# NealLiufighting/hpmpc

Measured on AMD Instinct MI355X. Metric: Riccati factorisations/sec + IP iters/sec, fp64, N=100 nx=12 nu=4 batch=1024, higher is better.
Workload: dtype f64

## Files before the change

hpmpc_amd/bindings.py:

```python
from __future__ import annotations

import ctypes as C
import os

import numpy as np

LIBPATH = os.environ.get("HPMPC_MI355X_LIB") or os.path.join(os.path.dirname(os.path.abspath(__file__)), "lib",
                                                             "libhpmpc_mi355x.so")

_CTYPE = dict(v=None, i=C.c_int, d=C.c_double, l=C.c_longlong, p=C.c_void_p, s=C.c_char_p)
_SIG = dict(
    plan_create="p:ippppp",
    plan_destroy="v:p",
    ws_doubles="l:p",
    ipm_batch="i:ppiiippppppppidddiipppp",
    ipm_solo="i:ppiiippppppppidddiipppp",
    ipm_pass="i:ppiiippppppppidddiipppip",
    ipm_batch_profiled="i:ppiiippppppppidddiippppp",
    ipm_queue="i:ppiiipppppppppidddiipppppp",
    ric_sv_batch="i:ppiiipppppiipp",
    ric_trf_batch="i:ppiiipppp",
    ric_trs_batch="i:ppiiipppppppiipp",
    last_error="i:",
    version="s:",
    pcond_plan_create="p:ipppppi",
    pcond_plan_destroy="v:p",
    pcond_sizes="i:pp",
    pcond_offsets="i:pip",
    pcond_batch="i:piiippppppppp",
    pcond_ric_sv_batch="i:piiipppppip",
    pexpand_batch="i:piiippppppppppp",
    wide_plan_create="p:ippppp",
    wide_plan_destroy="v:p",
    wide_sizes="i:pp",
    wide_offsets="i:pp",
    wide_ipm_batch="i:piiipppppppppidddiipppp",
    pcond_wide_plan="p:p",
    soft_plan_create="p:ipppppp",
    soft_plan_destroy="v:p",
    soft_sizes="i:pp",
    soft_offsets="i:pp",
    ipm_soft_batch="i:ppiiippppppppppidddiipppp",
    ocp_plan_create="p:ipppppi",
    ocp_plan_destroy="v:p",
    ocp_tile_plan="p:p",
    ocp_sizes="i:pp",
    ocp_offsets="i:pp",
    ocp_pack_batch="i:ppiiiipppppppp",
    ocp_ipm_batch="i:piiipppppppppidddiipppp",
    ocp_finish_batch="i:piiipppppppppppppppp",
    kkt_scratch_doubles="l:p",
    kkt_new_rhs_batch="i:ppiiiippppppppppppip",
    ocp_kkt_batch="i:piiippppppppppp",
    ocp_unpack_sets="i:piiiippppppppppp",
    kkt_tangent_batch="i:ppiiiippppppppppppip",
    ocp_tangent_batch="i:ppiiiippppppppppip",
    kkt_adjoint_batch="i:ppiiiippppppppppppp",
    ocp_adjoint_batch="i:piiiipppppppppppppppppp",
    ocp_matrix_grads_batch="i:piiiipppppppp",
    ocp_adjoint_data_batch="i:piiiippppppppppppppp",
    ocp_matrix_dirs_batch="i:ppiiiippppppp",
    ocp_tangent_data_batch="i:ppiiiipppppppppppppip",
)
SIGNATURES = {"hpmpc_mi355x_" + n: (_CTYPE[s[0]], [_CTYPE[c] for c in s[2:]]) for n, s in _SIG.items()}

_LIB = None


def bind(L):
    for name, (restype, argtypes) in SIGNATURES.items():
        fn = getattr(L, name, None)
        if fn is not None:
            fn.restype, fn.argtypes = restype, argtypes
    return L


def lib() -> C.CDLL:
    global _LIB
    if _LIB is None:
        if not os.path.exists(LIBPATH):
            raise RuntimeError(f"libhpmpc_mi355x.so not built ({LIBPATH}); run __graft_entry__.build()")
        _LIB = bind(C.CDLL(LIBPATH, mode=os.RTLD_LOCAL | getattr(os, "RTLD_NOW", 2)))
    return _LIB


def check(rc: int, name: str) -> None:
    if rc != 0:
        raise RuntimeError(f"{name} failed ({rc})")


def plan_args(idxb, *sizes):
    ints = lambda a: np.ascontiguousarray(a, dtype=np.int32)
    arrs, idx = [ints(a) for a in sizes], [ints(a) for a in idxb]
    idxp = (C.POINTER(C.c_int) * len(idx))(*[a.ctypes.data_as(C.POINTER(C.c_int)) for a in idx])
    return [a.ctypes.data for a in arrs], C.cast(idxp, C.c_void_p), (arrs, idx, idxp)
```

hpmpc_amd/build.py:

```python
from __future__ import annotations

import os
import subprocess

ROOT = os.path.dirname(os.path.dirname(os.path.abspath(__file__)))
CSRC = os.path.join(ROOT, "hpmpc_amd", "csrc")
LIBDIR = os.path.join(ROOT, "hpmpc_amd", "lib")
HIPCC = os.environ.get("HIPCC", "/opt/rocm/bin/hipcc")
ARCH = os.environ.get("HPMPC_ARCH", "gfx950")
SOURCES = ["hpmpc_kernels.hip", "hk_wide.hip", "hk_wide_ipm.hip", "hk_soft.hip", "hk_soft_ipm.hip", "hk_ocp.hip", "hk_kkt.hip", "hk_tan.hip", "hk_adj.hip", "hk_matgrad.hip", "hk_matdir.hip", "hpmpc_capi.cpp",
           "hpmpc_capi_queue.cpp", "hpmpc_capi_dropin.cpp", "hpmpc_capi_soft.cpp", "hpmpc_capi_soft_batch.cpp",
           "hpmpc_capi_wide.cpp", "hpmpc_capi_pcond.cpp", "hpmpc_capi_wide_ipm.cpp", "hpmpc_capi_iface.cpp",
           "hpmpc_capi_mpc.cpp", "hpmpc_capi_ocp.cpp", "hpmpc_capi_kkt.cpp"]
HEADERS = ["hpmpc_api.h", "hk_ipm_body.h", "hk_prims.h", "hk_riccati.h", "hk_ipm.h", "hk_mw.h", "hpmpc_kargs.h", "hk_wide_args.h", "hk_wide_core.h", "hk_wide_host.h", "hk_pcond_plan.h", "hk_soft_args.h", "hk_soft_body.h", "hk_launch_guard.h", "hk_launch.h", "hk_host.h", "hk_plan.h", "hk_ocp_args.h", "hk_kkt_args.h", "hk_kkt_body.h", "hk_ocp_plan.h", "hk_tan_args.h", "hk_tan_body.h", "hk_ocp_place.h", "hk_kkt_launch.h", "hk_adj_args.h", "hk_adj_body.h", "hk_matgrad_args.h", "hk_matdir_args.h"]
KFLAGS = ["-mllvm", "-amdgpu-mfma-vgpr-form"] + os.environ.get("HK_EXTRA_FLAGS", "").split()
SRC_FLAGS = {"hpmpc_kernels.hip": ["-mllvm", "-amdgpu-sched-strategy=max-memory-clause"],
             "hk_kkt.hip": ["-mllvm", "-amdgpu-sched-strategy=max-memory-clause"],
             "hk_tan.hip": ["-mllvm", "-amdgpu-sched-strategy=max-memory-clause"],
             "hk_adj.hip": ["-mllvm", "-amdgpu-sched-strategy=max-memory-clause"]}


EXPORTS = os.path.join(CSRC, "exports.map")


def _newer(out, deps):
    if not os.path.exists(out):
        return False
    t = os.path.getmtime(out)
    return all(os.path.getmtime(d) <= t for d in deps)


def _deps(src, hdrs_all):
    import re
    seen, todo = set(), [os.path.join(CSRC, src)]
    while todo:
        path = todo.pop()
        try:
            text = open(path).read()
        except OSError:
            continue
        for name in re.findall(r'^\s*#\s*include\s+"([^"]+)"', text, re.M):
            for cand in (os.path.join(os.path.dirname(path), name), os.path.join(CSRC, name),
                         os.path.join(ROOT, "include", os.path.basename(name))):
                if os.path.exists(cand) and cand not in seen:
                    seen.add(cand)
                    todo.append(cand)
                    break
    return sorted(seen | {h for h in hdrs_all if os.path.basename(h) == "hpmpc_mi355x.h"})


def build_hip(force: bool = False, verbose: bool = False, variant: str | None = None, extra=(), sources=()) -> str:
    os.makedirs(LIBDIR, exist_ok=True)
    objdir = os.path.join(ROOT, "build", "obj" if variant is None else f"obj_{variant}")
    os.makedirs(objdir, exist_ok=True)
    out = os.path.join(LIBDIR, "libhpmpc_mi355x.so")
    if variant is not None:
        os.makedirs(os.path.join(LIBDIR, "ab"), exist_ok=True)
        out = os.path.join(LIBDIR, "ab", f"lib{variant}.so")
    hdrs_all = [os.path.join(CSRC, h) for h in HEADERS] + [os.path.join(ROOT, "include", "hpmpc_mi355x.h")]
    common = [HIPCC, f"--offload-arch={ARCH}", "-O3", "-std=c++17", "-fPIC", "-fvisibility=hidden", "-Wall",
              "-Wno-unused-function"] + KFLAGS + list(extra)
    objs, procs = [], []
    for src in SOURCES + list(sources):
        obj = os.path.join(objdir, src + ".o")
        objs.append(obj)
        if force or not _newer(obj, [os.path.join(CSRC, src)] + _deps(src, hdrs_all)):
            cmd = common + SRC_FLAGS.get(src, []) + ["-c", os.path.join(CSRC, src), "-o", obj]
            if verbose:
                print(" ".join(cmd), flush=True)
            procs.append((src, subprocess.Popen(cmd)))
    for src, pr in procs:
        if pr.wait() != 0:
            raise subprocess.CalledProcessError(pr.returncode, src)
    if procs or force or not _newer(out, objs + [EXPORTS]):
        cmd = [HIPCC, f"--offload-arch={ARCH}", "-shared", "-fPIC", f"-Wl,--version-script={EXPORTS}"] + objs + \
              ["-o", out]
        if verbose:
            print(" ".join(cmd), flush=True)
        subprocess.run(cmd, check=True)
    return out


def build_stamps(verbose: bool = False, force: bool = False) -> str:
    out = build_hip(force=force, verbose=verbose, variant="stamps", extra=["-DHK_STAMPS"])
    dst = os.path.join(LIBDIR, "libhpmpc_mi355x_stamps.so")
    if not _newer(dst, [out]):
        import shutil

        shutil.copy2(out, dst)
    return dst


def build_ric2(verbose: bool = False, force: bool = False) -> str:
    return build_hip(force=force, verbose=verbose, variant="ric2", extra=["-DHK_RIC2"], sources=["hk_ric2.hip"])


def build_calib(verbose: bool = False) -> str:
    os.makedirs(LIBDIR, exist_ok=True)
    out = os.path.join(LIBDIR, "libhbm_calib.so")
    src = os.path.join(ROOT, "tools", "hbm_calib.hip")
    if _newer(out, [src, os.path.join(CSRC, "hk_prims.h")]):
        return out
    cmd = [HIPCC, f"--offload-arch={ARCH}", "-O3", "-std=c++17", "-fPIC", "-shared", src, "-o", out]
    if verbose:
        print(" ".join(cmd), flush=True)
    subprocess.run(cmd, check=True)
    return out


def build_oracle(force: bool = False) -> None:
    odir = os.path.join(ROOT, "oracle")
    targets = ["oracle", "oracle_fma"]
    if os.path.isdir(os.environ.get("HPMPC_REF", "/root/reference")):
        targets += ["ref", "ref_avx"]
    subprocess.run(["make", "-s", "-C", odir] + (["-B"] if force else []) + targets, check=True)
    if "ref" in targets:
        subprocess.run(["make", "-s", "-C", os.path.join(ROOT, "tools", "relink"), "drivers"], check=True)


def build_all(force: bool = False, verbose: bool = False) -> None:
    build_hip(force=force, verbose=verbose)
    build_stamps(verbose=verbose, force=force)
    build_ric2(verbose=verbose, force=force)
    build_calib(verbose=verbose)
    build_oracle(force=force)


if __name__ == "__main__":
    build_all(force=True, verbose=True)
```

hpmpc_amd/csrc/hk_ipm_body.h:

```cpp
#pragma once
#include "hk_ipm.h"
#include "hk_launch_guard.h"
#include "hpmpc_kargs.h"

using namespace hk;

#ifndef HK_WAVES
#define HK_WAVES 2
#endif
#define HK_TWO_WAVES __attribute__((amdgpu_waves_per_eu(HK_WAVES)))

namespace {

struct Ws {
    double *F, *dux, *dpi, *Pb, *Qx, *qx, *res_q, *res_b, *ux_bkp, *pi_bkp;
    double *dlam, *dt, *t_inv, *lamt, *res_d, *res_m, *t_bkp, *lam_bkp;
    double* state;
    double* cert;
};

enum { S_MU = 0, S_ALPHA, S_SIGMA, S_SMU, S_KK, S_PHASE, S_ACTIVE, S_MUSCAL, S_RET };

__device__ __forceinline__ Ws carve(double* W, int N) {
    Ws w;
    const long n1 = N + 1, a = n1 * V16, b = n1 * V32;
    w.F = W;
    W += n1 * FSTRIDE;
    w.dux = W;
    w.dpi = W + a;
    w.Pb = W + 2 * a;
    w.Qx = W + 3 * a;
    w.qx = W + 4 * a;
    w.res_q = W + 5 * a;
    w.res_b = W + 6 * a;
    w.ux_bkp = W + 7 * a;
    w.pi_bkp = W + 8 * a;
    W += 9 * a;
    w.dlam = W;
    w.dt = W + b;
    w.t_inv = W + 2 * b;
    w.lamt = W + 3 * b;
    w.res_d = W + 4 * b;
    w.res_m = W + 5 * b;
    w.t_bkp = W + 6 * b;
    w.lam_bkp = W + 7 * b;
    w.state = W + 8 * b;
    w.cert = w.state + 16;
    return w;
}

extern __shared__ __attribute__((aligned(16))) char hk_smem[];

struct LdsTabs {
    Scratch* sm;
    const StageInfo* st;
    const signed char* tileslot;
    const signed char* slotvar;
    double* gc;
};

__device__ __forceinline__ LdsTabs lds_tables(const KArgs& a) {
    LdsTabs T;
    T.sm = reinterpret_cast<Scratch*>(hk_smem);
    StageInfo* st = reinterpret_cast<StageInfo*>(hk_smem + sizeof(Scratch));
    signed char* ts = reinterpret_cast<signed char*>(st + (a.N + 1));
    signed char* sv = ts + (a.N + 1) * 16;
    const int l = lane_id(), n1 = a.N + 1;
    const int* gst = reinterpret_cast<const int*>(a.st);
    int* lst = reinterpret_cast<int*>(st);
    for (int i = l; i < n1 * 16; i += 64) lst[i] = gst[i];
    const int* gts = reinterpret_cast<const int*>(a.tileslot);
    const int* gsv = reinterpret_cast<const int*>(a.slotvar);
    int* lts = reinterpret_cast<int*>(ts);
    int* lsv = reinterpret_cast<int*>(sv);
    for (int i = l; i < n1 * 4; i += 64) {
        lts[i] = gts[i];
        lsv[i] = gsv[i];
    }
    __syncthreads();
    T.st = st;
    T.tileslot = ts;
    T.slotvar = sv;
    T.gc = reinterpret_cast<double*>(sv + n1 * 16);
    return T;
}

static_assert(LDS_FIXED == sizeof(Scratch) && LDS_PER_STAGE == sizeof(StageInfo) + 40, "hpmpc_kargs.h LDS constants");
constexpr size_t lds_table_bytes(int N) { return LDS_FIXED + (size_t)(N + 1) * LDS_PER_STAGE; }

__device__ __forceinline__ RicIO make_io(const KArgs& a, const LdsTabs& T, int p, double* F) {
    RicIO io;
    io.N = a.N;
    io.st = T.st;
    io.tileslot = T.tileslot;
    io.BAbt = a.BAbt + (long)p * a.sB;
    io.RSQ = a.RSQ + (long)p * a.sR;
    io.BAbtS = a.BAbt;
    io.RSQS = a.RSQ;
    io.F = F;
    io.DCt = a.DCt ? a.DCt + (long)p * a.sG : a.RSQ;
    return io;
}

__device__ __forceinline__ void wsync() { __syncthreads(); }

}

namespace {

template <int CH>
__device__ void init_var(const RicIO& io, const double* dv, double* ux, double* pi, double* dpi, double* lam,
                         double* t, double mu0, int warm_start) {
    const int l = lane_id(), g = l >> 4, c = l & 15;
    const double thr0 = 0.1;
    const int nq = (io.N + 4) / 4;
    for (int q0 = 0; q0 < nq; q0 += CH) {
        double dl[CH], du[CH], xv[CH];
        int lo[CH], up[CH], iv[CH];
        bool kv[CH], bx[CH], kp[CH];
#pragma unroll
        for (int j = 0; j < CH; j++) {
            const int k = 4 * (q0 + j) + g;
            kv[j] = k <= io.N;
            kp[j] = k < io.N;
            const int kc = kv[j] ? k : io.N;
            const StageInfo& si = io.st[kc];
            const bool okv = c < si.nu + si.nx;
            const int tile = c < si.nu ? c : si.xo + (c - si.nu);
            const int slot = okv ? io.tileslot[kc * 16 + (okv ? tile : 0)] : -1;
            bx[j] = kv[j] && slot >= 0;
            lo[j] = kc * V32 + (slot >= 0 ? slot : 0);
            up[j] = lo[j] + si.pnb;
            iv[j] = kc * V16 + c;
            dl[j] = gld(dv, lo[j], bx[j]);
            du[j] = gld(dv, up[j], bx[j]);
            xv[j] = warm_start ? gld(ux, iv[j], kv[j]) : 0.0;
        }
#pragma unroll
        for (int j = 0; j < CH; j++) {
            double x = xv[j];
            double tl = -dl[j] + x, tu = du[j] - x;
            if (tl < thr0) {
                if (tu < thr0) {
                    x = (-du[j] + dl[j]) * 0.5;
                    tl = thr0;
                    tu = thr0;
                } else {
                    tl = thr0;
                    x = dl[j] + thr0;
                }
            } else if (tu < thr0) {
                tu = thr0;
                x = du[j] - thr0;
            }
            x = bx[j] ? x : xv[j];
            gst(ux, iv[j], x, kv[j]);
            gst(pi, iv[j], 0.0, kp[j]);
            gst(dpi, iv[j], 0.0, kv[j]);
            gst(t, lo[j], tl, bx[j]);
            gst(t, up[j], tu, bx[j]);
            gst(lam, lo[j], mu0 / tl, bx[j]);
            gst(lam, up[j], mu0 / tu, bx[j]);
        }
    }
}

__device__ void init_var_gen(const RicIO& io, const double* dv, const double* ux, double* lam, double* t,
                             double mu0) {
    const int l = lane_id(), c = l & 15;
    const double thr0 = 0.1;
    for (int k = 0; k <= io.N; k++) {
        const StageInfo si = load_stage(io.st, k);
        if (si.ng == 0) continue;
        const DynSh sh(si);
        const int vc = tile_var(c, sh.nu, sh.nx, sh.xo);
        const double x = gld(ux, k * V16 + vc, vc >= 0);
        double dg[4];
        gen_dg(io, sh, dg);
#pragma unroll
        for (int lc = 0; lc < 4; lc++) {
            if (4 * lc >= sh.ng) continue;
            const GenLane q = gen_lane(k, sh.pnb, sh.ng, lc);
            const bool st = q.ok && c == 0;
            const double dx = row_sum16(dg[lc] * x);
            const double tl = fmax(thr0, dx + (-gld(dv, q.lo, q.ok)));
            const double tu = fmax(thr0, -dx + gld(dv, q.up, q.ok));
            gst(t, q.lo, tl, st);
            gst(t, q.up, tu, st);
            gst(lam, q.lo, mu0 / tl, st);
            gst(lam, q.up, mu0 / tu, st);
        }
    }
}

__device__ __forceinline__ BoxCtx box_ctx(const Ws& w, const double* dv, double* lam, double* t) {
    BoxCtx bc{};
    bc.d = dv;
    bc.lam = lam;
    bc.t = t;
    bc.dlam = w.dlam;
    bc.dt = w.dt;
    bc.t_inv = w.t_inv;
    bc.lamt = w.lamt;
    bc.res_d = w.res_d;
    bc.res_m = w.res_m;
    bc.qxs = w.qx;
    bc.Qx = w.Qx;
    bc.qx = w.qx;
    bc.cert = w.cert;
    bc.cert_out = w.cert;
    bc.cert_new = 0;
    bc.res_q = w.res_q;
    bc.res_b = w.res_b;
    return bc;
}

}

namespace {

struct IpmView {
    int N, q, l;
    Ws w;
    RicIO io;
    BoxTab bt;
    double *ux, *pi, *lam, *t, *stat;
    const double* dv;
    BoxCtx bc;
};

__device__ __forceinline__ int* qcount(const KArgs& a, int p) { return a.qctl + 2 + a.nslots + p; }
__device__ __forceinline__ int* qlist(const KArgs& a, int p) { return a.qctl + 4 + a.nslots + p * a.nslots; }
__device__ __forceinline__ void qlist_push(const KArgs& a, int p, int s) {
    if (lane_id() == 0) qlist(a, p)[atomicAdd(qcount(a, p), 1)] = s;
}

struct Who {
    int s, q, d;
};

__device__ __forceinline__ bool who_am_i(const KArgs& a, Who& w) {
    if (a.nq == 0) {
        const int p = blockIdx.x + a.p0;
        w.s = w.q = w.d = p;
        return p < a.nprob;
    }
    const int n = __builtin_amdgcn_readfirstlane(*qcount(a, a.qpar));
    if ((int)blockIdx.x >= n) return false;
    w.s = __builtin_amdgcn_readfirstlane(qlist(a, a.qpar)[blockIdx.x]);
    w.q = __builtin_amdgcn_readfirstlane(a.qctl[2 + w.s]);
    w.d = w.q >= 0 ? w.q % a.nprob : 0;
    return w.q >= 0;
}

__device__ __forceinline__ bool slot_active(const KArgs& a, const Who& who) {
    return carve(a.ws + (long)who.s * a.sW, a.N).state[S_ACTIVE] != 0.0;
}

__device__ __forceinline__ IpmView ipm_view(const KArgs& a, const LdsTabs& T, const Who& who) {
    IpmView v;
    v.N = a.N;
    v.q = who.q;
    v.l = lane_id();
    v.w = carve(a.ws + (long)who.s * a.sW, a.N);
    v.io = make_io(a, T, who.d, v.w.F);
    v.bt = BoxTab{T.tileslot, T.slotvar};
    const long o16 = (long)who.q * a.sV16, o32 = (long)who.q * a.sV32;
    v.ux = a.ux + o16;
    v.pi = a.pi + o16;
    v.lam = a.lam + o32;
    v.t = a.t + o32;
    v.dv = a.d + (long)who.d * a.sV32;
    v.stat = a.stat + (long)who.q * 5 * a.k_max;
    v.bc = box_ctx(v.w, v.dv, v.lam, v.t);
    v.bc.ux = v.ux;
    v.bc.pi = v.pi;
    return v;
}

__device__ __forceinline__ ResIO res_io(const IpmView& v) {
    ResIO ro{};
    ro.ux = v.ux;
    ro.pi = v.pi;
    ro.dux = v.w.dux;
    ro.dpi = v.w.dpi;
    ro.ux_bkp = v.w.ux_bkp;
    ro.pi_bkp = v.w.pi_bkp;
    ro.lam_bkp = v.w.lam_bkp;
    ro.t_bkp = v.w.t_bkp;
    ro.rq = v.w.res_q;
    ro.rb = v.w.res_b;
    ro.rd = v.w.res_d;
    ro.rm = v.w.res_m;
    return ro;
}

template <class FX, int CI, int NW = 1>
__device__ double p2_start(const KArgs& a, IpmView& v, const MwSplit& mws = MwSplit{0, nullptr}) {
    const double mu = update_p2_pass<CI, false, true, NW>(v.io, v.bc, v.bt.slotvar, 0.0, 1.0 / (2.0 * a.nbt), v.ux,
                                                          v.pi, nullptr, nullptr, nullptr, nullptr, nullptr, nullptr,
                                                          v.w.res_d, v.w.res_m, mws);
    wsync();
    return mu;
}

template <class FX, int CI, int NW = 1>
__device__ bool ipm_continue(const KArgs& a, IpmView& v, int kk, double mu, double alpha, double sigma, int phase,
                             const MwSplit& mws = MwSplit{0, nullptr}) {
    const bool sn = a.single_newton != 0;
    bool active;
    if (a.phase1_only) {
        active = kk < a.k_max && mu > a.mu_tol && alpha >= a.alpha_min;
    } else {
        if (phase == 1) {
            const double mu_tol_low = a.mu_tol < 1e-5 ? 1e-5 : a.mu_tol;
            if (!(kk < a.k_max && mu > mu_tol_low && alpha >= a.alpha_min)) {
                mu = p2_start<FX, CI, NW>(a, v, mws);
                phase = 2;
            }
        }
        active = phase == 1;
        if (phase == 2) active = kk < a.k_max && (sn || (mu > a.mu_tol && alpha >= a.alpha_min));
    }
    int ret = 0;
    if (!active) {
        if (!sn && mu <= a.mu_tol)
            ret = 0;
        else if (kk >= a.k_max)
            ret = 1;
        else if (alpha < a.alpha_min)
            ret = 2;
        else
            ret = -1;
    }
    if (v.l == 0) {
        double* st = v.w.state;
        st[S_MU] = mu;
        st[S_ALPHA] = alpha;
        st[S_SIGMA] = sigma;
        st[S_KK] = kk;
        st[S_PHASE] = phase;
        st[S_ACTIVE] = active ? 1.0 : 0.0;
        if (!active) {
            a.kk[v.q] = kk;
            a.ret[v.q] = ret;
        }
    }
    return active;
}

template <class FX, int CI, bool SHORTCUT>
__device__ bool ipm_start(const KArgs& a, const LdsTabs& T, IpmView& v) {
    Scratch& sm = *T.sm;
    const int N = v.N, l = v.l;
    const int nbt = a.nbt;
    if (!SHORTCUT && nbt == 0) return false;
    if (SHORTCUT && nbt == 0 && a.phase1_only) {
        ric_backward<true, BX_NONE, FX>(v.io, &sm, 0, nullptr, 0, nullptr, v.bc, 1, v.w.Pb);
        wsync();
        ric_forward_sv<FX>(v.io, &sm, 0, nullptr, v.w.dux, a.compute_mult, v.w.dpi);
        if (l == 0) {
            v.w.state[S_ACTIVE] = 0.0;
            a.kk[v.q] = 0;
            a.ret[v.q] = 0;
        }
        return false;
    }
    if (SHORTCUT && nbt == 0) {
        ric_backward<true, BX_NONE, FX>(v.io, &sm, 0, nullptr, 0, nullptr, v.bc, 1, v.w.Pb);
        wsync();
        ric_forward_sv<FX>(v.io, &sm, 0, nullptr, v.ux, a.compute_mult, v.pi);
        wsync();
        for (int i = l; i < (N + 1) * V16; i += 64) {
            v.w.ux_bkp[i] = v.ux[i];
            v.w.pi_bkp[i] = v.pi[i];
        }
        if (l == 0) {
            v.w.state[S_ACTIVE] = 0.0;
            a.kk[v.q] = 0;
            a.ret[v.q] = 0;
        }
        return false;
    }
    const bool sn = a.single_newton != 0;
    if (!sn) {
        init_var<CI>(v.io, v.dv, v.ux, v.pi, v.w.dpi, v.lam, v.t, a.mu0, a.warm_start);
        if (a.ngt) {
            wsync();
            init_var_gen(v.io, v.dv, v.ux, v.lam, v.t, a.mu0);
        }
    } else {
        for (int i = l; i < (N + 1) * V16; i += 64) v.w.dpi[i] = 0.0;
    }
    if (l == 0) v.w.state[S_MUSCAL] = 1.0 / (2.0 * nbt);
    wsync();
    double mu = a.mu0;
    if (sn) mu = p2_start<FX, CI>(a, v);
    return ipm_continue<FX, CI>(a, v, 0, mu, 1.0, 0.0, sn ? 2 : 1);
}

template <class FX, int CI, bool SHORTCUT>
__device__ bool ipm_refill(const KArgs& a, const LdsTabs& T, int s) {
    const bool l0 = lane_id() == 0;
    for (;;) {
        int q = 0;
        if (l0) q = atomicAdd(a.qnext, 1);
        q = __builtin_amdgcn_readfirstlane(q);
        if (q >= a.nq) {
            if (l0) a.qctl[2 + s] = -1;
            return false;
        }
        if (l0) a.qctl[2 + s] = q;
        const Who who{s, q, q % a.nprob};
        IpmView v = ipm_view(a, T, who);
        if (ipm_start<FX, CI, SHORTCUT>(a, T, v)) return true;
        if (l0) atomicAdd(&a.qctl[1], 1);
    }
}

}

namespace {

template <class FX>
__device__ __forceinline__ void fact_body(const KArgs& a, const LdsTabs& T, IpmView& v) {
    Scratch& sm = *T.sm;
    const double* st = v.w.state;
    const bool sn = a.single_newton != 0;
    const bool first = st[S_KK] == 0.0;
    if (first && st[S_PHASE] != 1.0) {
        cert_pass(v.io, v.w.cert);
        wsync();
    }
    if (!first || st[S_PHASE] != 1.0)
        for (int i = v.l; i <= v.N; i += 64) T.gc[i] = v.w.cert[i];
    wsync();
    v.bc.cert = T.gc;
    if (st[S_PHASE] == 1.0) {
        if (first)
            ric_backward<true, BX_P1, FX, CERT_FORM>(v.io, &sm, 0, nullptr, 0, nullptr, v.bc, 1, v.w.Pb);
        else
            ric_backward<true, BX_P1, FX, CERT_LOAD>(v.io, &sm, 0, nullptr, 0, nullptr, v.bc, 1, v.w.Pb);
    } else {
        v.bc.res_rhs = !sn;
        v.bc.no_tinv = a.no_bkp;
        ric_backward<true, BX_P2R, FX, CERT_LOAD>(v.io, &sm, 0, nullptr, 0, nullptr, v.bc, 1, v.w.Pb);
    }
}

template <class FX>
__device__ __forceinline__ void pred_body(const KArgs& a, const LdsTabs& T, IpmView& v) {
    Scratch& sm = *T.sm;
    double* st = v.w.state;
    const bool sn = a.single_newton != 0;
    const int phase = (int)st[S_PHASE], kk = (int)st[S_KK];
    const double mu = st[S_MU];
    double sigma = st[S_SIGMA];
    double al = 1.0;
    if (phase == 1) {
        v.bc.pred = 1;
        ric_forward<0, BX_P1, FX, true>(v.io, &sm, nullptr, 0, v.w.dux, 0, v.w.dpi, v.bc, al);
    } else {
        ric_forward<0, BX_P2, FX, true>(v.io, &sm, v.w.res_b, !sn, v.w.dux, 0, v.w.dpi, v.bc, al);
    }
    al = wave_min(al);
    wsync();
    const double alpha = al * 0.995;
    const double mu_aff = mu_aff_pass<7>(v.io, v.bc, alpha, st[S_MUSCAL]);
    double smu = a.mu0;
    if (!sn) {
        sigma = mu_aff / mu;
        sigma = sigma * sigma * sigma;
        smu = sigma * mu;
    }
    if (v.l == 0) {
        v.stat[5 * kk] = st[S_SIGMA];
        v.stat[5 * kk + 1] = al;
        v.stat[5 * kk + 2] = mu_aff;
        st[S_SIGMA] = sigma;
        st[S_SMU] = smu;
    }
}

template <class FX>
__device__ __forceinline__ void corr_body(const KArgs& a, const LdsTabs& T, IpmView& v) {
    Scratch& sm = *T.sm;
    double* st = v.w.state;
    const int phase = (int)st[S_PHASE], kk = (int)st[S_KK];
    v.bc.smu = st[S_SMU];
    double al = 1.0;
    if (phase == 1)
        ric_trs<BX_P1, BX_P1, FX, false>(v.io, &sm, nullptr, nullptr, v.bc, v.w.dux, a.compute_mult, v.w.dpi, 0, v.w.Pb,
                                         al);
    else
        ric_trs<BX_P2, BX_P2, FX, false>(v.io, &sm, v.w.res_b, v.w.res_q, v.bc, v.w.dux, a.compute_mult, v.w.dpi, 0,
                                         v.w.Pb, al);
    al = wave_min(al);
    if (v.l == 0) {
        v.stat[5 * kk] = st[S_SIGMA];
        v.stat[5 * kk + 3] = al;
        st[S_ALPHA] = al * 0.995;
    }
}

template <class FX, int CI>
__device__ __forceinline__ bool update_body(const KArgs& a, IpmView& v) {
    double* st = v.w.state;
    const int phase = (int)st[S_PHASE];
    int kk = (int)st[S_KK];
    const double alpha = st[S_ALPHA];
    double mu;
    if (phase == 1) {
        mu = update_p1_pass<CI>(v.io, v.bc, alpha, st[S_MUSCAL], v.ux, v.pi, v.w.dux, v.w.dpi, v.w.ux_bkp,
                                v.w.pi_bkp, v.w.lam_bkp, v.w.t_bkp);
    } else {
        if (a.no_bkp)
            mu = update_p2_pass<CI, true, false>(v.io, v.bc, v.bt.slotvar, alpha, st[S_MUSCAL], v.ux, v.pi, v.w.dux,
                                                 v.w.dpi, v.w.ux_bkp, v.w.pi_bkp, v.w.lam_bkp, v.w.t_bkp, v.w.res_d,
                                                 v.w.res_m);
        else
            mu = update_p2_pass<CI, true>(v.io, v.bc, v.bt.slotvar, alpha, st[S_MUSCAL], v.ux, v.pi, v.w.dux, v.w.dpi,
                                          v.w.ux_bkp, v.w.pi_bkp, v.w.lam_bkp, v.w.t_bkp, v.w.res_d, v.w.res_m);
    }
    wsync();
    if (v.l == 0) v.stat[5 * kk + 4] = mu;
    kk++;
    return ipm_continue<FX, CI>(a, v, kk, mu, alpha, st[S_SIGMA], phase);
}

}
```

hpmpc_amd/csrc/hk_plan.h:

```cpp
#pragma once
#include <climits>
#include <mutex>
#include <vector>

#include "hk_host.h"
#include "hk_soft_args.h"
#include "hpmpc_kargs.h"

struct StageInfoH {
    int nu, nx, nb, ng, xo, nx1, nu1, xo1, sdB, sdR, oB, oR, oD, pnb, r0, oG;
};

struct hpmpc_mi355x_plan {
    int N = 0;
    std::vector<int> nx, nu, nb, ng;
    std::vector<std::vector<int>> idxb;
    std::vector<StageInfoH> st;
    std::vector<signed char> tileslot, slotvar;
    std::vector<long long> offB, offR;
    long long packB = 0, packR = 0;
    DevTable<StageInfoH> d_st;
    DevTable<signed char> d_tileslot, d_slotvar;
    struct LayoutTable {
        std::vector<StageInfoH> st;
        DevTable<StageInfoH> d;
    };
    mutable std::vector<LayoutTable> ltabs;
    mutable std::mutex ltabs_mu;
    int fixcls = 0;
    int nbt = 0;
    int ngt = 0;
    std::vector<long long> offG;
    long long packG = 0;
};

inline long long ws_doubles(int N) {
    const long long n = (long long)(N + 1) * (FSTRIDE + 9 * V16 + 8 * V32 + 1) + 16;
    return (n + 31) / 32 * 32;
}

bool plan_supported(int N, const int* nx, const int* nu, const int* nb, const int* const* idxb, const int* ng,
                    const char** why);
void idxb_table(int N, const int* nb, const int* const* idxb, int* out);
bool range_ok(const void* plan, int nprob, int p0, int count, const char* who);
int null_array(const char* who);
int launch_error(int e, const char* what);
inline bool sets_ok(int nprob, int n, const char* what) {
    if (n >= 1 && (long long)nprob * n <= INT_MAX) return true;
    hk_set_error(HPMPC_MI355X_EUNSUPPORTED, what);
    return false;
}
enum DctPolicy { DCT_NONE, DCT_ARRAY };
bool batch_args(KArgs& a, const hpmpc_mi355x_plan* P, const hpmpc_mi355x_layout* lay, int nprob, int p0,
                DctPolicy policy, const double* DCt = nullptr);
int launch(int which, const KArgs* a, int count, hipStream_t s);
int ipm_run(KArgs& a, int count, const double* BAbt, const double* RSQrq, const double* d, double* ux, double* pi,
            double* lam, double* t, double* ws, int k_max, double mu0, double mu_tol, double alpha_min, int warm_start,
            int compute_mult, int* kk, int* ret, double* stat, int which, void* stream);
hpmpc_mi355x_plan* thread_plan(int N, const int* nx, const int* nu, const int* nb, int** idxb, const int* ng);

struct Arena {
    size_t BAbt, RSQ, DCt, d, ux, pi, lam, t, ws, vb, vq, vQx, vqx, vPb, stat, ints, qctl, total;
};
Arena arena(const hpmpc_mi355x_plan* P, int k_max);
KArgs arena_args(const hpmpc_mi355x_plan* P, const Arena& A, double* dev);
void stage_BAbt(const hpmpc_mi355x_plan* P, double* H, const Arena& A, double** hpBAbt);
void stage_RSQ(const hpmpc_mi355x_plan* P, double* H, const Arena& A, double** hpQ);
bool run(int which, const KArgs& a, const char* name);
enum VecKind { VEC_UX, VEC_PI, VEC_CV };
void vec_in(const hpmpc_mi355x_plan* P, VecKind kind, double* H, size_t off, double** v);
void vec_out(const hpmpc_mi355x_plan* P, VecKind kind, double** v, const double* H, size_t off);

struct SoftLayout {
    std::vector<SoftStage> st;
    long sC = 0, sD = 0, sZ = 0;
    long sF = 0;
};
double soft_mu_scal(int N, const int* nb, const int* ns);
void soft_ric_flags(KArgs& a, int compute_mult);
SoftArgs soft_scalars(int N, int nprob, int p0, int k_max, int warm_start, double mu0, double mu_tol, double alpha_min,
                      double mu_scal);
const char* soft_unsupported(int N, const int* nx, const int* nu, const int* ng);
const char* soft_layout(int N, const int* nx, const int* nu, const int* nb, const int* ns, SoftLayout& L);
```

hpmpc_amd/csrc/hk_riccati.h:

```cpp
#pragma once

#include "hk_prims.h"
#include "hpmpc_kargs.h"

namespace hk {

struct StageInfo {
    int nu, nx, nb, ng;
    int xo;
    int nx1, nu1, xo1;
    int sdB, sdR;
    int oB, oR, oD;
    int pnb;
    int r0;
    int oG;
};

using ::FSTRIDE;
using ::V16;
using ::V32;

__device__ __forceinline__ bool tile_active(int t, int nu, int nx, int xo) {
    return t < nu || (t >= xo && t < xo + nx);
}
// ... 81 lines not shown
    HK_BSTAMP(2);
    const double i1 = chol_inv(fma(-l10, l10, a11));
    const double l21 = fma(-l20, l10, a21) * i1, l31 = fma(-l30, l10, a31) * i1;
    const double y1 = fma(-y0, l10, x[1]) * i1;
    const double p1 = fma(-p0, l10, m1) * i1;
    HK_BSTAMP(3);
    const double i2 = chol_inv(fma(-l21, l21, fma(-l20, l20, a22)));
    const double l32 = fma(-l31, l21, fma(-l30, l20, a32)) * i2;
    const double y2 = fma(-y1, l21, fma(-y0, l20, x[2])) * i2;
    const double p2 = fma(-p1, l21, fma(-p0, l20, m2)) * i2;
    HK_BSTAMP(4);
    const double i3 = chol_inv(fma(-l32, l32, fma(-l31, l31, fma(-l30, l30, a33))));
    const double y3 = fma(-y2, l32, fma(-y1, l31, fma(-y0, l30, x[3]))) * i3;
    const double p3 = fma(-p2, l32, fma(-p1, l31, fma(-p0, l30, m3))) * i3;
    HK_BSTAMP(5);
    if (KGEN && B == 0) {
        const bool ut = c < 4;
        const double e0 = ut ? (c == 0 ? 1.0 : 0.0) : y0, e1 = ut ? (c == 1 ? 1.0 : 0.0) : y1;
        const double e2 = ut ? (c == 2 ? 1.0 : 0.0) : y2, e3 = ut ? (c == 3 ? 1.0 : 0.0) : y3;
        const double z3 = e3 * i3;
        const double z2 = fma(-l32, z3, e2) * i2;
        const double z1 = fma(-l31, z3, fma(-l21, z2, e1)) * i1;
        const double z0 = fma(-l30, z3, fma(-l20, z2, fma(-l10, z1, e0))) * i0;
        *kg = -sel_g(z0, z1, z2, z3);
    }
    const double yg = sel_g(y0, y1, y2, y3);
    M[B] = yg;
    const int j = c - 4 * B;
    const bool inb = (c >> 2) == B, below = c > 4 * B + 3;
    invd = inb ? sel_q(i0, i1, i2, i3) : invd;
    if (AUG) {
        const double mt = fma(-p3, y3, fma(-p2, y2, fma(-p1, y1, fma(-p0, y0, ml))));
        const double mb = sel_q(p0, p1, p2, p3);
        ml = below ? mt : (inb ? mb : ml);
    }
    HK_BSTAMP(6);
    (void)j;
    if (B < 3) {
        const double a = below ? yg : 0.0;
        M = mfma(-a, a, M);
    }
#undef HK_BSTAMP
}

template <int B, bool AUG, bool KGEN>
__device__ __forceinline__ void chol_block_row(const d4& S, double invd, double& ml, double* kg) {
    const int l = lane_id(), c = l & 15;
    double y[4];
    rowgroup_gather(S[B], y);
    const double i0 = row_bcast<4 * B + 0>(invd), i1 = row_bcast<4 * B + 1>(invd);
    const double i2 = row_bcast<4 * B + 2>(invd), i3 = row_bcast<4 * B + 3>(invd);
    const double l10 = row_bcast<4 * B + 1>(y[0]), l20 = row_bcast<4 * B + 2>(y[0]), l30 = row_bcast<4 * B + 3>(y[0]);
    const double l21 = row_bcast<4 * B + 2>(y[1]), l31 = row_bcast<4 * B + 3>(y[1]);
    const double l32 = row_bcast<4 * B + 3>(y[2]);
    if (KGEN && B == 0) {
        const bool ut = c < 4;
        const double e0 = ut ? (c == 0 ? 1.0 : 0.0) : y[0], e1 = ut ? (c == 1 ? 1.0 : 0.0) : y[1];
        const double e2 = ut ? (c == 2 ? 1.0 : 0.0) : y[2], e3 = ut ? (c == 3 ? 1.0 : 0.0) : y[3];
        const double z3 = e3 * i3;
        const double z2 = fma(-l32, z3, e2) * i2;
        const double z1 = fma(-l31, z3, fma(-l21, z2, e1)) * i1;
        const double z0 = fma(-l30, z3, fma(-l20, z2, fma(-l10, z1, e0))) * i0;
        *kg = -sel_g(z0, z1, z2, z3);
    }
    if (AUG) {
        const double m0 = row_bcast<4 * B + 0>(ml), m1 = row_bcast<4 * B + 1>(ml);
        const double m2 = row_bcast<4 * B + 2>(ml), m3 = row_bcast<4 * B + 3>(ml);
        const double p0 = m0 * i0;
        const double p1 = fma(-p0, l10, m1) * i1;
        const double p2 = fma(-p1, l21, fma(-p0, l20, m2)) * i2;
        const double p3 = fma(-p2, l32, fma(-p1, l31, fma(-p0, l30, m3))) * i3;
        const bool inb = (c >> 2) == B, below = c > 4 * B + 3;
        const double mt = fma(-p3, y[3], fma(-p2, y[2], fma(-p1, y[1], fma(-p0, y[0], ml))));
        const double mb = sel_q(p0, p1, p2, p3);
        ml = below ? mt : (inb ? mb : ml);
    }
}

template <bool AUG, bool KGEN>
__device__ __forceinline__ void stage_chol_row(const d4& S, double invd, double& ml, int nu, int nx, int xo, bool full,
                                               double* kg) {
    const int hi = full ? xo + nx : nu;
    if (0 < nu || (full && 3 >= xo && 0 < hi)) chol_block_row<0, AUG, KGEN>(S, invd, ml, kg);
    if (4 < nu || (full && 7 >= xo && 4 < hi)) chol_block_row<1, AUG, false>(S, invd, ml, nullptr);
    if (8 < nu || (full && 11 >= xo && 8 < hi)) chol_block_row<2, AUG, false>(S, invd, ml, nullptr);
    if (12 < nu || (full && 15 >= xo && 12 < hi)) chol_block_row<3, AUG, false>(S, invd, ml, nullptr);
}

__device__ __forceinline__ double diag_sel(const d4& v) {
    const int c = lane_id() & 15;
    const bool b0 = (c & 4) != 0, b1 = (c & 8) != 0;
    const double lo = b0 ? v[1] : v[0], hi = b0 ? v[3] : v[2];
    return b1 ? hi : lo;
}
__device__ __forceinline__ bool diag_lane() {
    const int l = lane_id();
    return (l & 3) == (l >> 4);
}

__device__ __forceinline__ double wave_min_lb(double x) {
    float f = (float)x;
    f = f - fabsf(f) * 0x1p-22f - 0x1p-126f;
    asm volatile(
        "s_nop 1\n\t"
        "v_min_f32_dpp %0, %0, %0 row_ror:8 row_mask:0xf bank_mask:0xf\n\t"
        "s_nop 1\n\t"
        "v_min_f32_dpp %0, %0, %0 row_ror:4 row_mask:0xf bank_mask:0xf\n\t"
        "s_nop 1\n\t"
        "v_min_f32_dpp %0, %0, %0 row_ror:2 row_mask:0xf bank_mask:0xf\n\t"
        "s_nop 1\n\t"
        "v_min_f32_dpp %0, %0, %0 row_ror:1 row_mask:0xf bank_mask:0xf"
        : "+v"(f));
    int v = __builtin_bit_cast(int, f);
    const auto a = __builtin_amdgcn_permlane32_swap(v, v, false, false);
    f = __builtin_fminf(__builtin_bit_cast(float, (int)a[0]), __builtin_bit_cast(float, (int)a[1]));
    v = __builtin_bit_cast(int, f);
    const auto b = __builtin_amdgcn_permlane16_swap(v, v, false, false);
    return (double)__builtin_fminf(__builtin_bit_cast(float, (int)b[0]), __builtin_bit_cast(float, (int)b[1]));
}

template <class SH>
__device__ __forceinline__ double cert_g_gersh(const d4& Mi, const SH& sh) {
    const int c = lane_id() & 15;
    const double rs = xrow_sum((fabs(Mi[0]) + fabs(Mi[1])) + (fabs(Mi[2]) + fabs(Mi[3])));
    const double d = diag_sel(Mi);
    const double m = (diag_lane() && tile_active(c, sh.nu, sh.nx, sh.xo)) ? d + fabs(d) - rs : 1e300;
    return wave_min_lb(m);
}

#ifdef HK_STAMPS
__device__ unsigned long long g_xfac_stat[6];
__device__ unsigned g_xfac_sweep[1 << 16];
#endif
constexpr double CERT_ALLOW = 1e-11;

__device__ __forceinline__ bool cert_ok(const d4& M, double dq, double gc, double allow = CERT_ALLOW) {
    const double cc = fma(allow, gc, 1e-15), g2 = gc * gc;
    const bool bad = !(gc > 0.0) || dq < 0.0 || (diag_lane() && !((diag_sel(M) - dq) * cc < g2));
    return __builtin_amdgcn_ballot_w64(bad) == 0;
}

__device__ __forceinline__ double cert_thr(double g) {
    const double T = (g * g) * rcp_nr(fma(CERT_ALLOW, g, 1e-15)) * (1.0 - 0x1p-40);
    return g > 0.0 ? T : -__builtin_inf();
}
__device__ __forceinline__ d4 cert_diag_w() {
    const int l = lane_id(), g = l >> 4, c = l & 15;
    d4 w;
#pragma unroll
    for (int r = 0; r < 4; r++) w[r] = (c == g + 4 * r) ? 1.0 : 0.0;
    return w;
}
__device__ __forceinline__ bool cert_ok_thr(const d4& M, double dq, double T, const d4& w) {
    const double d = w[0] * M[0] + w[1] * M[1] + w[2] * M[2] + w[3] * M[3];
    return __builtin_amdgcn_ballot_w64(!(d - dq < T)) == 0;
}

template <class SH>
__device__ __forceinline__ double cert_form(const d4& Mi, double dq, const SH& sh) {
    const double T = cert_thr(cert_g(Mi, sh));
    return __builtin_amdgcn_ballot_w64(dq < 0.0) != 0 ? -__builtin_inf() : T;
}
__device__ __forceinline__ bool cert_test(const d4& M, double dq, double gc) {
    return cert_ok_thr(M, dq, gc, cert_diag_w());
}

template <int R>
__device__ __forceinline__ double lrow_blk(double v) {
    return sel_g(row_bcast<4 * R + 0>(v), row_bcast<4 * R + 1>(v), row_bcast<4 * R + 2>(v), row_bcast<4 * R + 3>(v));
}

__device__ __forceinline__ double xcol_op(const d4& L, int R, int xo) {
    const int l = lane_id(), g = l >> 4, c = l & 15;
    const int p = 4 * R + g;
    return (p >= xo && c >= p) ? L[R] : 0.0;
}

__device__ __forceinline__ void pform_eff_tile(const d4& L, int nx, int xo, d4& M) {
    const int l = lane_id(), g = l >> 4, c = l & 15;
    const d4 z = {0.0, 0.0, 0.0, 0.0};
    d4 Pe = z;
#pragma unroll
    for (int R = 0; R < 4; R++) {
        if (4 * R + 3 < xo || 4 * R >= xo + nx) continue;
        const double a = xcol_op(L, R, xo);
        Pe = mfma(a, a, Pe);
    }
#pragma unroll
    for (int r = 0; r < 4; r++) M[r] = (g + 4 * r >= xo && c >= xo) ? Pe[r] : M[r];
}

__device__ __forceinline__ void pform_eff_row(const d4& L, double lx, int nx, int xo, double& ml) {
    const int c = lane_id() & 15;
    double part = 0.0;
    if (4 * 0 + 3 >= xo && 0 < xo + nx) part += xcol_op(L, 0, xo) * lrow_blk<0>(lx);
    if (4 * 1 + 3 >= xo && 4 < xo + nx) part += xcol_op(L, 1, xo) * lrow_blk<1>(lx);
    if (4 * 2 + 3 >= xo && 8 < xo + nx) part += xcol_op(L, 2, xo) * lrow_blk<2>(lx);
    if (4 * 3 + 3 >= xo && 12 < xo + nx) part += xcol_op(L, 3, xo) * lrow_blk<3>(lx);
    const double pe = xrow_sum(part);
    ml = c >= xo ? pe : ml;
}

template <bool AUG>
__device__ __forceinline__ void xblocks_chol(d4& M, double& ml, double& invd, int nx, int xo) {
    const int hi = xo + nx;
    if (0 >= xo && 0 < hi) chol_block<0, AUG>(M, ml, invd);
    if (4 >= xo && 4 < hi) chol_block<1, AUG>(M, ml, invd);
    if (8 >= xo && 8 < hi) chol_block<2, AUG>(M, ml, invd);
    if (12 >= xo && 12 < hi) chol_block<3, AUG>(M, ml, invd);
}

__device__ __forceinline__ void xblocks_chol_row(const d4& L, double invd, double& ml, int nx, int xo) {
    const int hi = xo + nx;
    if (0 >= xo && 0 < hi) chol_block_row<0, true, false>(L, invd, ml, nullptr);
    if (4 >= xo && 4 < hi) chol_block_row<1, true, false>(L, invd, ml, nullptr);
    if (8 >= xo && 8 < hi) chol_block_row<2, true, false>(L, invd, ml, nullptr);
    if (12 >= xo && 12 < hi) chol_block_row<3, true, false>(L, invd, ml, nullptr);
}

struct XFac {
    d4 L;
    double invd;
};

template <bool AUG, bool KGEN = false>
__device__ __forceinline__ void stage_chol(d4& M, double& ml, double& invd, int nu, int nx, int xo, bool full,
                                           bool transpose, double* kg = nullptr, int kdbg = -1, bool xfac = false,
                                           XFac* xf = nullptr) {
    const int l = lane_id(), g = l >> 4, c = l & 15;
    (void)kdbg;
    invd = 0.0;
    const int hi = full ? xo + nx : nu;
    if (0 < nu || (full && 3 >= xo && 0 < hi)) chol_block<0, AUG, KGEN>(M, ml, invd, kg, kdbg);
    HK_STAMP(16, kdbg);
    if (4 < nu || (full && 7 >= xo && 4 < hi)) chol_block<1, AUG>(M, ml, invd, nullptr, kdbg);
    HK_STAMP(18, kdbg);
    if (8 < nu || (full && 11 >= xo && 8 < hi)) chol_block<2, AUG>(M, ml, invd, nullptr, kdbg);
    HK_STAMP(20, kdbg);
    if (12 < nu || (full && 15 >= xo && 12 < hi)) chol_block<3, AUG>(M, ml, invd, nullptr, kdbg);
    HK_STAMP(22, kdbg);
    const bool xf_now = xfac;
#ifdef HK_COUNT_NOFALLBACK
    asm volatile("" ::"s"(__builtin_amdgcn_readfirstlane((int)xf_now)));
    if (false) {
#else
    if (!full && xf_now) {
#endif
        d4 L = M;
        double lx = ml, ivx = invd;
        xblocks_chol<AUG>(L, lx, ivx, nx, xo);
        pform_eff_tile(L, nx, xo, M);
        if (AUG) pform_eff_row(L, lx, nx, xo, ml);
        if (xf) {
            xf->L = L;
            xf->invd = ivx;
        }
    }
    if (!transpose) return;
    const d4 z = {0.0, 0.0, 0.0, 0.0};
    d4 T0 = mfma(M[0], (c == g) ? 1.0 : 0.0, z);
    d4 T1 = mfma(M[1], (c == 4 + g) ? 1.0 : 0.0, z);
    T0 = mfma(M[2], (c == 8 + g) ? 1.0 : 0.0, T0);
    T1 = mfma(M[3], (c == 12 + g) ? 1.0 : 0.0, T1);
    const d4 T = T0 + T1;
#pragma unroll
    for (int r = 0; r < 4; r++) M[r] = (g + 4 * r > c) ? T[r] : M[r];
}

template <class SH>
__device__ __forceinline__ double cert_g_shift(const d4& Mi, const SH& sh) {
    const int l = lane_id(), g = l >> 4, c = l & 15;
    const bool act = tile_active(c, sh.nu, sh.nx, sh.xo);
    const double dm = -wave_min((diag_lane() && act) ? -diag_sel(Mi) : 0.0);
    const double tau = dm * 0x1p-10;
    d4 A = Mi;
#pragma unroll
    for (int r = 0; r < 4; r++) A[r] -= (g + 4 * r == c && act) ? tau : 0.0;
    double ml = 0.0, invd = 0.0;
    stage_chol<false, false>(A, ml, invd, sh.nu, sh.nx, sh.xo, true, false);
    const bool ok = dm > 0.0 && __builtin_amdgcn_ballot_w64(act && !(invd > 0.0)) == 0;
    return ok ? tau - 1e-12 * dm : -1.0;
}

template <class SH>
__device__ __forceinline__ double cert_g(const d4& Mi, const SH& sh) {
    const double g = cert_g_gersh(Mi, sh);
#ifdef HK_COUNT_NOSHIFT
    return g;
#endif
    if (g > 0.0) return g;
    return cert_g_shift(Mi, sh);
}

struct RicIO {
    int N;
    const StageInfo* st;
    const signed char* tileslot;
    const double* BAbt;
    const double* RSQ;
    const double* BAbtS;
    const double* RSQS;
    double* F;
    const double* DCt;
};

__device__ __forceinline__ StageInfo load_stage(const StageInfo* st, int k) {
    const StageInfo v = st[k];
    StageInfo u;
    u.nu = __builtin_amdgcn_readfirstlane(v.nu);
    u.nx = __builtin_amdgcn_readfirstlane(v.nx);
    u.nb = __builtin_amdgcn_readfirstlane(v.nb);
    u.ng = __builtin_amdgcn_readfirstlane(v.ng);
    u.xo = __builtin_amdgcn_readfirstlane(v.xo);
    u.nx1 = __builtin_amdgcn_readfirstlane(v.nx1);
    u.nu1 = __builtin_amdgcn_readfirstlane(v.nu1);
    u.xo1 = __builtin_amdgcn_readfirstlane(v.xo1);
    u.sdB = __builtin_amdgcn_readfirstlane(v.sdB);
    u.sdR = __builtin_amdgcn_readfirstlane(v.sdR);
    u.oB = __builtin_amdgcn_readfirstlane(v.oB);
    u.oR = __builtin_amdgcn_readfirstlane(v.oR);
    u.oD = __builtin_amdgcn_readfirstlane(v.oD);
    u.pnb = __builtin_amdgcn_readfirstlane(v.pnb);
    u.r0 = __builtin_amdgcn_readfirstlane(v.r0);
    u.oG = __builtin_amdgcn_readfirstlane(v.oG);
    return u;
}

struct StageRef {
    const StageInfo* p;
    int k;
};
__device__ __forceinline__ int srd(const StageRef& s, int StageInfo::*m) {
    return __builtin_amdgcn_readfirstlane(s.p[s.k].*m);
}

struct DynSh {
    static constexpr bool fixed = false;
    int nu, nx, xo, nx1, nu1, xo1, sdB, sdR, nb, pnb, oB, oR, ng, oG, fl;
    __device__ __forceinline__ explicit DynSh(const StageInfo& s)
        : nu(s.nu), nx(s.nx), xo(s.xo), nx1(s.nx1), nu1(s.nu1), xo1(s.xo1), sdB(s.sdB), sdR(s.sdR), nb(s.nb),
          pnb(s.pnb), oB(s.oB), oR(s.oR), ng(s.ng), oG(s.oG), fl(s.r0) {}
    __device__ __forceinline__ explicit DynSh(const StageRef& s)
        : nu(srd(s, &StageInfo::nu)), nx(srd(s, &StageInfo::nx)), xo(srd(s, &StageInfo::xo)),
          nx1(srd(s, &StageInfo::nx1)), nu1(srd(s, &StageInfo::nu1)), xo1(srd(s, &StageInfo::xo1)),
          sdB(srd(s, &StageInfo::sdB)), sdR(srd(s, &StageInfo::sdR)), nb(srd(s, &StageInfo::nb)),
          pnb(srd(s, &StageInfo::pnb)), oB(srd(s, &StageInfo::oB)), oR(srd(s, &StageInfo::oR)),
          ng(srd(s, &StageInfo::ng)), oG(srd(s, &StageInfo::oG)), fl(srd(s, &StageInfo::r0)) {}
};

template <int NU, int NX>
struct FixSh {
    static constexpr bool fixed = true, enabled = true;
    static constexpr int nu = NU, nx = NX, xo = (NU + 3) / 4 * 4, nx1 = NX, nu1 = NU, xo1 = xo,
                         sdB = (NX + 1) / 2 * 2, sdR = (NU + NX + 1) / 2 * 2;
    int nb, pnb, oB, oR, fl;
    __device__ __forceinline__ explicit FixSh(const StageInfo& s)
        : nb(s.nb), pnb(s.pnb), oB(s.oB), oR(s.oR), fl(s.r0) {}
    __device__ __forceinline__ explicit FixSh(const StageRef& s)
        : nb(srd(s, &StageInfo::nb)), pnb(srd(s, &StageInfo::pnb)), oB(srd(s, &StageInfo::oB)),
          oR(srd(s, &StageInfo::oR)), fl(srd(s, &StageInfo::r0)) {}
};


__device__ __forceinline__ int stage_flags(const StageInfo& s) { return s.r0; }
template <class SH>
__device__ __forceinline__ int stage_flags(const SH& s) { return s.fl; }
template <class SH>
__device__ __forceinline__ const double* stage_B(const RicIO& io, const SH& sh) {
    return ((stage_flags(sh) & 2) ? io.BAbtS : io.BAbt) + sh.oB;
}
template <class SH>
__device__ __forceinline__ const double* stage_R(const RicIO& io, const SH& sh) {
    return ((stage_flags(sh) & 4) ? io.RSQS : io.RSQ) + sh.oR;
}

struct NoFix {
    static constexpr bool enabled = false;
    __device__ __forceinline__ explicit NoFix(const StageInfo&) {}
    __device__ __forceinline__ explicit NoFix(const StageRef&) {}
};

inline int fixcls_of(int nu, int nx) { return nu == 4 && nx == 12 ? 1 : nu == 3 && nx == 8 ? 2 : 0; }
template <class FX>
struct FxTag {
    using type = FX;
};
template <class F>
int with_fixcls(int fixcls, F&& f) {
    switch (fixcls) {
        case 1: return f(FxTag<FixSh<4, 12>>{});
        case 2: return f(FxTag<FixSh<3, 8>>{});
        default: return f(FxTag<NoFix>{});
    }
}

template <class FX, class F>
__device__ __forceinline__ void with_shape(const StageInfo& s, F&& f) {
#ifdef HK_COUNT_FIXED
    if constexpr (FX::enabled) { f(FX(s)); return; }
#endif
    if constexpr (FX::enabled) {
        if (s.r0 & 1) {
            f(FX(s));
            return;
        }
    }
    f(DynSh(s));
}
template <class FX, class F>
__device__ __forceinline__ void with_shape(const StageRef& s, F&& f) {
#ifdef HK_COUNT_FIXED
    if constexpr (FX::enabled) { f(FX(s)); return; }
#endif
    if constexpr (FX::enabled) {
        if (srd(s, &StageInfo::r0) & 1) {
            f(FX(s));
            return;
        }
    }
    f(DynSh(s));
}

__device__ __forceinline__ double lowS(const d4& S, int r, int g, int c) { return (g + 4 * r >= c) ? S[r] : 0.0; }

__device__ __forceinline__ void load_factor(const double* Fk, d4& S, double& lc, double& invd) {
    const int l = lane_id(), c = l & 15;
#pragma unroll
    for (int r = 0; r < 4; r++) S[r] = Fk[r * 64 + l];
    lc = Fk[256 + c];
    invd = Fk[272 + c];
}

__device__ __forceinline__ void store_factor(double* Fk, const d4& S, double lc, double invd, double kg,
                                             bool ok = true) {
    const int l = lane_id(), g = l >> 4, c = l & 15;
#pragma unroll
    for (int r = 0; r < 4; r++) gst(Fk, r * 64 + l, S[r], ok);
    gst(Fk, 256 + 16 * g + c, g == 0 ? lc : invd, ok && g < 2);
    gst(Fk, 288 + l, kg, ok);
}

constexpr int FXR_L = 64, FXR_INVD = 80, FXR_KG = 96, FXR_P = 160;

__device__ __forceinline__ int fxr_pidx(int i, int j) {
    const int a = i > j ? i : j, b = i > j ? j : i;
    return FXR_P + (a * (a + 1) >> 1) + b;
}

template <int NX>
__device__ __forceinline__ void store_factor_fixed(double* Fk, const d4& S, double lc, double invd, double kg,
                                                   bool ok) {
    const int l = lane_id(), g = l >> 4, c = l & 15;
    gst(Fk, l, S[0], false);
    gst(Fk, FXR_L + 16 * g + c, g == 0 ? lc : invd, ok && g < 2);
    gst(Fk, FXR_KG + l, kg, ok);
    const int j = c - 4;
#pragma unroll
    for (int r = 1; r < 4; r++) {
        const int i = g + 4 * r - 4;
        gst(Fk, fxr_pidx(i, j), S[r], ok && j >= 0 && j <= i && i < NX);
    }
}

template <int NX>
__device__ __forceinline__ void load_p_fixed(const double* Fk, d4& S, bool ok) {
    const int l = lane_id(), g = l >> 4, c = l & 15;
    const int j = c - 4;
#pragma unroll
    for (int r = 1; r < 4; r++) {
        const int i = g + 4 * r - 4;
        S[r] = gld(Fk, fxr_pidx(i, j), ok && j >= 0 && i < NX && j < NX);
    }
}

enum BoxMode { BX_NONE = 0, BX_GIVEN = 1, BX_P1 = 2, BX_P2 = 3, BX_P2R = 4 };

constexpr bool cert_loaded(int bm) { return bm == BX_P1 || bm == BX_P2 || bm == BX_P2R; }

struct BoxCtx {
    const double* d;
    double *lam, *t;
    double *dlam, *dt, *t_inv, *lamt, *res_d, *res_m;
    double* qxs;
    const double *Qx, *qx;
    double smu;
    int pred;
    const double *ux, *pi;
    double *res_q, *res_b;
    int res_rhs;
    int no_tinv;
    const double* cert;
    double* cert_out;
    int cert_new;
};

struct BoxLane {
    int lo, up, s16;
    bool ok;
};

__device__ __forceinline__ BoxLane box_lane(const signed char* tileslot, int pnb, int k) {
    const int c = lane_id() & 15;
    const int slot = tileslot[k * 16 + c];
    BoxLane b;
    b.ok = slot >= 0;
    b.lo = k * V32 + slot;
    b.up = b.lo + pnb;
    b.s16 = k * V16 + slot;
    return b;
}

__device__ __forceinline__ void ld_lu(const double* p, const BoxLane& b, double& vlo, double& vup) {
    const bool odd = (lane_id() & 16) != 0;
    const int m = -(int)odd;
    const double x = gld(p, (b.up & m) | (b.lo & ~m), b.ok);
    const int xl = __double2loint(x), xh = __double2hiint(x);
    const auto cl = __builtin_amdgcn_permlane16_swap(xl, xl, false, false);
    const auto ch = __builtin_amdgcn_permlane16_swap(xh, xh, false, false);
    vlo = mk((int)ch[0], (int)cl[0]);
    vup = mk((int)ch[1], (int)cl[1]);
}

__device__ __forceinline__ void fetch_pair(const double* p, const BoxLane& b, double& e0, double& e1) {
    e0 = gld(p, b.lo, b.ok);
    e1 = gld(p, b.up, b.ok);
}
__device__ __forceinline__ void use_pair(double e0, double e1, double& vlo, double& vup) {
    vlo = e0;
    vup = e1;
}

__device__ __forceinline__ void st_lu(double* p, const BoxLane& b, double vlo, double vup, bool ok) {
    const bool odd = (lane_id() & 16) != 0;
    const int m = -(int)odd;
    gst(p, (b.up & m) | (b.lo & ~m), odd ? vup : vlo, ok && lane_id() < 32);
}

__device__ __forceinline__ void alpha_rule(double& al, double v, double dv) {
    const double cand = -v * rcp_nr(dv);
    al = (-al * dv > v) ? cand : al;
}


struct GenLane {
    int lo, up, s16;
    bool ok;
};

__device__ __forceinline__ GenLane gen_lane(int k, int pnb, int ng, int lc) {
    const int gl = 4 * lc + (lane_id() >> 4);
    const int png = (ng + 3) & ~3;
    GenLane q;
    q.ok = gl < ng;
    q.lo = k * V32 + 2 * pnb + gl;
    q.up = q.lo + png;
    q.s16 = k * V16 + pnb + gl;
    return q;
}

__device__ __forceinline__ void gen_dg(const RicIO& io, const DynSh& sh, double dg[4]) {
    const int l = lane_id(), g = l >> 4, c = l & 15;
    const int vc = tile_var(c, sh.nu, sh.nx, sh.xo);
    const int cng = (sh.ng + 1) & ~1;
    const double* D = io.DCt + sh.oG;
#pragma unroll
    for (int lc = 0; lc < 4; lc++) {
        const int gl = 4 * lc + g;
        dg[lc] = (4 * lc < sh.ng) ? gld(D, lib4_idx(cng, vc, gl), vc >= 0 && gl < sh.ng) : 0.0;
    }
}

template <int BM>
__device__ void gen_hessian(const RicIO& io, const DynSh& sh, int k, const BoxCtx& bc, double x, d4& M, double& ml,
                            bool aug) {
    const int c = lane_id() & 15;
    double dg[4];
    gen_dg(io, sh, dg);
    double part = 0.0;
#pragma unroll
    for (int lc = 0; lc < 4; lc++) {
        if (4 * lc >= sh.ng) continue;
        const GenLane q = gen_lane(k, sh.pnb, sh.ng, lc);
        const bool st = q.ok && c == 0;
        double Q = 0.0, qv = 0.0;
        if (BM == BX_GIVEN) {
            Q = gld(bc.Qx, q.s16, q.ok);
            qv = aug ? gld(bc.qx, q.s16, q.ok) : 0.0;
        } else if (BM == BX_P1) {
            const double lml = gld(bc.lam, q.lo, q.ok), lmu = gld(bc.lam, q.up, q.ok);
            const double tl = gld(bc.t, q.lo, q.ok), tu = gld(bc.t, q.up, q.ok);
            const double dl = gld(bc.d, q.lo, q.ok), du = gld(bc.d, q.up, q.ok);
            const double til = rcp_nr(tl), tiu = rcp_nr(tu);
            const double ltl = lml * til, ltu = lmu * tiu;
            const double dll = til * 0.0, dlu = tiu * 0.0;
            qv = lmu - ltu * du + dlu - lml - ltl * dl - dll;
            Q = ltl + ltu;
            gst(bc.t_inv, q.lo, til, st);
            gst(bc.t_inv, q.up, tiu, st);
            gst(bc.lamt, q.lo, ltl, st);
            gst(bc.lamt, q.up, ltu, st);
            gst(bc.qxs, q.s16, qv, st);
        } else if (BM == BX_P2 || BM == BX_P2R) {
            const double lml = gld(bc.lam, q.lo, q.ok), lmu = gld(bc.lam, q.up, q.ok);
            const double tl = gld(bc.t, q.lo, q.ok), tu = gld(bc.t, q.up, q.ok);
            const double rml = gld(bc.res_m, q.lo, q.ok), rmu = gld(bc.res_m, q.up, q.ok);
            double rdl, rdu;
            if (BM == BX_P2R) {
                const double dx = row_sum16(dg[lc] * x);
                rdl = gld(bc.d, q.lo, q.ok) - dx + tl;
                rdu = gld(bc.d, q.up, q.ok) - dx - tu;
                gst(bc.res_d, q.lo, rdl, st);
                gst(bc.res_d, q.up, rdu, st);
            } else {
                rdl = gld(bc.res_d, q.lo, q.ok);
                rdu = gld(bc.res_d, q.up, q.ok);
            }
            const double til = rcp_nr(tl), tiu = rcp_nr(tu);
            qv = til * (rml - lml * rdl) - tiu * (rmu + lmu * rdu);
            Q = til * lml + tiu * lmu;
            gst(bc.t_inv, q.lo, til, st);
            gst(bc.t_inv, q.up, tiu, st);
        }
        Q = q.ok ? Q : 0.0;
        qv = q.ok ? qv : 0.0;
        M = mfma(dg[lc] * Q, dg[lc], M);
        part += dg[lc] * qv;
    }
    if (aug) ml += xrow_sum(part);
}

__device__ double gen_rq(const RicIO& io, const DynSh& sh, int k, const double* lam) {
    double dg[4];
    gen_dg(io, sh, dg);
    double part = 0.0;
#pragma unroll
    for (int lc = 0; lc < 4; lc++) {
        if (4 * lc >= sh.ng) continue;
        const GenLane q = gen_lane(k, sh.pnb, sh.ng, lc);
        const double w = gld(lam, q.up, q.ok) - gld(lam, q.lo, q.ok);
        part += dg[lc] * (q.ok ? w : 0.0);
    }
    return xrow_sum(part);
}

template <int FM>
__device__ void gen_alpha(const RicIO& io, const DynSh& sh, int k, const BoxCtx& bc, double x, double& al) {
    if (FM == BX_NONE) return;
    const int c = lane_id() & 15;
    double dg[4];
    gen_dg(io, sh, dg);
#pragma unroll
    for (int lc = 0; lc < 4; lc++) {
        if (4 * lc >= sh.ng) continue;
        const GenLane q = gen_lane(k, sh.pnb, sh.ng, lc);
        const bool st = q.ok && c == 0;
        const double dx = row_sum16(dg[lc] * x);
        const double lml = gld(bc.lam, q.lo, q.ok), lmu = gld(bc.lam, q.up, q.ok);
        const double tl = gld(bc.t, q.lo, q.ok), tu = gld(bc.t, q.up, q.ok);
        double dtl, dtu, dll, dlu;
        if (FM == BX_P1) {
            dtl = dx - gld(bc.d, q.lo, q.ok) - tl;
            dtu = -dx + gld(bc.d, q.up, q.ok) - tu;
            const double d0l = gld(bc.dlam, q.lo, q.ok && !bc.pred), d0u = gld(bc.dlam, q.up, q.ok && !bc.pred);
            dll = d0l - (gld(bc.lamt, q.lo, q.ok) * dtl + lml);
            dlu = d0u - (gld(bc.lamt, q.up, q.ok) * dtu + lmu);
        } else {
            dtl = dx - gld(bc.res_d, q.lo, q.ok);
            dtu = -dx + gld(bc.res_d, q.up, q.ok);
            dll = -gld(bc.t_inv, q.lo, q.ok) * (lml * dtl + gld(bc.res_m, q.lo, q.ok));
            dlu = -gld(bc.t_inv, q.up, q.ok) * (lmu * dtu + gld(bc.res_m, q.up, q.ok));
        }
        gst(bc.dt, q.lo, dtl, st);
        gst(bc.dt, q.up, dtu, st);
        gst(bc.dlam, q.lo, dll, st);
        gst(bc.dlam, q.up, dlu, st);
        if (q.ok) {
            alpha_rule(al, lml, dll);
            alpha_rule(al, lmu, dlu);
            alpha_rule(al, tl, dtl);
            alpha_rule(al, tu, dtu);
        }
    }
}

template <int TM>
__device__ double gen_gradient(const RicIO& io, const DynSh& sh, int k, const BoxCtx& bc) {
    if (TM == BX_NONE) return 0.0;
    const int c = lane_id() & 15;
    double dg[4];
    gen_dg(io, sh, dg);
    double part = 0.0;
#pragma unroll
    for (int lc = 0; lc < 4; lc++) {
        if (4 * lc >= sh.ng) continue;
        const GenLane q = gen_lane(k, sh.pnb, sh.ng, lc);
        const bool st = q.ok && c == 0;
        double qv = 0.0;
        if (TM == BX_GIVEN) {
            qv = gld(bc.qx, q.s16, q.ok);
        } else if (TM == BX_P1) {
            const double dll = gld(bc.t_inv, q.lo, q.ok) * (bc.smu - gld(bc.dlam, q.lo, q.ok) * gld(bc.dt, q.lo, q.ok));
            const double dlu = gld(bc.t_inv, q.up, q.ok) * (bc.smu - gld(bc.dlam, q.up, q.ok) * gld(bc.dt, q.up, q.ok));
            gst(bc.dlam, q.lo, dll, st);
            gst(bc.dlam, q.up, dlu, st);
            qv = gld(bc.qxs, q.s16, q.ok) + (dlu - dll);
        } else if (TM == BX_P2) {
            const double rml = gld(bc.res_m, q.lo, q.ok) + (gld(bc.dt, q.lo, q.ok) * gld(bc.dlam, q.lo, q.ok) - bc.smu);
            const double rmu = gld(bc.res_m, q.up, q.ok) + (gld(bc.dt, q.up, q.ok) * gld(bc.dlam, q.up, q.ok) - bc.smu);
            gst(bc.res_m, q.lo, rml, st);
            gst(bc.res_m, q.up, rmu, st);
            qv = gld(bc.t_inv, q.lo, q.ok) * (rml - gld(bc.lam, q.lo, q.ok) * gld(bc.res_d, q.lo, q.ok)) -
                 gld(bc.t_inv, q.up, q.ok) * (rmu + gld(bc.lam, q.up, q.ok) * gld(bc.res_d, q.up, q.ok));
        }
        part += dg[lc] * (q.ok ? qv : 0.0);
    }
    return xrow_sum(part);
}

struct BwdFrag {
    d4 Mi;
    double mlq;
    d4 bop;
    d4 brow;
    double bx[8];
    BoxLane bl;
    double uc, pc, pim1;
    double gc;
};

template <class SH>
__device__ __forceinline__ void load_rsq_tile(const double* R, const SH& sh, d4& Mi) {
    const int l = lane_id(), g = l >> 4, c = l & 15;
    const int vc = tile_var(c, sh.nu, sh.nx, sh.xo);
#pragma unroll
    for (int r = 0; r < 4; r++) {
        const int vi = tile_var(g + 4 * r, sh.nu, sh.nx, sh.xo);
        const int hi = vi > vc ? vi : vc, lo = vi > vc ? vc : vi;
        Mi[r] = ldsel(R, lib4_idx(sh.sdR, hi, lo), vi >= 0 && vc >= 0);
    }
}

__device__ void cert_pass(const RicIO& io, double* cert) {
    const int l = lane_id(), g = l >> 4, c = l & 15;
    for (int k0 = 0; k0 <= io.N; k0 += 8) {
        d4 Mi[8], bop[8];
#pragma unroll
        for (int j = 0; j < 8; j++) {
            const int k = k0 + j <= io.N ? k0 + j : io.N;
            const DynSh sh(StageRef{io.st, k});
            load_rsq_tile(stage_R(io, sh), sh, Mi[j]);
            const int vc = tile_var(c, sh.nu, sh.nx, sh.xo);
            const double* Bk = stage_B(io, sh);
#pragma unroll
            for (int r = 0; r < 4; r++) {
                const int s = 4 * r + g - sh.xo1;
                bop[j][r] = ldsel(Bk, lib4_idx(sh.sdB, vc, s), k < io.N && s >= 0 && s < sh.nx1 && vc >= 0);
            }
        }
#pragma unroll
        for (int j = 0; j < 8; j++) {
            const int k = k0 + j <= io.N ? k0 + j : io.N;
            const DynSh sh(StageRef{io.st, k});
            const double tau = cert_form(Mi[j], 0.0, sh);
            gst(cert, k0 + j, tau, lane_id() == 0 && k0 + j <= io.N);
        }
    }
}

template <bool AUG, int BM, class SH>
__device__ __forceinline__ void bwd_fetch(const RicIO& io, const SH& sh, int k, int update_b, const double* bsrc,
                                          int update_q, const double* qsrc, const BoxCtx& bc, BwdFrag& f) {
    const int l = lane_id(), g = l >> 4, c = l & 15;
    const int nux = sh.nu + sh.nx;
    const double* R = stage_R(io, sh);
    const int vc = tile_var(c, sh.nu, sh.nx, sh.xo);
    load_rsq_tile(R, sh, f.Mi);
    f.mlq = 0.0;
    if (AUG) {
        const double* qp = update_q ? qsrc + k * V16 : R;
        const int qi = update_q ? vc : lib4_idx(sh.sdR, nux, vc);
        f.mlq = ldsel(qp, qi, vc >= 0);
    }
    const BoxLane b = box_lane(io.tileslot, sh.pnb, k);
    f.bl = b;
    f.gc = cert_loaded(BM) ? bc.cert[k] : 0.0;
#pragma unroll
    for (int i = 0; i < 8; i++) f.bx[i] = 0.0;
    if (BM == BX_GIVEN) {
        f.bx[0] = ldsel(bc.Qx, b.s16, b.ok);
        f.bx[1] = AUG ? ldsel(bc.qx, b.s16, b.ok) : 0.0;
    } else if (BM == BX_P1) {
        f.bx[0] = ldsel(bc.lam, b.lo, b.ok);
        f.bx[1] = ldsel(bc.lam, b.up, b.ok);
        f.bx[2] = ldsel(bc.t, b.lo, b.ok);
        f.bx[3] = ldsel(bc.t, b.up, b.ok);
        f.bx[4] = ldsel(bc.d, b.lo, b.ok);
        f.bx[5] = ldsel(bc.d, b.up, b.ok);
    } else if (BM == BX_P2 || BM == BX_P2R) {
        ld_lu(bc.lam, b, f.bx[0], f.bx[1]);
        ld_lu(bc.t, b, f.bx[2], f.bx[3]);
        if (BM == BX_P2) ld_lu(bc.res_m, b, f.bx[4], f.bx[5]);
        ld_lu(bc.res_d, b, f.bx[6], f.bx[7]);
    }
    const bool live = SH::fixed || k < io.N;
    const double* Bk = stage_B(io, sh);
    const double* bp = update_b ? bsrc + k * V16 : Bk;
#pragma unroll
    for (int r = 0; r < 4; r++) {
        const int s = 4 * r + g - sh.xo1;
        const bool ok = live && s >= 0 && s < sh.nx1;
        f.bop[r] = ldsel(Bk, lib4_idx(sh.sdB, vc, s), ok && vc >= 0);
        if (BM != BX_P2R) f.brow[r] = AUG ? ldsel(bp, update_b ? s : lib4_idx(sh.sdB, nux, s), ok) : 0.0;
    }
    if (BM == BX_P2R) {
        static_assert(BM != BX_P2R || AUG, "residual right-hand sides need the augmented row");
        const int sc = c - sh.xo1;
        const bool oks = live && sc >= 0 && sc < sh.nx1;
        f.uc = ldsel(bc.ux, k * V16 + vc, vc >= 0);
        f.pc = ldsel(bc.pi, k * V16 + sc, oks);
        f.pim1 = ldsel(bc.pi, (k - 1) * V16 + (vc - sh.nu), k > 0 && vc >= sh.nu);
        f.brow[0] = ldsel(Bk, lib4_idx(sh.sdB, nux, sc), oks);
    }
}

template <bool AUG, int BM>
__device__ __forceinline__ void box_hessian(const BoxCtx& bc, const BwdFrag& f, double& dq, double& qxv) {
    const int g = lane_id() >> 4;
    const BoxLane& b = f.bl;
    const bool st = b.ok && g == 0;
    dq = 0.0;
    qxv = 0.0;
    if (BM == BX_GIVEN) {
        dq = f.bx[0];
        qxv = f.bx[1];
    } else if (BM == BX_P1) {
        const double til = rcp_nr(f.bx[2]), tiu = rcp_nr(f.bx[3]);
        const double ltl = f.bx[0] * til, ltu = f.bx[1] * tiu;
        const double dll = til * 0.0, dlu = tiu * 0.0;
        const double q = f.bx[1] - ltu * f.bx[5] + dlu - f.bx[0] - ltl * f.bx[4] - dll;
        gst(bc.t_inv, b.lo, til, st);
        gst(bc.t_inv, b.up, tiu, st);
        gst(bc.lamt, b.lo, ltl, st);
        gst(bc.lamt, b.up, ltu, st);
        gst(bc.qxs, b.s16, q, st);
        dq = b.ok ? ltl + ltu : 0.0;
        qxv = (AUG && b.ok) ? q : 0.0;
    } else if (BM == BX_P2 || BM == BX_P2R) {
        const double til = rcp_nr(f.bx[2]), tiu = rcp_nr(f.bx[3]);
        const double rml = BM == BX_P2R ? f.bx[0] * f.bx[2] : f.bx[4];
        const double rmu = BM == BX_P2R ? f.bx[1] * f.bx[3] : f.bx[5];
        const double q = til * (rml - f.bx[0] * f.bx[6]) - tiu * (rmu + f.bx[1] * f.bx[7]);
        if (!bc.no_tinv) st_lu(bc.t_inv, b, til, tiu, b.ok);
        dq = b.ok ? til * f.bx[0] + tiu * f.bx[1] : 0.0;
        qxv = (AUG && b.ok) ? q : 0.0;
    }
}

template <class SH>
__device__ __forceinline__ void bwd_residual(const RicIO& io, Scratch* sm, const SH& sh, int k, const BoxCtx& bc,
                                             BwdFrag& f, double x1c, bool store) {
    const int l = lane_id(), g = l >> 4, c = l & 15;
    const bool live = SH::fixed || k < io.N;
    const int vc = tile_var(c, sh.nu, sh.nx, sh.xo);
    const int sc = c - sh.xo1;
    const bool oks = live && sc >= 0 && sc < sh.nx1;
    double h = f.mlq;
    if (k > 0 && vc >= sh.nu) h -= f.pim1;
    if (f.bl.ok) h += -f.bx[0] + f.bx[1];
    double ur[4], pr[4];
    col2row2(sm, f.uc, f.pc, ur, pr);
    d4 bt = {0.0, 0.0, 0.0, 0.0};
#pragma unroll
    for (int r = 0; r < 4; r++) {
        if (4 * r + 3 < sh.xo1 || 4 * r >= sh.xo1 + sh.nx1) continue;
        bt = mfma(f.bop[r], (c == 4 * r + g) ? 1.0 : 0.0, bt);
    }
    double part = 0.0, p2 = 0.0, p3 = 0.0;
#pragma unroll
    for (int r = 0; r < 4; r++) part += f.Mi[r] * ur[r];
    h += xrow_sum(part);
#pragma unroll
    for (int r = 0; r < 4; r++) {
        p2 += f.bop[r] * pr[r];
        p3 += bt[r] * ur[r];
    }
    const double bpi = xrow_sum(p2);
    const double atu = xrow_sum(p3);
    if (live) h += bpi;
    if constexpr (!SH::fixed) {
        if (sh.ng > 0) h += gen_rq(io, sh, k, bc.lam);
    }
    const double rb = f.brow[0] - (oks ? x1c : 0.0) + atu;
    const int db = (int)(bc.res_b - bc.res_q);
    gst(bc.res_q, g == 0 ? k * V16 + vc : db + k * V16 + sc, g == 0 ? h : rb,
        store && ((g == 0 && vc >= 0) || (g == 1 && oks)));
    f.mlq = bc.res_rhs ? h : f.mlq;
    double bcol = bc.res_rhs ? rb : f.brow[0];
    bcol = oks ? bcol : 0.0;
    double br[4];
    col2row(sm, bcol, br);
#pragma unroll
    for (int r = 0; r < 4; r++) f.brow[r] = br[r];
}

enum CertMode { CERT_LOAD = 0, CERT_FORM = 1, CERT_RT = 2 };
template <bool AUG, int BM, int CN = CERT_RT, class SH>
__device__ __forceinline__ void bwd_pre(const RicIO& io, const SH& sh, int k, const BwdFrag& cur, const BoxCtx& bc,
                                        d4& M, double& ml, double& dq, double& gc) {
    const int l = lane_id(), g = l >> 4, c = l & 15;
    double qxv;
    box_hessian<AUG, BM>(bc, cur, dq, qxv);
#ifdef HK_COUNT_NOCERT
    gc = 0.0;
#else
    if constexpr (cert_loaded(BM)) {
        if constexpr (CN == CERT_LOAD) {
            gc = cur.gc;
        } else if constexpr (CN == CERT_FORM) {
            gc = cert_form(cur.Mi, 0.0, sh);
            gst(bc.cert_out, k, gc, lane_id() == 0);
        } else {
            gc = bc.cert_new ? cert_form(cur.Mi, 0.0, sh) : cur.gc;
            gst(bc.cert_out, k, gc, bc.cert_new && lane_id() == 0);
        }
    } else {
        gc = (SH::fixed || k > 0) ? cert_form(cur.Mi, dq, sh) : 0.0;
    }
#endif
    M = cur.Mi;
    ml = cur.mlq + qxv;
#pragma unroll
    for (int r = 0; r < 4; r++) M[r] += (g + 4 * r == c) ? dq : 0.0;
    if constexpr (!SH::fixed && BM != BX_NONE) {
        if (sh.ng > 0) gen_hessian<BM>(io, sh, k, bc, BM == BX_P2R ? cur.uc : 0.0, M, ml, AUG);
    }
}

template <class SH>
__device__ __forceinline__ void bwd_tile_update(const SH& sh, bool live, const d4& bop, const d4& S, d4& M) {
    const int nx1 = sh.nx1, xo1 = sh.xo1;
    if (live) {
        d4 a0 = {0.0, 0.0, 0.0, 0.0}, a1 = {0.0, 0.0, 0.0, 0.0};
#pragma unroll
        for (int kc = 0; kc < 4; kc++) {
            if (4 * kc + 3 < xo1 || 4 * kc >= xo1 + nx1) continue;
            const double aop = S[kc];
            if (kc & 1)
                a1 = mfma(aop, bop[kc], a1);
            else
                a0 = mfma(aop, bop[kc], a0);
        }
        const d4 acc = a0 + a1;
        d4 m1 = {0.0, 0.0, 0.0, 0.0};
#pragma unroll
        for (int r = 0; r < 4; r++) {
            if (4 * r + 3 < xo1 || 4 * r >= xo1 + nx1) continue;
            if (r & 1)
                m1 = mfma(bop[r], acc[r], m1);
            else
                M = mfma(bop[r], acc[r], M);
        }
        M = M + m1;
    }
}

template <class SH>
__device__ __forceinline__ void bwd_row_update(const RicIO& io, Scratch* sm, const SH& sh, int k, bool live,
                                               const d4& bop, const d4& brow, const d4& S, double ml_prev,
                                               int compute_Pb, double* Pb, double& ml) {
    const int l = lane_id(), g = l >> 4, c = l & 15;
    const int nx1 = sh.nx1, xo1 = sh.xo1;
    const bool xc = c >= xo1;
    double part = 0.0;
#pragma unroll
    for (int r = 0; r < 4; r++) part += S[r] * brow[r];
    const double pb = xrow_sum(part);
    gst(Pb, k * V16 + (c - xo1), pb, compute_Pb && live && g == 0 && xc && c < xo1 + nx1);
    const double wc = xc ? pb + ml_prev : 0.0;
    double wrow[4];
    col2row(sm, wc, wrow);
    double mp = 0.0;
#pragma unroll
    for (int r = 0; r < 4; r++) mp += bop[r] * wrow[r];
    if (live) ml += xrow_sum(mp);
}

template <bool AUG, bool THR, class SH>
__device__ __forceinline__ void bwd_core(const RicIO& io, Scratch* sm, const SH& sh, int k, const d4& bop,
                                         const d4& brow, d4 M, double ml, double dq, double gc, int compute_Pb,
                                         double* Pb, d4& S, double& ml_prev, double& invd_prev, double& kg_prev) {
    const bool live = SH::fixed || k < io.N;
    bwd_tile_update(sh, live, bop, S, M);
    const bool full = !SH::fixed && k == 0;
#ifdef HK_COUNT_NOCERT
    const bool xcert = false;
    (void)dq;
    (void)gc;
#else
    const bool xcert = !full && !cert_test(M, dq, gc);
#endif
#ifdef HK_STAMPS
    if (!full) {
        const bool xfac = xcert, f12 = xcert, f13 = xcert;
        if (lane_id() == 0) {
            atomicAdd(&g_xfac_stat[0], 1ull);
            if (xfac) atomicAdd(&g_xfac_stat[1], 1ull);
            if (xfac) g_xfac_sweep[blockIdx.x & 0xffff] = 1u;
            if (f12) atomicAdd(&g_xfac_stat[2], 1ull);
            if (f13) atomicAdd(&g_xfac_stat[3], 1ull);
        }
    }
#endif
    if (AUG) bwd_row_update(io, sm, sh, k, live, bop, brow, S, ml_prev, compute_Pb, Pb, ml);
    HK_STAMP(2, k);
    double invd, kg = 0.0;
    stage_chol<AUG, SH::fixed>(M, ml, invd, sh.nu, sh.nx, sh.xo, full, !SH::fixed, &kg, k, xcert);
    kg_prev = kg;
    HK_STAMP(3, k);
#pragma unroll
    for (int r = 0; r < 4; r++) S[r] = M[r];
    ml_prev = ml;
    invd_prev = invd;
}

template <bool AUG, int BM, int CN, class SH>
__device__ __forceinline__ void bwd_step(const RicIO& io, Scratch* sm, const SH& sh, int k, const BwdFrag& cur,
                                         const BoxCtx& bc, int compute_Pb, double* Pb, d4& S, double& ml_prev,
                                         double& invd_prev, double& kg_prev) {
    d4 M;
    double ml, dq, gc;
    bwd_pre<AUG, BM, CN>(io, sh, k, cur, bc, M, ml, dq, gc);
    bwd_core<AUG, cert_loaded(BM)>(io, sm, sh, k, cur.bop, cur.brow, M, ml, dq, gc, compute_Pb, Pb, S, ml_prev, invd_prev, kg_prev);
}

template <bool AUG, int BM, class FX, int CN = CERT_LOAD>
__device__ void ric_backward(const RicIO& io, Scratch* sm, int update_b, const double* bsrc, int update_q,
                             const double* qsrc, const BoxCtx& bc, int compute_Pb, double* Pb) {
    d4 S = {0.0, 0.0, 0.0, 0.0};
    double ml_prev = 0.0, invd_prev = 0.0, kg_prev = 0.0;
#ifdef HK_STAMPS
    if (lane_id() == 0) g_xfac_sweep[blockIdx.x & 0xffff] = 0u;
#endif
    StageRef si{io.st, io.N};
    BwdFrag cur;
    with_shape<FX>(si, [&](const auto& sh) {
        bwd_fetch<AUG, BM>(io, sh, io.N, update_b, bsrc, update_q, qsrc, bc, cur);
        if constexpr (BM == BX_P2R) bwd_residual(io, sm, sh, io.N, bc, cur, 0.0, true);
    });
    bool rec_fixed = false;
    auto stage = [&](int k, const BwdFrag& cur, BwdFrag& nxt) __attribute__((always_inline)) {
        HK_STAMP(0, k);
        const int kn = k > 0 ? k - 1 : 0;
        const StageRef sn{io.st, kn};
        HK_STAMP(5, k);
        with_shape<FX>(sn, [&](const auto& sh) { bwd_fetch<AUG, BM>(io, sh, kn, update_b, bsrc, update_q, qsrc, bc, nxt); });
        HK_STAMP(6, k);
        double* Fk1 = io.F + (long)(k + 1) * FSTRIDE;
        if constexpr (FX::enabled) {
            if (rec_fixed)
                store_factor_fixed<FX::nx>(Fk1, S, AUG ? ml_prev : 0.0, invd_prev, kg_prev, k < io.N);
            else
                store_factor(Fk1, S, AUG ? ml_prev : 0.0, invd_prev, kg_prev, k < io.N);
        } else {
            store_factor(Fk1, S, AUG ? ml_prev : 0.0, invd_prev, kg_prev, k < io.N);
        }
        asm volatile("" ::: "memory");
        HK_STAMP(1, k);
        with_shape<FX>(si, [&](const auto& sh) {
            bwd_step<AUG, BM, CN>(io, sm, sh, k, cur, bc, compute_Pb, Pb, S, ml_prev, invd_prev, kg_prev);
            rec_fixed = std::remove_reference_t<decltype(sh)>::fixed;
        });
        if constexpr (BM == BX_P2R)
            with_shape<FX>(sn, [&](const auto& sh) { bwd_residual(io, sm, sh, kn, bc, nxt, cur.uc, k > 0); });
        HK_STAMP(4, k);
        si = sn;
    };
    BwdFrag alt;
    for (int k = io.N;;) {
        stage(k, cur, alt);
        if (--k < 0) break;
        stage(k, alt, cur);
        if (--k < 0) break;
    }
    store_factor(io.F, S, AUG ? ml_prev : 0.0, invd_prev, kg_prev);
#ifdef HK_STAMPS
    if (lane_id() == 0) {
        atomicAdd(&g_xfac_stat[4], 1ull);
        if (g_xfac_sweep[blockIdx.x & 0xffff]) atomicAdd(&g_xfac_stat[5], 1ull);
    }
#endif
}

template <class SH>
__device__ __forceinline__ void solve_lt(const SH& sh, const d4& S, double invd, double rrow[4], double ur[4],
                                         bool all) {
    const int l = lane_id(), g = l >> 4;
#pragma unroll
    for (int p = 15; p >= 0; p--) {
        const bool unk = all ? tile_active(p, sh.nu, sh.nx, sh.xo) : (p < sh.nu);
        if (!unk) continue;
        const int rp = p >> 2, gp = p & 3;
        const double rv = (rp == 0) ? rrow[0] : (rp == 1) ? rrow[1] : (rp == 2) ? rrow[2] : rrow[3];
        const double y = readlane(rv, gp * 16) * readlane(invd, p);
#pragma unroll
        for (int r = 0; r < 4; r++) {
            double sv;
            switch (p) {
#define HK_CASE(P) \
    case P: sv = row_bcast<P>(S[r]); break;
                HK_CASE(0) HK_CASE(1) HK_CASE(2) HK_CASE(3) HK_CASE(4) HK_CASE(5) HK_CASE(6) HK_CASE(7)
                HK_CASE(8) HK_CASE(9) HK_CASE(10) HK_CASE(11) HK_CASE(12) HK_CASE(13) HK_CASE(14)
                default: sv = row_bcast<15>(S[r]); break;
#undef HK_CASE
            }
            if (g + 4 * r < p) rrow[r] -= sv * y;
            if (r == rp && g == gp) ur[r] = y;
        }
    }
}

template <class SH>
__device__ __forceinline__ double solve_ln(const SH& sh, const d4& S, double invd, double h, bool all) {
    const int l = lane_id(), c = l & 15;
#pragma unroll
    for (int p = 0; p < 16; p++) {
        const bool unk = all ? tile_active(p, sh.nu, sh.nx, sh.xo) : (p < sh.nu);
        if (!unk) continue;
        const int rp = p >> 2, gp = p & 3;
        const double y = readlane(h, p) * readlane(invd, p);
        const double src = (rp == 0) ? S[0] : (rp == 1) ? S[1] : (rp == 2) ? S[2] : S[3];
        double colp;
        switch (gp) {
            case 0: colp = rowgroup_bcast<0>(src); break;
            case 1: colp = rowgroup_bcast<1>(src); break;
            case 2: colp = rowgroup_bcast<2>(src); break;
            default: colp = rowgroup_bcast<3>(src); break;
        }
        h = (c == p) ? y : ((c > p) ? h - colp * y : h);
    }
    return h;
}

template <class SH>
__device__ __forceinline__ double trs_usolve(const SH& sh, const d4& S, double invd, double h, bool all) {
    if constexpr (SH::fixed) {
        static_assert(SH::xo == 4, "gain form needs the u block in tile block 0");
        const int c = lane_id() & 15;
        const double hg = sel_g(row_bcast<0>(h), row_bcast<1>(h), row_bcast<2>(h), row_bcast<3>(h));
        const double t = xrow_sum(S[0] * hg);
        return c < 4 ? -t : h + t;
    } else {
        return solve_ln(sh, S, invd, h, all);
    }
}

__device__ __forceinline__ double pi_from_x(const d4& S1, int xo1, const double x1row[4], double pcol) {
    (void)xo1;
    double part = 0.0;
#pragma unroll
    for (int r = 0; r < 4; r++) part += S1[r] * x1row[r];
    return xrow_sum(part) + pcol;
}

struct FwdFrag {
    d4 S;
    double lc, invd;
    double kg;
    d4 bt;
    double bval;
    double hc;
    double pk;
    double bx[10];
    BoxLane bl;
};

template <int MODE, int FM, bool PRED, class SH>
__device__ __forceinline__ void fwd_fetch(const RicIO& io, const SH& sh, int k, int pnbk, const double* bsrc,
                                          int use_bsrc, const double* ux, int compute_pi_, const BoxCtx& bc,
                                          FwdFrag& f) {
    const int compute_pi = PRED ? 0 : compute_pi_;
    const int l = lane_id(), g = l >> 4, c = l & 15;
    const double* Fk = io.F + (long)k * FSTRIDE;
    const bool needS = !SH::fixed || compute_pi;
    if constexpr (SH::fixed) {
        f.S[0] = 0.0;
        if (PRED) {
            f.S[1] = f.S[2] = f.S[3] = 0.0;
        } else {
            load_p_fixed<SH::nx>(Fk, f.S, needS);
        }
        f.lc = MODE == 0 ? gld(Fk, FXR_L + c) : 0.0;
        f.invd = 0.0;
        f.kg = gld(Fk, FXR_KG + l);
    } else {
#pragma unroll
        for (int r = 0; r < 4; r++) f.S[r] = gld(Fk, r * 64 + l, needS);
        f.lc = MODE == 0 ? gld(Fk, 256 + c) : 0.0;
        f.invd = gld(Fk, 272 + c);
        f.kg = gld(Fk, 288 + l);
    }
    const int kk = k < io.N ? k : io.N - 1;
    const bool live = k < io.N;
    const double* Bk = stage_B(io, sh);
    const int s = c - sh.xo1;
    const bool ok = live && s >= 0 && s < sh.nx1;
#pragma unroll
    for (int r = 0; r < 4; r++) {
        const int vi = tile_var(g + 4 * r, sh.nu, sh.nx, sh.xo);
        f.bt[r] = ldsel(Bk, lib4_idx(sh.sdB, vi, s), vi >= 0 && ok);
    }
    f.bval = use_bsrc ? ldsel(bsrc + kk * V16, s, ok) : ldsel(Bk, lib4_idx(sh.sdB, sh.nu + sh.nx, s), ok);
    f.hc = 0.0;
    f.pk = 0.0;
    if (MODE == 1) {
        const int vc = tile_var(c, sh.nu, sh.nx, sh.xo);
        f.hc = ldsel(ux + kk * V16, vc, live && vc >= 0);
    }
#pragma unroll
    for (int i = 0; i < 10; i++) f.bx[i] = 0.0;
    if (FM != BX_NONE) {
        const BoxLane b = box_lane(io.tileslot, pnbk, k);
        f.bl = b;
        if (FM == BX_P1) {
            f.bx[0] = ldsel(bc.d, b.lo, b.ok);
            f.bx[1] = ldsel(bc.d, b.up, b.ok);
            f.bx[2] = ldsel(bc.t, b.lo, b.ok);
            f.bx[3] = ldsel(bc.t, b.up, b.ok);
            f.bx[4] = ldsel(bc.lamt, b.lo, b.ok);
            f.bx[5] = ldsel(bc.lamt, b.up, b.ok);
            f.bx[6] = ldsel(bc.lam, b.lo, b.ok);
            f.bx[7] = ldsel(bc.lam, b.up, b.ok);
            f.bx[8] = ldsel(bc.dlam, b.lo, b.ok && !bc.pred);
            f.bx[9] = ldsel(bc.dlam, b.up, b.ok && !bc.pred);
        } else if (FM == BX_P2) {
            fetch_pair(bc.res_d, b, f.bx[0], f.bx[1]);
            fetch_pair(bc.lam, b, f.bx[4], f.bx[5]);
            if (!PRED) fetch_pair(bc.res_m, b, f.bx[6], f.bx[7]);
            fetch_pair(bc.t, b, f.bx[8], f.bx[9]);
        }
    }
}

template <int MODE, int FM, class FX, bool PRED>
__device__ __forceinline__ void fwd_fetch_k(const RicIO& io, int k, const double* bsrc, int use_bsrc,
                                            const double* ux, int compute_pi, const BoxCtx& bc, FwdFrag& f) {
    const int kk = k < io.N ? k : io.N - 1;
    const StageRef sk{io.st, kk};
    const int pnbk = srd(StageRef{io.st, k}, &StageInfo::pnb);
    with_shape<FX>(sk, [&](const auto& sh) {
        fwd_fetch<MODE, FM, PRED>(io, sh, k, pnbk, bsrc, use_bsrc, ux, compute_pi, bc, f);
    });
}

template <int FM, bool PRED>
__device__ __forceinline__ void box_alpha(const BoxCtx& bc, const FwdFrag& f, double x, double& al) {
    if (FM == BX_NONE) return;
    const BoxLane& b = f.bl;
    double dtl, dtu, dll, dlu, lml, lmu, tl, tu;
    if (FM == BX_P1) {
        dtl = x - f.bx[0] - f.bx[2];
        dtu = -x + f.bx[1] - f.bx[3];
        dll = f.bx[8] - (f.bx[4] * dtl + f.bx[6]);
        dlu = f.bx[9] - (f.bx[5] * dtu + f.bx[7]);
        lml = f.bx[6];
        lmu = f.bx[7];
        tl = f.bx[2];
        tu = f.bx[3];
    } else {
        double bx[10];
        use_pair(f.bx[0], f.bx[1], bx[0], bx[1]);
        use_pair(f.bx[4], f.bx[5], bx[4], bx[5]);
        if (!PRED) use_pair(f.bx[6], f.bx[7], bx[6], bx[7]);
        use_pair(f.bx[8], f.bx[9], bx[8], bx[9]);
        const double til = rcp_nr(bx[8]), tiu = rcp_nr(bx[9]);
        const double rml = PRED ? __dmul_rn(bx[4], bx[8]) : bx[6];
        const double rmu = PRED ? __dmul_rn(bx[5], bx[9]) : bx[7];
        dtl = x - bx[0];
        dtu = -x + bx[1];
        dll = -til * (bx[4] * dtl + rml);
        dlu = -tiu * (bx[5] * dtu + rmu);
        lml = bx[4];
        lmu = bx[5];
        tl = bx[8];
        tu = bx[9];
    }
    st_lu(bc.dt, b, dtl, dtu, b.ok);
    st_lu(bc.dlam, b, dll, dlu, b.ok);
    if (b.ok) {
        alpha_rule(al, lml, dll);
        alpha_rule(al, lmu, dlu);
        alpha_rule(al, tl, dtl);
        alpha_rule(al, tu, dtu);
    }
}

template <int MODE>
__device__ __forceinline__ void fwd_pi(int xo, int nx, int k, const d4& S, const double xrow[4], double pc,
                                       int compute_pi, double* pi) {
    const int g = lane_id() >> 4, c = lane_id() & 15;
    const int s = c - xo;
    const bool okp = s >= 0 && s < nx;
    double pv = 0.0;
    if (compute_pi && k > 0) pv = pi_from_x(S, xo, xrow, okp ? pc : 0.0);
    gst(pi, (k - 1) * V16 + s, pv, compute_pi && k > 0 && g == 0 && okp);
}

template <int MODE, int FM, bool PRED, class SH>
__device__ __forceinline__ void fwd_step(const RicIO& io, Scratch* sm, const SH& sh, int k, const FwdFrag& cur,
                                         double& xcol, double* ux, int compute_pi, double* pi, const BoxCtx& bc,
                                         double& al) {
    const int l = lane_id(), g = l >> 4, c = l & 15;
    const bool all = !SH::fixed && k == 0;
    double xrow[4];
    col2row(sm, xcol, xrow);
    if constexpr (!PRED) fwd_pi<MODE>(sh.xo, sh.nx, k, cur.S, xrow, MODE == 0 ? cur.lc : cur.hc, compute_pi, pi);
    const double rhs = (MODE == 0) ? cur.lc : cur.hc;
    double ur[4];
    if constexpr (SH::fixed) {
        const double v = (c < sh.xo) ? rhs : xcol;
        ur[0] = row_sum16(cur.kg * v);
#pragma unroll
        for (int r = 1; r < 4; r++) ur[r] = xrow[r];
        static_assert(SH::xo <= 4, "gain form needs the u block in tile block 0");
    } else {
        double part = 0.0;
        if (!all) {
#pragma unroll
            for (int r = 0; r < 4; r++) part += (g + 4 * r >= sh.xo) ? lowS(cur.S, r, g, c) * xrow[r] : 0.0;
        }
        const double rc = -rhs - xrow_sum(part);
        double rrow[4];
        col2row(sm, rc, rrow);
#pragma unroll
        for (int r = 0; r < 4; r++) ur[r] = all ? 0.0 : xrow[r];
        HK_STAMP(9, k);
        solve_lt(sh, cur.S, cur.invd, rrow, ur, all);
        HK_STAMP(10, k);
    }
    const double ucol = row2col(sm, ur);
    const int vcs = tile_var(c, sh.nu, sh.nx, sh.xo);
    if (!PRED) gst(ux, k * V16 + vcs, ucol, g == 0 && vcs >= 0);
    box_alpha<FM, PRED>(bc, cur, ucol, al);
    if constexpr (!SH::fixed && FM != BX_NONE) {
        if (sh.ng > 0) gen_alpha<FM>(io, sh, k, bc, ucol, al);
    }
    double gp = 0.0;
#pragma unroll
    for (int r = 0; r < 4; r++) gp += cur.bt[r] * ur[r];
    const int s = c - sh.xo1;
    const bool ok = s >= 0 && s < sh.nx1;
    const double x1 = cur.bval + xrow_sum(gp);
    xcol = ok ? x1 : 0.0;
    HK_STAMP(11, k);
}

template <int MODE, int FM, class FX, bool PRED = false>
__device__ void ric_forward(const RicIO& io, Scratch* sm, const double* bsrc, int use_bsrc, double* ux,
                            int compute_pi, double* pi, const BoxCtx& bc, double& al) {
    const int l = lane_id(), g = l >> 4, c = l & 15;
    double xcol = 0.0;
    FwdFrag f0, f1, f2;
    fwd_fetch_k<MODE, FM, FX, PRED>(io, 0, bsrc, use_bsrc, ux, compute_pi, bc, f0);
    fwd_fetch_k<MODE, FM, FX, PRED>(io, 1, bsrc, use_bsrc, ux, compute_pi, bc, f1);
    auto stage = [&](int k, const FwdFrag& fa, const FwdFrag& fb, FwdFrag& fc) __attribute__((always_inline)) {
        (void)fb;
        HK_STAMP(8, k);
        fwd_fetch_k<MODE, FM, FX, PRED>(io, k + 2 <= io.N ? k + 2 : io.N, bsrc, use_bsrc, ux, compute_pi, bc, fc);
        const StageRef si{io.st, k};
        with_shape<FX>(si, [&](const auto& sh) {
            fwd_step<MODE, FM, PRED>(io, sm, sh, k, fa, xcol, ux, compute_pi, pi, bc, al);
        });
        HK_STAMP(12, k);
    };
    auto finish = [&](const FwdFrag& fN) __attribute__((always_inline)) {
        const DynSh sN(StageRef{io.st, io.N});
        const int v = tile_var(c, sN.nu, sN.nx, sN.xo);
        if constexpr (!PRED) {
            double pc = MODE == 0 ? fN.lc : ldsel(ux + io.N * V16, v, compute_pi && v >= 0);
            double xrow[4] = {0.0, 0.0, 0.0, 0.0};
            if (compute_pi) col2row(sm, xcol, xrow);
            fwd_pi<MODE>(sN.xo, sN.nx, io.N, fN.S, xrow, pc, compute_pi, pi);
            gst(ux, io.N * V16 + v, xcol, g == 0 && v >= 0);
        }
        box_alpha<FM, PRED>(bc, fN, xcol, al);
    };
    for (int k = 0;;) {
        if (k >= io.N) { finish(f0); break; }
        stage(k, f0, f1, f2);
        if (++k >= io.N) { finish(f1); break; }
        stage(k, f1, f2, f0);
        if (++k >= io.N) { finish(f2); break; }
        stage(k, f2, f0, f1);
        ++k;
    }
    if (FM != BX_NONE) {
        const DynSh sN(StageRef{io.st, io.N});
        if (sN.ng > 0) gen_alpha<FM>(io, sN, io.N, bc, xcol, al);
    }
}

template <class FX>
__device__ __forceinline__ void ric_forward_sv(const RicIO& io, Scratch* sm, int update_b, const double* bsrc,
                                               double* ux, int compute_pi, double* pi) {
    BoxCtx bc{};
    double al = 1.0;
    ric_forward<0, BX_NONE, FX>(io, sm, bsrc, update_b, ux, compute_pi, pi, bc, al);
}

struct TrsFrag {
    d4 S;
    double invd;
    d4 bop;
    d4 brow;
    double h0;
    double pbc;
    double bx[12];
    BoxLane bl;
};

template <int TM, bool RPB, class SH>
__device__ __forceinline__ void trs_fetch(const RicIO& io, const SH& sh, int k, const double* hb, const double* hq,
                                          const BoxCtx& bc, int compute_Pb_, const double* Pb, TrsFrag& f) {
    const int compute_Pb = RPB ? compute_Pb_ : 0;
    const int l = lane_id(), g = l >> 4, c = l & 15;
    const double* Fk = io.F + (long)k * FSTRIDE;
    if constexpr (SH::fixed) {
        f.S[0] = gld(Fk, FXR_KG + l);
        if (RPB) {
            load_p_fixed<SH::nx>(Fk, f.S, compute_Pb);
        } else {
            f.S[1] = f.S[2] = f.S[3] = 0.0;
        }
        f.invd = 0.0;
    } else {
#pragma unroll
        for (int r = 0; r < 4; r++) f.S[r] = gld(Fk, r * 64 + l);
        f.invd = gld(Fk, 272 + c);
    }
    const int nux = sh.nu + sh.nx;
    const int vc = tile_var(c, sh.nu, sh.nx, sh.xo);
    const double* R = stage_R(io, sh);
    f.h0 = hq ? ldsel(hq + k * V16, vc, vc >= 0) : ldsel(R, lib4_idx(sh.sdR, nux, vc), vc >= 0);
    const BoxLane b = box_lane(io.tileslot, sh.pnb, k);
    f.bl = b;
#pragma unroll
    for (int i = 0; i < 12; i++) f.bx[i] = 0.0;
    if (TM == BX_GIVEN) {
        f.bx[0] = ldsel(bc.qx, b.s16, b.ok);
    } else if (TM == BX_P1) {
        f.bx[0] = ldsel(bc.t_inv, b.lo, b.ok);
        f.bx[1] = ldsel(bc.t_inv, b.up, b.ok);
        f.bx[2] = ldsel(bc.dlam, b.lo, b.ok);
        f.bx[3] = ldsel(bc.dlam, b.up, b.ok);
        f.bx[4] = ldsel(bc.dt, b.lo, b.ok);
        f.bx[5] = ldsel(bc.dt, b.up, b.ok);
        f.bx[6] = ldsel(bc.qxs, b.s16, b.ok);
    } else if (TM == BX_P2) {
        fetch_pair(bc.t, b, f.bx[0], f.bx[1]);
        fetch_pair(bc.dt, b, f.bx[2], f.bx[3]);
        fetch_pair(bc.dlam, b, f.bx[4], f.bx[5]);
        fetch_pair(bc.lam, b, f.bx[8], f.bx[9]);
        fetch_pair(bc.res_d, b, f.bx[10], f.bx[11]);
    }
    const bool live = SH::fixed || k < io.N;
    const double* Bk = stage_B(io, sh);
    const double* bp = hb ? hb + k * V16 : Bk;
#pragma unroll
    for (int r = 0; r < 4; r++) {
        const int sr = g + 4 * r - sh.xo1;
        const bool ok = live && sr >= 0 && sr < sh.nx1;
        f.bop[r] = ldsel(Bk, lib4_idx(sh.sdB, vc, sr), ok && vc >= 0);
        f.brow[r] = RPB ? ldsel(bp, hb ? sr : lib4_idx(sh.sdB, nux, sr), ok && compute_Pb) : 0.0;
    }
    const int s = c - sh.xo1;
    f.pbc = ldsel(Pb + k * V16, s, !compute_Pb && live && s >= 0 && s < sh.nx1);
}

template <int TM>
__device__ __forceinline__ double box_gradient(const BoxCtx& bc, const TrsFrag& f) {
    const int g = lane_id() >> 4;
    const BoxLane& b = f.bl;
    const bool st = b.ok && g == 0;
    if (TM == BX_GIVEN) return f.bx[0];
    if (TM == BX_P1) {
        const double dll = f.bx[0] * (bc.smu - f.bx[2] * f.bx[4]);
        const double dlu = f.bx[1] * (bc.smu - f.bx[3] * f.bx[5]);
        gst(bc.dlam, b.lo, dll, st);
        gst(bc.dlam, b.up, dlu, st);
        return b.ok ? f.bx[6] + (dlu - dll) : 0.0;
    }
    if (TM == BX_P2) {
        double bx[12];
        use_pair(f.bx[0], f.bx[1], bx[0], bx[1]);
        use_pair(f.bx[2], f.bx[3], bx[2], bx[3]);
        use_pair(f.bx[4], f.bx[5], bx[4], bx[5]);
        use_pair(f.bx[8], f.bx[9], bx[8], bx[9]);
        use_pair(f.bx[10], f.bx[11], bx[10], bx[11]);
        const double til = rcp_nr(bx[0]), tiu = rcp_nr(bx[1]);
        const double rml = __dmul_rn(bx[8], bx[0]) + (bx[2] * bx[4] - bc.smu);
        const double rmu = __dmul_rn(bx[9], bx[1]) + (bx[3] * bx[5] - bc.smu);
        st_lu(bc.res_m, b, rml, rmu, b.ok);
        return b.ok ? til * (rml - bx[8] * bx[10]) - tiu * (rmu + bx[9] * bx[11]) : 0.0;
    }
    return 0.0;
}

template <int TM, bool RPB, class SH>
__device__ __forceinline__ void trs_step(const RicIO& io, Scratch* sm, const SH& sh, int k, const TrsFrag& cur,
                                         const BoxCtx& bc, double* ux, int compute_Pb_, double* Pb, d4& S1,
                                         double& pcol) {
    const int compute_Pb = RPB ? compute_Pb_ : 0;
    const int l = lane_id(), g = l >> 4, c = l & 15;
    const int xo1 = sh.xo1, nx1 = sh.nx1;
    const int vc = tile_var(c, sh.nu, sh.nx, sh.xo);
    const int s = c - xo1;
    double pbc = cur.pbc;
    if (compute_Pb) {
        double part = 0.0;
#pragma unroll
        for (int r = 0; r < 4; r++) part += S1[r] * cur.brow[r];
        pbc = xrow_sum(part);
    }
    gst(Pb, k * V16 + s, pbc, compute_Pb && g == 0 && s >= 0 && s < nx1);
    const double wc = (s >= 0 && s < nx1) ? pbc + pcol : 0.0;
    double wrow[4];
    col2row(sm, wc, wrow);
    double part = 0.0;
#pragma unroll
    for (int r = 0; r < 4; r++) part += cur.bop[r] * wrow[r];
    double h = cur.h0 + box_gradient<TM>(bc, cur);
    if constexpr (!SH::fixed) {
        if (sh.ng > 0) h += gen_gradient<TM>(io, sh, k, bc);
    }
    h += xrow_sum(part);
    h = trs_usolve(sh, cur.S, cur.invd, h, !SH::fixed && k == 0);
    gst(ux, k * V16 + vc, h, g == 0 && vc >= 0);
    pcol = h;
    S1 = cur.S;
}

template <int TM, int FM, class FX, bool RPB = true>
__device__ void ric_trs(const RicIO& io, Scratch* sm, const double* hb, const double* hq, const BoxCtx& bc,
                        double* ux, int compute_pi, double* pi, int compute_Pb, double* Pb, double& al) {
    const int l = lane_id(), g = l >> 4, c = l & 15;
    TrsFrag cur;
    with_shape<FX>(StageRef{io.st, io.N}, [&](const auto& sh) { trs_fetch<TM, RPB>(io, sh, io.N, hb, hq, bc, compute_Pb, Pb, cur); });
    double hN = cur.h0 + box_gradient<TM>(bc, cur);
    {
        const DynSh sN(StageRef{io.st, io.N});
        if (sN.ng > 0) hN += gen_gradient<TM>(io, sN, io.N, bc);
        const int v = tile_var(c, sN.nu, sN.nx, sN.xo);
        gst(ux, io.N * V16 + v, hN, g == 0 && v >= 0);
    }
    double pcol = hN;
    d4 S1 = cur.S;
    TrsFrag nxt;
    {
        with_shape<FX>(StageRef{io.st, io.N - 1}, [&](const auto& sh) { trs_fetch<TM, RPB>(io, sh, io.N - 1, hb, hq, bc, compute_Pb, Pb, nxt); });
    }
    auto stage = [&](int k, const TrsFrag& fa, TrsFrag& fb) __attribute__((always_inline)) {
        const int kn = k > 0 ? k - 1 : 0;
        with_shape<FX>(StageRef{io.st, kn}, [&](const auto& sh) { trs_fetch<TM, RPB>(io, sh, kn, hb, hq, bc, compute_Pb, Pb, fb); });
        asm volatile("" ::: "memory");
        const StageRef si{io.st, k};
        with_shape<FX>(si, [&](const auto& sh) { trs_step<TM, RPB>(io, sm, sh, k, fa, bc, ux, compute_Pb, Pb, S1, pcol); });
    };
    for (int k = io.N - 1;;) {
        if (k < 0) break;
        stage(k, nxt, cur);
        if (--k < 0) break;
        stage(k, cur, nxt);
        --k;
    }
    __syncthreads();
    ric_forward<1, FM, FX>(io, sm, hb, hb != nullptr, ux, compute_pi, pi, bc, al);
}

}
```

hpmpc_amd/csrc/hpmpc_capi.cpp:

```cpp
#include <cstdlib>

#include "hk_launch_guard.h"
#include "hk_plan.h"

thread_local int g_err = 0;
thread_local DevCtx g_dev;

extern "C" void hk_set_error(int code, const char* what) {
    g_err = code;
    if (code) fprintf(stderr, "[hpmpc_mi355x] %s (code %d)\n", what, code);
}

int launch(int which, const KArgs* a, int count, hipStream_t s) {
#ifdef HK_RIC2
    if (which == K_SV) {
        const char* e = getenv("HPMPC_MI355X_RIC_WAVES");
        if (e && e[0] == '2') {
            const int r = hk_launch_ric2(which, a, count, s);
            if (r != HK_LAUNCH_REFUSED) return r;
        }
    }
#endif
    return hk_launch(which, a, count, s);
}

bool plan_supported(int N, const int* nx, const int* nu, const int* nb, const int* const* idxb, const int* ng,
                    const char** why) {
    if (LDS_FIXED + (long long)LDS_PER_STAGE * (N + 1) > 160 * 1024) {
        *why = "horizon beyond the LDS stage tables of the tile kernels (N <= 1571)";
        return false;
    }
    for (int k = 0; k <= N; k++) {
        const int u = k < N ? nu[k] : 0;
        if (ng[k] < 0 || rup(nb[k], 4) + rup(ng[k], 4) > 16) {
            *why = "round_up(nb[k],4) + round_up(ng[k],4) must be <= 16 (one 32-slot constraint vector per stage)";
            return false;
        }
        if (u < 0 || nx[k] < 0 || u + nx[k] > 16 || rup(u, 4) + nx[k] > 16) {
            *why = "stage size beyond the 16-wide tile (nu+nx <= 16, round_up(nu,4)+nx <= 16)";
            return false;
        }
        if (nb[k] < 0 || nb[k] > u + nx[k]) {
            *why = "nb[k] > nu[k]+nx[k]";
            return false;
        }
        if (idxb) {
            unsigned seen = 0;
            for (int j = 0; j < nb[k]; j++) {
                const int v = idxb[k][j];
                if (v < 0 || v >= u + nx[k] || (seen >> v & 1u)) {
                    *why = "idxb[k] must hold distinct variable indices in [0, nu[k]+nx[k])";
                    return false;
                }
                seen |= 1u << v;
            }
        }
    }
    if (N < 1) {
        *why = "N must be >= 1";
        return false;
    }
    return true;
}

static const void* plan_stage_table(const hpmpc_mi355x_plan* P, const long long* offB, const long long* offR,
                                    const unsigned char* shB = nullptr, const unsigned char* shR = nullptr) {
    const int N = P->N;
    std::vector<StageInfoH> st = P->st;
    for (int k = 0; k <= N; k++) {
        st[k].oB = k < N ? (int)offB[k] : 0;
        st[k].oR = (int)offR[k];
        st[k].r0 = (P->st[k].r0 & 1) | ((shB && k < N && shB[k]) ? 2 : 0) | ((shR && shR[k]) ? 4 : 0);
    }
    const size_t bytes = sizeof(StageInfoH) * (N + 1);
    if (!memcmp(st.data(), P->st.data(), bytes)) return P->d_st.get();
    std::lock_guard<std::mutex> lock(P->ltabs_mu);
    for (const auto& t : P->ltabs)
        if (!memcmp(st.data(), t.st.data(), bytes)) return t.d.get();
    constexpr size_t kMaxLayouts = 64;
    if (P->ltabs.size() >= kMaxLayouts) {
        hk_set_error(HPMPC_MI355X_EUNSUPPORTED, "more than 64 distinct stage layouts on one plan (create a plan per layout "
                                           "family, or keep the offsets fixed)");
        return nullptr;
    }
    DevTable<StageInfoH> d;
    if (!d.upload(st, "layout stage table")) return nullptr;
    P->ltabs.push_back({std::move(st), std::move(d)});
    return P->ltabs.back().d.get();
}

extern "C" hpmpc_mi355x_plan* hpmpc_mi355x_plan_create(int N, const int* nx, const int* nu, const int* nb,
                                                       const int* const* idxb, const int* ng) {
    const char* why = nullptr;
    if (!plan_supported(N, nx, nu, nb, idxb, ng, &why)) {
        hk_set_error(HPMPC_MI355X_EUNSUPPORTED, why);
        return nullptr;
    }
    auto* P = new hpmpc_mi355x_plan();
    P->N = N;
    P->nx.assign(nx, nx + N + 1);
    P->nu.assign(nu, nu + N + 1);
    P->nu[N] = 0;
    P->nb.assign(nb, nb + N + 1);
    P->ng.assign(ng, ng + N + 1);
    P->idxb.resize(N + 1);
    P->st.resize(N + 1);
    P->tileslot.assign((N + 1) * 16, -1);
    P->slotvar.assign((N + 1) * 16, 0);
    P->offB.resize(N);
    P->offR.resize(N + 1);
    P->offG.resize(N + 1);
    for (int k = 0; k <= N; k++) {
        StageInfoH& s = P->st[k];
        s.nu = P->nu[k];
        s.nx = nx[k];
        s.nb = nb[k];
        s.ng = ng[k];
        s.xo = rup(s.nu, 4);
        s.nx1 = k < N ? nx[k + 1] : 0;
        s.nu1 = k + 1 < N ? P->nu[k + 1] : 0;
        s.xo1 = rup(s.nu1, 4);
        s.sdB = rup(s.nx1, NCL);
        s.sdR = rup(s.nu + s.nx, NCL);
        s.pnb = rup(nb[k], BS);
        s.oD = k * V32;
        s.r0 = 0;
        s.oG = (int)P->packG;
        P->offG[k] = P->packG;
        if (ng[k] > 0) P->packG += (long long)rup(s.nu + s.nx, BS) * rup(ng[k], NCL);
        P->nbt += ng[k];
        P->ngt += ng[k];
        const int nux = s.nu + s.nx;
        if (k < N) {
            P->offB[k] = P->packB;
            P->packB += (long long)rup(nux + 1, BS) * s.sdB;
        }
        P->offR[k] = P->packR;
        P->packR += (long long)rup(nux + 1, BS) * s.sdR;
        if (nb[k] > 0) P->idxb[k].assign(idxb[k], idxb[k] + nb[k]);
        P->nbt += nb[k];
        for (int l = 0; l < nb[k]; l++) {
            const int v = idxb[k][l];
            const int t = v < s.nu ? v : s.xo + (v - s.nu);
            P->tileslot[k * 16 + t] = (signed char)l;
            P->slotvar[k * 16 + l] = (signed char)v;
        }
    }
    if (N >= 3) {
        const int nuc = P->nu[1], nxc = nx[1];
        P->fixcls = hk_fixcls(nuc, nxc);
        if (P->fixcls)
            for (int k = 1; k <= N - 2; k++)
                P->st[k].r0 = (P->nu[k] == nuc && nx[k] == nxc && P->nu[k + 1] == nuc && nx[k + 1] == nxc &&
                               ng[k] == 0)
                                  ? 1
                                  : 0;
    }
    for (int k = 0; k <= N; k++) {
        P->st[k].oB = k < N ? (int)P->offB[k] : 0;
        P->st[k].oR = (int)P->offR[k];
    }
    if (!P->d_st.upload(P->st, "plan tables") || !P->d_tileslot.upload(P->tileslot, "plan tables") ||
        !P->d_slotvar.upload(P->slotvar, "plan tables")) {
        delete P;
        return nullptr;
    }
    g_err = 0;
    return P;
}

extern "C" void hpmpc_mi355x_plan_destroy(hpmpc_mi355x_plan* P) { delete P; }

void idxb_table(int N, const int* nb, const int* const* idxb, int* out) {
    for (int k = 0; k <= N; k++)
        for (int l = 0; l < nb[k]; l++) out[k * 16 + l] = idxb[k][l];
}

extern "C" long long hpmpc_mi355x_ws_doubles(const hpmpc_mi355x_plan* P) { return P ? ws_doubles(P->N) : 0; }

extern "C" int hpmpc_mi355x_last_error(void) { return g_err; }

static unsigned long long* g_dbg_buf = nullptr;
#ifdef HK_STAMPS
extern "C" __attribute__((visibility("default"))) void hpmpc_mi355x_debug_buffer(void* dev_ptr) {
    g_dbg_buf = (unsigned long long*)dev_ptr;
}
#endif

extern "C" const char* hpmpc_mi355x_version(void) {
    return "hpmpc_mi355x 0.1 gfx950 (wave-per-problem, f64 MFMA 16x16x4 stage contractions)";
}

bool range_ok(const void* plan, int nprob, int p0, int count, const char* who) {
    if (plan && nprob > 0 && p0 >= 0 && count >= 0 && (long long)p0 + count <= nprob) return true;
    char msg[128];
    snprintf(msg, sizeof msg, "%s: plan or problem range", who);
    hk_set_error(HPMPC_MI355X_EUNSUPPORTED, msg);
    return false;
}

int null_array(const char* who) {
    char msg[128];
    snprintf(msg, sizeof msg, "%s: a required array is null", who);
    hk_set_error(HPMPC_MI355X_EUNSUPPORTED, msg);
    return g_err;
}

int launch_error(int e, const char* what) {
    hk_set_error(e == HK_LAUNCH_REFUSED ? HPMPC_MI355X_EUNSUPPORTED : HPMPC_MI355X_EHIP, what);
    return g_err;
}

bool batch_args(KArgs& a, const hpmpc_mi355x_plan* P, const hpmpc_mi355x_layout* lay, int nprob, int p0,
                DctPolicy policy, const double* DCt) {
    if (!P) {
        g_err = HPMPC_MI355X_EUNSUPPORTED;
        return false;
    }
    if (policy == DCT_NONE && P->ngt) {
        hk_set_error(HPMPC_MI355X_EUNSUPPORTED, "batched entry points: general constraints (ng > 0) need the "
                                           "reference-named entry points");
        return false;
    }
    memset(&a, 0, sizeof a);
    a.N = P->N;
    a.nprob = nprob;
    a.p0 = p0;
    a.st = P->d_st.get();
    a.tileslot = P->d_tileslot.get();
    a.slotvar = P->d_slotvar.get();
    if (lay && lay->BAbt_off && lay->RSQrq_off) {
        a.st = plan_stage_table(P, lay->BAbt_off, lay->RSQrq_off, lay->BAbt_shared, lay->RSQrq_shared);
        if (!a.st) return false;
    }
    a.sB = lay ? lay->BAbt_stride : P->packB;
    a.sR = lay ? lay->RSQrq_stride : P->packR;
    a.DCt = P->ngt ? DCt : nullptr;
    a.sV16 = (long long)(P->N + 1) * V16;
    a.sV32 = (long long)(P->N + 1) * V32;
    a.sW = ws_doubles(P->N);
    a.fixcls = P->fixcls;
    a.nbt = P->nbt;
    a.ngt = P->ngt;
    a.sG = P->packG;
    a.dbg = g_dbg_buf;
    return true;
}

hpmpc_mi355x_plan* thread_plan(int N, const int* nx, const int* nu, const int* nb, int** idxb, const int* ng) {
    struct Cache {
        hpmpc_mi355x_plan* plan = nullptr;
        std::vector<int> key;
        ~Cache() {
            if (plan) hpmpc_mi355x_plan_destroy(plan);
        }
    };
    thread_local Cache c;
    std::vector<int> k;
    k.push_back(N);
    for (int i = 0; i <= N; i++) {
        k.push_back(nx[i]);
        k.push_back(i < N ? nu[i] : 0);
        k.push_back(nb[i]);
        k.push_back(ng[i]);
        for (int l = 0; l < nb[i]; l++) k.push_back(idxb[i][l]);
    }
    if (c.plan && k == c.key) return c.plan;
    if (c.plan) hpmpc_mi355x_plan_destroy(c.plan);
    c.plan = hpmpc_mi355x_plan_create(N, nx, nu, nb, idxb, ng);
    c.key = c.plan ? k : std::vector<int>();
    return c.plan;
}

int ipm_run(KArgs& a, int count, const double* BAbt, const double* RSQrq, const double* d, double* ux, double* pi,
            double* lam, double* t, double* ws, int k_max, double mu0, double mu_tol, double alpha_min, int warm_start,
            int compute_mult, int* kk, int* ret, double* stat, int which, void* stream) {
    a.BAbt = BAbt;
    a.RSQ = RSQrq;
    a.d = d;
    a.ux = ux;
    a.pi = pi;
    a.lam = lam;
    a.t = t;
    a.ws = ws;
    a.k_max = k_max;
    a.mu0 = mu0;
    a.mu_tol = mu_tol;
    a.alpha_min = alpha_min;
    a.warm_start = warm_start;
    a.compute_mult = compute_mult;
    a.kk = kk;
    a.ret = ret;
    a.stat = stat;
    if (const int e = hk_launch(which, &a, count, (hipStream_t)stream)) return launch_error(e, "hk_ipm launch failed");
    return g_err = 0;
}

namespace {

int ipm_launch(const hpmpc_mi355x_plan* plan, const hpmpc_mi355x_layout* lay, int nprob, int p0, int count,
               const double* BAbt, const double* RSQrq, const double* d, double* ux, double* pi, double* lam,
               double* t, double* ws, int k_max, double mu0, double mu_tol, double alpha_min, int warm_start,
               int compute_mult, int* kk, int* ret, double* stat, int which, void* stream) {
    KArgs a;
    if (!batch_args(a, plan, lay, nprob, p0, DCT_NONE)) return g_err;
    return ipm_run(a, count, BAbt, RSQrq, d, ux, pi, lam, t, ws, k_max, mu0, mu_tol, alpha_min, warm_start,
                   compute_mult, kk, ret, stat, which, stream);
}

struct CallEvents {
    std::vector<hipEvent_t> e;
    bool create(int n) {
        e.reserve(n);
        for (int i = 0; i < n; i++) {
            hipEvent_t x;
            if (!hip_ok(hipEventCreate(&x), "event create")) return false;
            e.push_back(x);
        }
        return true;
    }
    hipEvent_t& operator[](size_t i) { return e[i]; }
    ~CallEvents() {
        for (hipEvent_t x : e) {
            (void)hipEventSynchronize(x);
            (void)hipEventDestroy(x);
        }
    }
};

}

extern "C" int hpmpc_mi355x_ipm_batch(const hpmpc_mi355x_plan* plan, const hpmpc_mi355x_layout* lay, int nprob,
                                      int p0, int count, const double* BAbt, const double* RSQrq, const double* d,
                                      double* ux, double* pi, double* lam, double* t, double* ws, int k_max,
                                      double mu0, double mu_tol, double alpha_min, int warm_start, int compute_mult,
                                      int* kk, int* ret, double* stat, void* stream) {
    return ipm_launch(plan, lay, nprob, p0, count, BAbt, RSQrq, d, ux, pi, lam, t, ws, k_max, mu0, mu_tol, alpha_min,
                      warm_start, compute_mult, kk, ret, stat, K_IPM, stream);
}

extern "C" int hpmpc_mi355x_ipm_solo(const hpmpc_mi355x_plan* plan, const hpmpc_mi355x_layout* lay, int nprob, int p0,
                                     int count, const double* BAbt, const double* RSQrq, const double* d, double* ux,
                                     double* pi, double* lam, double* t, double* ws, int k_max, double mu0,
                                     double mu_tol, double alpha_min, int warm_start, int compute_mult, int* kk,
                                     int* ret, double* stat, void* stream) {
    return ipm_launch(plan, lay, nprob, p0, count, BAbt, RSQrq, d, ux, pi, lam, t, ws, k_max, mu0, mu_tol, alpha_min,
                      warm_start, compute_mult, kk, ret, stat, K_SOLO, stream);
}

extern "C" int hpmpc_mi355x_ipm_batch_profiled(const hpmpc_mi355x_plan* plan, const hpmpc_mi355x_layout* lay,
                                               int nprob, int p0, int count, const double* BAbt, const double* RSQrq,
                                               const double* d, double* ux, double* pi, double* lam, double* t,
                                               double* ws, int k_max, double mu0, double mu_tol, double alpha_min,
                                               int warm_start, int compute_mult, int* kk, int* ret, double* stat,
                                               double* pass_ms, void* stream) {
    const int npass = 1 + 4 * (k_max > 0 ? k_max : 0);
    CallEvents ev;
    if (!ev.create(2 * npass)) return g_err;
    hipStream_t st = (hipStream_t)stream;
    for (int i = 0; i < npass; i++) {
        const int which = i == 0 ? K_PASS_INIT : K_PASS_FACT + (i - 1) % 4;
        if (!hip_ok(hipEventRecord(ev[2 * i], st), "event record")) return g_err;
        int rc = ipm_launch(plan, lay, nprob, p0, count, BAbt, RSQrq, d, ux, pi, lam, t, ws, k_max, mu0, mu_tol,
                            alpha_min, warm_start, compute_mult, kk, ret, stat, which, stream);
        if (rc) return rc;
        if (!hip_ok(hipEventRecord(ev[2 * i + 1], st), "event record")) return g_err;
    }
    if (!hip_ok(hipStreamSynchronize(st), "sync")) return g_err;
    for (int p = 0; p < 5; p++) pass_ms[p] = 0.0;
    for (int i = 0; i < npass; i++) {
        float ms = 0.f;
        if (!hip_ok(hipEventElapsedTime(&ms, ev[2 * i], ev[2 * i + 1]), "event time")) return g_err;
        pass_ms[i == 0 ? 0 : 1 + (i - 1) % 4] += ms;
    }
    return g_err = 0;
}

extern "C" int hpmpc_mi355x_ipm_pass(const hpmpc_mi355x_plan* plan, const hpmpc_mi355x_layout* lay, int nprob,
                                     int p0, int count, const double* BAbt, const double* RSQrq, const double* d,
                                     double* ux, double* pi, double* lam, double* t, double* ws, int k_max,
                                     double mu0, double mu_tol, double alpha_min, int warm_start, int compute_mult,
                                     int* kk, int* ret, double* stat, int pass, void* stream) {
    if (pass < 0 || pass > 4) return g_err = HPMPC_MI355X_EUNSUPPORTED;
    return ipm_launch(plan, lay, nprob, p0, count, BAbt, RSQrq, d, ux, pi, lam, t, ws, k_max, mu0, mu_tol, alpha_min,
                      warm_start, compute_mult, kk, ret, stat, K_PASS_INIT + pass, stream);
}

extern "C" int hpmpc_mi355x_ric_sv_batch(const hpmpc_mi355x_plan* plan, const hpmpc_mi355x_layout* lay, int nprob,
                                         int p0, int count, const double* BAbt, const double* RSQrq, double* ux,
                                         double* pi, double* ws, int compute_pi, int compute_Pb, double* Pb,
                                         void* stream) {
    KArgs a;
    if (!batch_args(a, plan, lay, nprob, p0, DCT_NONE)) return g_err;
    a.BAbt = BAbt;
    a.RSQ = RSQrq;
    a.ux = ux;
    a.pi = pi;
    a.ws = ws;
    a.compute_pi = compute_pi;
    a.compute_Pb = compute_Pb && Pb;
    a.vPb = Pb;
    if (const int e = launch(K_SV, &a, count, (hipStream_t)stream)) return launch_error(e, "hk_ric_sv launch failed");
    return g_err = 0;
}

extern "C" int hpmpc_mi355x_ric_trf_batch(const hpmpc_mi355x_plan* plan, const hpmpc_mi355x_layout* lay, int nprob,
                                          int p0, int count, const double* BAbt, const double* RSQrq, double* ws,
                                          void* stream) {
    KArgs a;
    if (!batch_args(a, plan, lay, nprob, p0, DCT_NONE)) return g_err;
    a.BAbt = BAbt;
    a.RSQ = RSQrq;
    a.ws = ws;
    if (const int e = hk_launch(K_TRF, &a, count, (hipStream_t)stream))
        return launch_error(e, "hk_ric_trf launch failed");
    return g_err = 0;
}

extern "C" int hpmpc_mi355x_ric_trs_batch(const hpmpc_mi355x_plan* plan, const hpmpc_mi355x_layout* lay, int nprob,
                                          int p0, int count, const double* BAbt, const double* RSQrq, const double* b,
                                          const double* q, double* ux, double* pi, double* ws, int compute_pi,
                                          int compute_Pb, double* Pb, void* stream) {
    KArgs a;
    if (!batch_args(a, plan, lay, nprob, p0, DCT_NONE)) return g_err;
    a.BAbt = BAbt;
    a.RSQ = RSQrq;
    a.vb = b;
    a.vq = q;
    a.ux = ux;
    a.pi = pi;
    a.ws = ws;
    a.compute_pi = compute_pi;
    a.compute_Pb = compute_Pb;
    a.vPb = Pb;
    if (const int e = hk_launch(K_TRS, &a, count, (hipStream_t)stream))
        return launch_error(e, "hk_ric_trs launch failed");
    return g_err = 0;
}
```

hpmpc_amd/csrc/hpmpc_kargs.h:

```cpp
#pragma once

constexpr int FSTRIDE = 352;
constexpr int V16 = 16;
constexpr int V32 = 32;
constexpr int LDS_FIXED = 256;
constexpr int LDS_PER_STAGE = 104;

enum HkLaunch {
    K_SV = 0,
    K_TRF = 1,
    K_TRS = 2,
    K_RES = 3,
    K_IPM = 4,
    K_KKT = 5,
    K_KKT_P1 = 6,
    K_PASS_INIT = 10,
    K_PASS_FACT = 11,
    K_PASS_PRED = 12,
    K_PASS_CORR = 13,
    K_PASS_UPDATE = 14,
    K_SOLO = 15,
    K_SOLO_1W = 16,
    K_QDRAIN = 17,
    K_PASS_PREDCORR = 18,
};
static_assert(K_PASS_FACT == K_PASS_INIT + 1 && K_PASS_PRED == K_PASS_INIT + 2 && K_PASS_CORR == K_PASS_INIT + 3 &&
                  K_PASS_UPDATE == K_PASS_INIT + 4,
              "the pass ids are consecutive: the host computes them as K_PASS_INIT + pass and K_PASS_FACT + i % 4");

struct KArgs {
    int N, nprob, p0;
    int nbt;
    int ngt;
    int fixcls;
    const void* st;
    const signed char* tileslot;
    const signed char* slotvar;
    const double* BAbt;
    long long sB;
    const double* RSQ;
    long long sR;
    const double* d;
    const double* DCt;
    long long sG;
    double* ws;
    long long sW;
    double *ux, *pi;
    double *lam, *t;
    long long sV16, sV32;
    const double *vb, *vq, *vQx, *vqx;
    double* vPb;
    int update_b, update_q, use_box, compute_pi, compute_Pb;
    int k_max, warm_start, compute_mult, single_newton;
    int phase1_only;
    int res_plain;
    double mu0, mu_tol, alpha_min;
    int *kk, *ret;
    double* stat;
    double* mu_out;
    int nq;
    int* qctl;
    unsigned long long* dbg;
    int nslots;
    int no_bkp;
    int qpar;
    int* dctr;
    int* qnext;
};
```

hpmpc_amd/csrc/hpmpc_kernels.hip:

```cpp
#include "hk_ipm_body.h"
#include "hk_kkt_body.h"
#include "hk_launch.h"
#include "hk_mw.h"
#include <cstdlib>

template <class FX>
__global__ __launch_bounds__(64) void hk_ric_sv(KArgs a) {
    const LdsTabs T = lds_tables(a);
    Scratch& sm = *T.sm;
    const int p = blockIdx.x + a.p0;
    if (p >= a.nprob) return;
    double* F = a.ws + (long)p * a.sW;
    RicIO io = make_io(a, T, p, F);
    const long o16 = (long)p * a.sV16;
    const double* b = a.vb ? a.vb + o16 : nullptr;
    const double* q = a.vq ? a.vq + o16 : nullptr;
    BoxCtx bc{};
    bc.Qx = a.vQx ? a.vQx + o16 : nullptr;
    bc.qx = a.vqx ? a.vqx + o16 : nullptr;
    double* Pb = a.vPb ? a.vPb + o16 : nullptr;
#ifdef HK_STAMPS
    const unsigned long long t0 = mw_clock();
#endif
    if (a.use_box)
        ric_backward<true, BX_GIVEN, FX, CERT_LOAD>(io, &sm, a.update_b, b, a.update_q, q, bc, a.compute_Pb, Pb);
    else
        ric_backward<true, BX_NONE, FX, CERT_LOAD>(io, &sm, a.update_b, b, a.update_q, q, bc, a.compute_Pb, Pb);
    wsync();
#ifdef HK_STAMPS
    const unsigned long long t1 = mw_clock();
#endif
    ric_forward_sv<FX>(io, &sm, a.update_b, b, a.ux + o16, a.compute_pi, a.pi + o16);
#ifdef HK_STAMPS
    const unsigned long long t2 = mw_clock();
    if (a.dbg && p == 0 && lane_id() == 0) {
        a.dbg[60] = t1 - t0;
        a.dbg[61] = t2 - t1;
    }
#endif
}

template <class FX>
__global__ __launch_bounds__(64) void hk_ric_trf(KArgs a) {
    const LdsTabs T = lds_tables(a);
    Scratch& sm = *T.sm;
    const int p = blockIdx.x + a.p0;
    if (p >= a.nprob) return;
    double* F = a.ws + (long)p * a.sW;
    RicIO io = make_io(a, T, p, F);
    const long o16 = (long)p * a.sV16;
    BoxCtx bc{};
    bc.Qx = a.vQx ? a.vQx + o16 : nullptr;
    if (a.use_box)
        ric_backward<false, BX_GIVEN, FX, CERT_LOAD>(io, &sm, 0, nullptr, 0, nullptr, bc, 0, nullptr);
    else
        ric_backward<false, BX_NONE, FX, CERT_LOAD>(io, &sm, 0, nullptr, 0, nullptr, bc, 0, nullptr);
}

template <class FX>
__global__ __launch_bounds__(64) void hk_ric_trs(KArgs a) {
    const LdsTabs T = lds_tables(a);
    Scratch& sm = *T.sm;
    const int p = blockIdx.x + a.p0;
    if (p >= a.nprob) return;
    double* F = a.ws + (long)p * a.sW;
    RicIO io = make_io(a, T, p, F);
    const long o16 = (long)p * a.sV16;
    BoxCtx bc{};
    bc.qx = a.vqx ? a.vqx + o16 : nullptr;
    double al = 1.0;
    if (a.use_box)
        ric_trs<BX_GIVEN, BX_NONE, FX>(io, &sm, a.vb + o16, a.vq + o16, bc, a.ux + o16, a.compute_pi, a.pi + o16,
                                   a.compute_Pb, a.vPb + o16, al);
    else
        ric_trs<BX_NONE, BX_NONE, FX>(io, &sm, a.vb + o16, a.vq + o16, bc, a.ux + o16, a.compute_pi, a.pi + o16,
                                  a.compute_Pb, a.vPb + o16, al);
}

template <class FX>
__global__ __launch_bounds__(64) void hk_res(KArgs a) {
    const LdsTabs T = lds_tables(a);
    const int p = blockIdx.x + a.p0;
    if (p >= a.nprob) return;
    RicIO io = make_io(a, T, p, nullptr);
    const long o16 = (long)p * a.sV16, o32 = (long)p * a.sV32;
    double* out = a.ws + (long)p * a.sW;
    const long n1 = a.N + 1;
    BoxCtx bc{};
    bc.d = a.d + o32;
    bc.lam = a.lam + o32;
    bc.t = a.t + o32;
    ResIO ro{};
    ro.bsrc = a.vb ? a.vb + o16 : nullptr;
    ro.qsrc = a.vq ? a.vq + o16 : nullptr;
    ro.ux = a.ux + o16;
    ro.pi = a.pi + o16;
    ro.rq = out;
    ro.rb = out + n1 * V16;
    ro.rd = out + 2 * n1 * V16;
    ro.rm = out + 2 * n1 * V16 + n1 * V32;
    double mu = 0.0;
    const bool have = residual_pass<false, FX>(io, bc, ro, mu);
    if (a.res_plain) {
        wsync();
        HK_FOR_BOX(io, k, { ro.rd[up] = -ro.rd[up]; });
        HK_FOR_GEN(io, k, { ro.rd[up] = -ro.rd[up]; });
        if (lane_id() == 0) a.mu_out[p] = have ? mu : 0.0;
        return;
    }
    if (lane_id() == 0 && have) a.mu_out[p] = mu;
}

template <class FX>
__global__ __launch_bounds__(64) HK_TWO_WAVES void hk_ipm_init(KArgs a) {
    const LdsTabs T = lds_tables(a);
    if (a.nq) {
        if (ipm_refill<FX, 7, true>(a, T, blockIdx.x)) qlist_push(a, a.qpar, blockIdx.x);
        return;
    }
    Who who;
    if (!who_am_i(a, who)) return;
    IpmView v = ipm_view(a, T, who);
    ipm_start<FX, 7, true>(a, T, v);
}


template <class FX>
__global__ __launch_bounds__(64) HK_TWO_WAVES void hk_ipm_fact(KArgs a) {
    if (a.nq && blockIdx.x == 0 && lane_id() == 0) *qcount(a, a.qpar ^ 1) = 0;
    Who who;
    if (!who_am_i(a, who) || !slot_active(a, who)) return;
    const LdsTabs T = lds_tables(a);
    IpmView v = ipm_view(a, T, who);
    if (v.w.state[S_ACTIVE] == 0.0) return;
    fact_body<FX>(a, T, v);
}

template <class FX>
__global__ __launch_bounds__(64) HK_TWO_WAVES void hk_ipm_pred(KArgs a) {
    Who who;
    if (!who_am_i(a, who) || !slot_active(a, who)) return;
    const LdsTabs T = lds_tables(a);
    IpmView v = ipm_view(a, T, who);
    if (v.w.state[S_ACTIVE] == 0.0) return;
    pred_body<FX>(a, T, v);
}

template <class FX>
__global__ __launch_bounds__(64) HK_TWO_WAVES void hk_ipm_corr(KArgs a) {
    Who who;
    if (!who_am_i(a, who) || !slot_active(a, who)) return;
    const LdsTabs T = lds_tables(a);
    IpmView v = ipm_view(a, T, who);
    if (v.w.state[S_ACTIVE] == 0.0) return;
    corr_body<FX>(a, T, v);
}

template <class FX>
__global__ __launch_bounds__(64) HK_TWO_WAVES void hk_ipm_predcorr(KArgs a) {
    Who who;
    if (!who_am_i(a, who) || !slot_active(a, who)) return;
    const LdsTabs T = lds_tables(a);
    {
        IpmView v = ipm_view(a, T, who);
        if (v.w.state[S_ACTIVE] == 0.0) return;
        pred_body<FX>(a, T, v);
    }
    wsync();
    int s = who.s, q = who.q, d = who.d;
    asm volatile("" : "+v"(s), "+v"(q), "+v"(d));
    const Who w2{__builtin_amdgcn_readfirstlane(s), __builtin_amdgcn_readfirstlane(q), __builtin_amdgcn_readfirstlane(d)};
    IpmView v = ipm_view(a, T, w2);
    corr_body<FX>(a, T, v);
}

template <class FX>
__global__ __launch_bounds__(64) HK_TWO_WAVES void hk_ipm_update(KArgs a) {
    Who who;
    if (!who_am_i(a, who) || !slot_active(a, who)) return;
    const LdsTabs T = lds_tables(a);
    IpmView v = ipm_view(a, T, who);
    if (v.w.state[S_ACTIVE] == 0.0) return;
    bool again = update_body<FX, 4>(a, v);
    if (!again && a.nq) {
        if (v.l == 0) atomicAdd(&a.qctl[1], 1);
        again = ipm_refill<FX, 4, false>(a, T, who.s);
    }
    if (a.nq && again) qlist_push(a, a.qpar ^ 1, who.s);
}

template <class FX>
__global__ __launch_bounds__(64) void hk_ipm_solo(KArgs a) {
    const LdsTabs T = lds_tables(a);
    const int p = blockIdx.x + a.p0;
    if (p >= a.nprob) return;
    if (carve(a.ws + (long)p * a.sW, a.N).state[S_ACTIVE] == 0.0) return;
    auto view = [&]() __attribute__((always_inline)) {
        int q = p;
        asm volatile("" : "+v"(q));
        q = __builtin_amdgcn_readfirstlane(q);
        const Who w{q, q, q};
        return ipm_view(a, T, w);
    };
    for (int it = 0; it < a.k_max; it++) {
        wsync();
        {
            IpmView v = view();
            fact_body<FX>(a, T, v);
        }
        wsync();
        {
            IpmView v = view();
            pred_body<FX>(a, T, v);
        }
        wsync();
        {
            IpmView v = view();
            corr_body<FX>(a, T, v);
        }
        wsync();
        IpmView v = view();
        if (!update_body<FX, 4>(a, v)) break;
    }
}

namespace {

template <class FX>
__device__ __forceinline__ void fact_body_mw(const KArgs& a, IpmView& v, int& tb, int w) {
    const double* st = v.w.state;
    const bool sn = a.single_newton != 0;
    v.bc.cert_new = st[S_KK] == 0.0;
    if (st[S_PHASE] == 1.0)
        tb = ric_backward_mw<true, BX_P1, FX>(v.io, tb, w, 0, nullptr, 0, nullptr, v.bc, 1, v.w.Pb);
    else {
        v.bc.res_rhs = !sn;
        v.bc.no_tinv = a.no_bkp;
        tb = ric_backward_mw<true, BX_P2R, FX>(v.io, tb, w, 0, nullptr, 0, nullptr, v.bc, 1, v.w.Pb);
    }
}

template <class FX>
__device__ __forceinline__ void pred_body_mw(const KArgs& a, IpmView& v, int& tb, int w) {
    double* st = v.w.state;
    const bool sn = a.single_newton != 0;
    const int phase = (int)st[S_PHASE], kk = (int)st[S_KK];
    const double mu = st[S_MU];
    double sigma = st[S_SIGMA];
    double al = 1.0;
    if (phase == 1) {
        v.bc.pred = 1;
        tb = ric_forward_mw<0, BX_P1, FX, true>(v.io, tb, w, nullptr, 0, v.w.dux, 0, v.w.dpi, v.bc, al);
    } else {
        tb = ric_forward_mw<0, BX_P2, FX, true>(v.io, tb, w, v.w.res_b, !sn, v.w.dux, 0, v.w.dpi, v.bc, al);
    }
    const double alpha = al * 0.995;
    double mu_aff;
    {
        const RicIO io = v.io;
        const BoxCtx bc = v.bc;
        mu_aff = mu_aff_pass<7>(io, bc, alpha, st[S_MUSCAL]);
    }
    double smu = a.mu0;
    if (!sn) {
        sigma = mu_aff / mu;
        sigma = sigma * sigma * sigma;
        smu = sigma * mu;
    }
    __syncthreads();
    if (v.l == 0) {
        v.stat[5 * kk] = st[S_SIGMA];
        v.stat[5 * kk + 1] = al;
        v.stat[5 * kk + 2] = mu_aff;
        st[S_SIGMA] = sigma;
        st[S_SMU] = smu;
    }
}

template <class FX>
__device__ __forceinline__ void corr_body_mw(const KArgs& a, IpmView& v, int& tb, int w) {
    double* st = v.w.state;
    const int phase = (int)st[S_PHASE], kk = (int)st[S_KK];
    v.bc.smu = st[S_SMU];
    double al = 1.0;
    if (phase == 1)
        tb = ric_trs_mw<BX_P1, BX_P1, FX>(v.io, tb, w, nullptr, nullptr, v.bc, v.w.dux, a.compute_mult, v.w.dpi,
                                     v.w.Pb, al);
    else
        tb = ric_trs_mw<BX_P2, BX_P2, FX>(v.io, tb, w, v.w.res_b, v.w.res_q, v.bc, v.w.dux, a.compute_mult, v.w.dpi,
                                     v.w.Pb, al);
    if (v.l == 0) {
        v.stat[5 * kk] = st[S_SIGMA];
        v.stat[5 * kk + 3] = al;
        st[S_ALPHA] = al * 0.995;
    }
}

template <class FX, int CI>
__device__ __forceinline__ bool update_body_mw(const KArgs& a, const IpmView& v0, const MwSplit& mws0) {
    IpmView v = v0;
    const MwSplit mws = mws0;
    double* st = v.w.state;
    const int phase = (int)st[S_PHASE];
    int kk = (int)st[S_KK];
    const double alpha = st[S_ALPHA];
    const double sigma = st[S_SIGMA];
    double mu;
    if (phase == 1) {
        mu = update_p1_pass<CI, MW_WAVES>(v.io, v.bc, alpha, st[S_MUSCAL], v.ux, v.pi, v.w.dux, v.w.dpi, v.w.ux_bkp,
                                          v.w.pi_bkp, v.w.lam_bkp, v.w.t_bkp, mws);
    } else {
        if (a.no_bkp)
            mu = update_p2_pass<CI, true, false, MW_WAVES>(v.io, v.bc, v.bt.slotvar, alpha, st[S_MUSCAL], v.ux, v.pi,
                                                           v.w.dux, v.w.dpi, v.w.ux_bkp, v.w.pi_bkp, v.w.lam_bkp,
                                                           v.w.t_bkp, v.w.res_d, v.w.res_m, mws);
        else
            mu = update_p2_pass<CI, true, true, MW_WAVES>(v.io, v.bc, v.bt.slotvar, alpha, st[S_MUSCAL], v.ux, v.pi,
                                                          v.w.dux, v.w.dpi, v.w.ux_bkp, v.w.pi_bkp, v.w.lam_bkp,
                                                          v.w.t_bkp, v.w.res_d, v.w.res_m, mws);
    }
    wsync();
    if (v.l == 0) v.stat[5 * kk + 4] = mu;
    kk++;
    return ipm_continue<FX, CI, MW_WAVES>(a, v, kk, mu, alpha, sigma, phase, mws);
}

}

template <class FX>
__device__ __forceinline__ void mw_solve(const KArgs& a, const LdsTabs& T, const Who& who) {
    const int p = who.q;
    const int w = threadIdx.x >> 6;
    if (threadIdx.x < MW_D) {
        hk_mw.full[threadIdx.x] = 0;
        hk_mw.freed[threadIdx.x] = 0;
        hk_mw.freedB[threadIdx.x] = 0;
    }
    if (threadIdx.x < MW_DP) {
        hk_mw.fullP[threadIdx.x] = 0;
        hk_mw.freedP[threadIdx.x] = 0;
    }
    if (threadIdx.x == 0) hk_mw.err = 0;
    __syncthreads();
    int tb = 0;
    const MwSplit mws{w, (lds_f64*)&hk_mw.red[0][0]};
#ifdef HK_STAMPS
    unsigned long long tph[4] = {0, 0, 0, 0}, tm = 0;
    if (threadIdx.x < MW_WAVES) hk_mw.wait_cyc[threadIdx.x] = hk_mw.seg[threadIdx.x] = 0;
#define HK_MW_PHASE(i)                            \
    do {                                          \
        const unsigned long long t_ = mw_clock(); \
        if (i >= 0) tph[(i) & 3] += t_ - tm;      \
        tm = t_;                                  \
    } while (0)
#else
#define HK_MW_PHASE(i) \
    do {               \
    } while (0)
#endif
    for (int it = 0; it < a.k_max; it++) {
        __syncthreads();
        HK_MW_PHASE(-1);
        {
            IpmView v = ipm_view(a, T, who);
            v.l = threadIdx.x;
            fact_body_mw<FX>(a, v, tb, w);
        }
        __syncthreads();
        HK_MW_PHASE(0);
        {
            IpmView v = ipm_view(a, T, who);
            v.l = threadIdx.x;
            pred_body_mw<FX>(a, v, tb, w);
        }
        __syncthreads();
        HK_MW_PHASE(1);
        {
            IpmView v = ipm_view(a, T, who);
            v.l = threadIdx.x;
            corr_body_mw<FX>(a, v, tb, w);
        }
        __syncthreads();
        HK_MW_PHASE(2);
        IpmView v = ipm_view(a, T, who);
        v.l = threadIdx.x;
        const bool again = update_body_mw<FX, 4>(a, v, mws);
        __syncthreads();
        HK_MW_PHASE(3);
        if (!again || __atomic_load_n(&hk_mw.err, __ATOMIC_RELAXED)) break;
    }
#ifdef HK_STAMPS
    if (a.dbg && p == 0 && threadIdx.x == 0) {
        for (int i = 0; i < 4; i++) a.dbg[32 + i] = tph[i];
        for (int i = 0; i < MW_WAVES; i++) a.dbg[40 + i] = hk_mw.wait_cyc[i];
        for (int i = 0; i < 4; i++) a.dbg[48 + i] = hk_mw.seg[i];
    }
#endif
#undef HK_MW_PHASE
    if (threadIdx.x == 0 && hk_mw.err) {
        a.ret[p] = HK_MW_ERR;
        for (int i = 0; i < 4; i++) a.stat[(long)p * 5 * a.k_max + i] = hk_mw.dbg[i];
    }
}

template <class FX>
__global__ __launch_bounds__(256) void hk_ipm_solo_mw(KArgs a) {
    const LdsTabs T = lds_tables(a);
    const int p = blockIdx.x + a.p0;
    if (p >= a.nprob) return;
    if (carve(a.ws + (long)p * a.sW, a.N).state[S_ACTIVE] == 0.0) return;
    mw_solve<FX>(a, T, Who{p, p, p});
}

template <class FX>
__global__ __launch_bounds__(256) void hk_ipm_qdrain_mw(KArgs a) {
    const LdsTabs T = lds_tables(a);
    const int n = __builtin_amdgcn_readfirstlane(*qcount(a, a.qpar));
    if ((int)blockIdx.x >= n) return;
    const int s = __builtin_amdgcn_readfirstlane(qlist(a, a.qpar)[blockIdx.x]);
    const int q = __builtin_amdgcn_readfirstlane(a.qctl[2 + s]);
    const double* st = carve(a.ws + (long)s * a.sW, a.N).state;
    if (q < 0 || st[S_ACTIVE] == 0.0) return;
    const int kk0 = (int)st[S_KK];
    __syncthreads();
    mw_solve<FX>(a, T, Who{s, q, q % a.nprob});
    __syncthreads();
    if (threadIdx.x == 0) {
        a.qctl[2 + s] = -1;
        atomicAdd(&a.dctr[0], a.kk[q] - kk0);
        atomicAdd(&a.dctr[1], 1);
        atomicAdd(&a.qctl[1], 1);
    }
}

template <class FX>
__global__ __launch_bounds__(64) void hk_kkt_new_rhs(KArgs a) {
    const LdsTabs T = lds_tables(a);
    Scratch& sm = *T.sm;
    const int p = blockIdx.x + a.p0;
    if (p >= a.nprob) return;
    const int N = a.N;
    Ws w = carve(a.ws + (long)p * a.sW, N);
    RicIO io = make_io(a, T, p, w.F);
    BoxTab bt{T.tileslot, T.slotvar};
    const long o16 = (long)p * a.sV16, o32 = (long)p * a.sV32;
    double* ux = a.ux + o16;
    double* pi = a.pi + o16;
    double* lam = a.lam + o32;
    double* t = a.t + o32;
    const double* dv = a.d + o32;
    const KktIO v{a.vb, a.vq, o16, dv, ux, pi, lam, t};
    kkt_body<FX, false>(a, io, &sm, bt, w, v);
}

template <class FX>
__global__ __launch_bounds__(64) void hk_kkt_new_rhs_p1(KArgs a) {
    const LdsTabs T = lds_tables(a);
    Scratch& sm = *T.sm;
    const int p = blockIdx.x + a.p0;
    if (p >= a.nprob) return;
    const int N = a.N;
    Ws w = carve(a.ws + (long)p * a.sW, N);
    RicIO io = make_io(a, T, p, w.F);
    BoxTab bt{T.tileslot, T.slotvar};
    const long o16 = (long)p * a.sV16, o32 = (long)p * a.sV32;
    double* ux = a.ux + o16;
    double* pi = a.pi + o16;
    double* lam = a.lam + o32;
    double* t = a.t + o32;
    const double* rC = a.d + o32;
    const int l = lane_id();
    BoxCtx bc = box_ctx(w, rC, lam, t);
    HK_FOR_BOX(io, k, { w.qx[k * V16 + slot] = -w.lamt[up] * rC[up] - w.lamt[lo] * rC[lo]; });
    HK_FOR_GEN(io, k, { w.qx[s16] = -w.lamt[up] * rC[up] - w.lamt[lo] * rC[lo]; });
    wsync();
    double al = 1.0;
// ... 118 lines not shown
```

include/hpmpc_mi355x.h:

```cpp
#ifndef HPMPC_MI355X_H_
#define HPMPC_MI355X_H_

#ifdef __cplusplus
extern "C" {
#endif

#define HPMPC_MI355X_EUNSUPPORTED (-10)
#define HPMPC_MI355X_EHIP (-11)
#define HPMPC_MI355X_EMW (-20)
#define HPMPC_MI355X_QUEUE_LANES_MAX 4
#define HPMPC_MI355X_QUEUE_CTL_INTS(n_slots) (6 * HPMPC_MI355X_QUEUE_LANES_MAX + 2 + 3 * (n_slots))


int d_back_ric_rec_sv_tv_work_space_size_bytes(int N, int *nx, int *nu, int *nb, int *ng);
int d_back_ric_rec_sv_tv_memory_space_size_bytes(int N, int *nx, int *nu, int *nb, int *ng);
void d_back_ric_rec_sv_tv_res(int N, int *nx, int *nu, int *nb, int **idxb, int *ng, int update_b, double **hpBAbt,
                              double **b, int update_q, double **hpQ, double **q, double **bd, double **hpDCt,
                              double **Qx, double **qx, double **hux, int compute_pi, double **hpi, int compute_Pb,
                              double **hPb, double *memory, double *work);
void d_back_ric_rec_trf_tv_res(int N, int *nx, int *nu, int *nb, int **idxb, int *ng, double **hpBAbt, double **hpQ,
                               double **hpDCt, double **Qx, double **bd, double *memory, double *work);
void d_back_ric_rec_trs_tv_res(int N, int *nx, int *nu, int *nb, int **idxb, int *ng, double **hpBAbt, double **hb,
                               double **hq, double **hpDCt, double **qx, double **hux, int compute_pi, double **hpi,
                               int compute_Pb, double **hPb, double *memory, double *work);

int d_ip2_res_mpc_hard_tv_work_space_size_bytes(int N, int *nx, int *nu, int *nb, int *ng);
int d_ip2_res_mpc_hard_tv(int *kk, int k_max, double mu0, double mu_tol, double alpha_min, int warm_start,
                          double *stat, int N, int *nx, int *nu_N, int *nb, int **idxb, int *ng, double **pBAbt,
                          double **pQ, double **pDCt, double **d, double **ux, int compute_mult, double **pi,
                          double **lam, double **t, double *double_work_memory);
int d_ip2_res_mpc_hard_tv_single_newton_step(int *kk, int k_max, double mu0, double mu_tol, double alpha_min,
                                             int warm_start, double *stat, int N, int *nx, int *nu_N, int *nb,
                                             int **idxb, int *ng, double **pBAbt, double **pQ, double **pDCt,
                                             double **d, double **ux, int compute_mult, double **pi, double **lam,
                                             double **t, double *double_work_memory, double **ux0, double **pi0,
                                             double **lam0, double **t0);
void d_kkt_solve_new_rhs_res_mpc_hard_tv(int N, int *nx, int *nu_N, int *nb, int **idxb, int *ng, double **pBAbt,
                                         double **b, double **pQ, double **q, double **pDCt, double **d,
                                         double **ux, int compute_mult, double **pi, double **lam, double **t,
                                         double *double_work_memory);
void d_res_res_mpc_hard_tv(int N, int *nx, int *nu, int *nb, int **idxb, int *ng, double **hpBAbt, double **hb,
                           double **hpQ, double **hq, double **hux, double **hpDCt, double **hd, double **hpi,
                           double **hlam, double **ht, double *work, double **hrq, double **hrb, double **hrd,
                           double **hrm, double *mu);

int d_ip2_mpc_hard_tv_work_space_size_bytes(int N, int *nx, int *nu, int *nb, int *ng);
int d_ip2_mpc_hard_tv(int *kk, int k_max, double mu0, double mu_tol, double alpha_min, int warm_start, double *stat,
                      int N, int *nx, int *nu, int *nb, int **idxb, int *ng, double **pBAbt, double **pQ,
                      double **pDCt, double **d, double **ux, int compute_mult, double **pi, double **lam, double **t,
                      double *double_work_memory);
void d_kkt_solve_new_rhs_mpc_hard_tv(int N, int *nx, int *nu_N, int *nb, int **idxb, int *ng, double **pBAbt,
                                     double **r_A, double **pQ, double **r_H, double **pDCt, double **r_C,
                                     double **ux, int compute_mult, double **pi, double **lam, double **t,
                                     double *double_work_memory);
int d_ip2_mpc_soft_tv_work_space_size_bytes(int N, int *nx, int *nu, int *nb, int *ng, int *ns);
int d_ip2_mpc_soft_tv(int *kk, int k_max, double mu0, double mu_tol, double alpha_min, int warm_start, double *stat,
                      int N, int *nx, int *nu, int *nb, int **idxb, int *ng, int *ns, double **pBAbt, double **pQ,
                      double **Z, double **z, double **pDCt, double **d, double **ux, int compute_mult, double **pi,
                      double **lam, double **t, double *double_work_memory);
void d_res_mpc_soft_tv(int N, int *nx, int *nu, int *nb, int **idxb, int *ng, int *ns, double **hpBAbt, double **hpQ,
                       double **hq, double **hZ, double **hz, double **hux, double **hpDCt, double **hd, double **hpi,
                       double **hlam, double **ht, double **hrq, double **hrb, double **hrd, double **hrz, double *mu);
void d_res_mpc_hard_tv(int N, int *nx, int *nu, int *nb, int **idxb, int *ng, double **hpBAbt, double **hb,
                       double **hpQ, double **hq, double **hux, double **hpDCt, double **hd, double **hpi,
                       double **hlam, double **ht, double **hrq, double **hrb, double **hrd, double *mu);

void d_cond_BAbt(int N, int *nx, int *nu, double **hpBAbt, double *work, double **hpGamma, double *pBAbt2);
void d_cond_RSQrq(int N, int *nx, int *nu, double **hpBAbt, double **hpRSQrq, double **hpGamma, double *work,
                  double *pRSQrq2);
void d_cond_DCtd(int N, int *nx, int *nu, int *nb, int **hidxb, double **hd, double **hpGamma, double *pDCt2,
                 double *d2, int *idxb2);
void d_part_cond_compute_problem_size(int N, int *nx, int *nu, int *nb, int **hidxb, int *ng, int N2, int *nx2,
                                      int *nu2, int *nb2, int *ng2);
int d_part_cond_work_space_size_bytes(int N, int *nx, int *nu, int *nb, int **hidxb, int *ng, int N2, int *nx2,
                                      int *nu2, int *nb2, int *ng2);
int d_part_cond_memory_space_size_bytes(int N, int *nx, int *nu, int *nb, int **hidxb, int *ng, int N2, int *nx2,
                                        int *nu2, int *nb2, int *ng2);
void d_part_cond(int N, int *nx, int *nu, int *nb, int **hidxb, int *ng, double **hpBAbt, double **hpRSQrq,
                 double **hpDCt, double **hd, int N2, int *nx2, int *nu2, int *nb2, int **hidxb2, int *ng2,
                 double **hpBAbt2, double **hpRSQrq2, double **hpDCt2, double **hd2, void *memory, void *work);
int d_part_expand_work_space_size_bytes(int N, int *nx, int *nu, int *nb, int *ng);
void d_part_expand_solution(int N, int *nx, int *nu, int *nb, int **hidxb, int *ng, double **hpBAbt, double **hb,
                            double **hpRSQrq, double **hrq, double **hpDCt, double **hux, double **hpi,
                            double **hlam, double **ht, int N2, int *nx2, int *nu2, int *nb2, int **hidxb2,
                            int *ng2, double **hux2, double **hpi2, double **hlam2, double **ht2, void *work);

int hpmpc_d_ip_ocp_hard_tv_work_space_size_bytes(int N, int *nx, int *nu, int *nb, int **hidxb, int *ng, int N2);
int hpmpc_d_ip_ocp_hard_tv_work_space_size_bytes_noidxb(int N, int *nx, int *nu, int *nb, int *nbx, int *nbu, int *ng, int N2);
int fortran_order_d_ip_ocp_hard_tv_single_newton_step(int *kk, int k_max, double mu0, double mu_tol, int N, int *nx, int *nu_N, int *nb, int **hidxb, int *ng, int N2, int warm_start, double **A, double **B, double **b, double **Q, double **S, double **R, double **q, double **r, double **lb, double **ub, double **C, double **D, double **lg, double **ug, double **x, double **u, double **pi, double **lam, double **t, double *inf_norm_res, void *work0, double *stat, double **ux0, double **pi0, double **lam0, double **t0);
int hpmpc_d_ip_ocp_soft_tv_work_space_size_bytes(int N, int *nx, int *nu, int *nb, int **hidxb, int *ng, int *ns);
int fortran_order_d_ip_ocp_soft_tv(int *kk, int k_max, double mu0, double mu_tol, int N, int *nx, int *nu_N, int *nb,
                                   int **hidxb, int *ng, int *ns, int warm_start, double **A, double **B, double **b,
                                   double **Q, double **S, double **R, double **q, double **r, double **Z, double **z,
                                   double **lb, double **ub, double **C, double **D, double **lg, double **ug,
                                   double **x, double **u, double **pi, double **lam, double *inf_norm_res,
                                   void *work0, double *stat);
int c_order_d_ip_ocp_hard_tv(int *kk, int k_max, double mu0, double mu_tol, int N, int *nx, int *nu, int *nb,
                             int **hidxb, int *ng, int N2, int warm_start, double **A, double **B, double **b,
                             double **Q, double **S, double **R, double **q, double **r, double **lb, double **ub,
                             double **C, double **D, double **lg, double **ug, double **x, double **u, double **pi,
                             double **lam, double *inf_norm_res, void *work0, double *stat);
void c_order_d_solve_kkt_new_rhs_ocp_hard_tv(int N, int *nx, int *nu, int *nb, int **hidxb, int *ng, double **A,
                                             double **B, double **b, double **Q, double **S, double **R, double **q,
                                             double **r, double **lb, double **ub, double **C, double **D, double **lg,
                                             double **ug, double **x, double **u, double **pi, double **lam,
                                             double *inf_norm_res, double *work0);
int fortran_order_d_ip_ocp_hard_tv(int *kk, int k_max, double mu0, double mu_tol, int N, int *nx, int *nu, int *nb,
                                   int **hidxb, int *ng, int N2, int warm_start, double **A, double **B, double **b,
                                   double **Q, double **S, double **R, double **q, double **r, double **lb,
                                   double **ub, double **C, double **D, double **lg, double **ug, double **x,
                                   double **u, double **pi, double **lam, double *inf_norm_res, void *work0,
                                   double *stat);
void fortran_order_d_solve_kkt_new_rhs_ocp_hard_tv(int N, int *nx, int *nu, int *nb, int **hidxb, int *ng,
                                                   double **A, double **B, double **b, double **Q, double **S,
                                                   double **R, double **q, double **r, double **lb, double **ub,
                                                   double **C, double **D, double **lg, double **ug, double **x,
                                                   double **u, double **pi, double **lam, double *inf_norm_res,
                                                   double *work0);

int hpmpc_d_ip_mpc_hard_tv_work_space_size_doubles(int N, int nx, int nu, int nb, int ng, int ngN);
int c_order_d_ip_mpc_hard_tv(int *kk, int k_max, double mu0, double mu_tol, int N, int nx, int nu, int nb, int ng,
                             int ngN, int time_invariant, int free_x0, int warm_start, double *A, double *B,
                             double *b, double *Q, double *Qf, double *S, double *R, double *q, double *qf, double *r,
                             double *lb, double *ub, double *C, double *D, double *lg, double *ug, double *Cf,
                             double *lgf, double *ugf, double *x, double *u, double *pi, double *lam, double *t,
                             double *inf_norm_res, double *work0, double *stat);
void c_order_d_solve_kkt_new_rhs_mpc_hard_tv(int N, int nx, int nu, int nb, int ng, int ngN, int time_invariant,
                                             int free_x0, double *A, double *B, double *b, double *Q, double *Qf,
                                             double *S, double *R, double *q, double *qf, double *r, double *lb,
                                             double *ub, double *C, double *D, double *lg, double *ug, double *Cf,
                                             double *lgf, double *ugf, double *x, double *u, double *pi, double *lam,
                                             double *t, double *inf_norm_res, double *work0);
int fortran_order_d_ip_mpc_hard_tv(int *kk, int k_max, double mu0, double mu_tol, int N, int nx, int nu, int nb,
                                   int ng, int ngN, int time_invariant, int free_x0, int warm_start, double *A,
                                   double *B, double *b, double *Q, double *Qf, double *S, double *R, double *q,
                                   double *qf, double *r, double *lb, double *ub, double *C, double *D, double *lg,
                                   double *ug, double *Cf, double *lgf, double *ugf, double *x, double *u, double *pi,
                                   double *lam, double *t, double *inf_norm_res, double *work0, double *stat);
void fortran_order_d_solve_kkt_new_rhs_mpc_hard_tv(int N, int nx, int nu, int nb, int ng, int ngN, int time_invariant,
                                                   int free_x0, double *A, double *B, double *b, double *Q, double *Qf,
                                                   double *S, double *R, double *q, double *qf, double *r, double *lb,
                                                   double *ub, double *C, double *D, double *lg, double *ug,
                                                   double *Cf, double *lgf, double *ugf, double *x, double *u,
                                                   double *pi, double *lam, double *t, double *inf_norm_res,
                                                   double *work0);


typedef struct hpmpc_mi355x_plan hpmpc_mi355x_plan;

hpmpc_mi355x_plan *hpmpc_mi355x_plan_create(int N, const int *nx, const int *nu, const int *nb,
                                            const int *const *idxb, const int *ng);
void hpmpc_mi355x_plan_destroy(hpmpc_mi355x_plan *plan);

typedef struct {
    long long BAbt_stride;
    long long RSQrq_stride;
    const long long *BAbt_off;
    const long long *RSQrq_off;
    const unsigned char *BAbt_shared;
    const unsigned char *RSQrq_shared;
} hpmpc_mi355x_layout;

long long hpmpc_mi355x_ws_doubles(const hpmpc_mi355x_plan *plan);

int hpmpc_mi355x_ipm_batch(const hpmpc_mi355x_plan *plan, const hpmpc_mi355x_layout *lay, int nprob, int p0,
                           int count, const double *BAbt, const double *RSQrq, const double *d, double *ux, double *pi,
                           double *lam, double *t, double *ws, int k_max, double mu0, double mu_tol, double alpha_min,
                           int warm_start, int compute_mult, int *kk, int *ret, double *stat, void *stream);

int hpmpc_mi355x_ipm_solo(const hpmpc_mi355x_plan *plan, const hpmpc_mi355x_layout *lay, int nprob, int p0, int count,
                          const double *BAbt, const double *RSQrq, const double *d, double *ux, double *pi,
                          double *lam, double *t, double *ws, int k_max, double mu0, double mu_tol, double alpha_min,
                          int warm_start, int compute_mult, int *kk, int *ret, double *stat, void *stream);

int hpmpc_mi355x_ipm_pass(const hpmpc_mi355x_plan *plan, const hpmpc_mi355x_layout *lay, int nprob, int p0,
                          int count, const double *BAbt, const double *RSQrq, const double *d, double *ux, double *pi,
                          double *lam, double *t, double *ws, int k_max, double mu0, double mu_tol, double alpha_min,
                          int warm_start, int compute_mult, int *kk, int *ret, double *stat, int pass, void *stream);

int hpmpc_mi355x_ipm_batch_profiled(const hpmpc_mi355x_plan *plan, const hpmpc_mi355x_layout *lay, int nprob,
                                    int p0, int count, const double *BAbt, const double *RSQrq, const double *d,
                                    double *ux, double *pi, double *lam, double *t, double *ws, int k_max, double mu0,
                                    double mu_tol, double alpha_min, int warm_start, int compute_mult, int *kk,
                                    int *ret, double *stat, double *pass_ms, void *stream);

int hpmpc_mi355x_ipm_queue(const hpmpc_mi355x_plan *plan, const hpmpc_mi355x_layout *lay, int nprob, int nq,
                           int n_slots, const double *BAbt, const double *RSQrq, const double *d, double *ux,
                           double *pi, double *lam, double *t, double *ws, int *qctl, int k_max, double mu0,
                           double mu_tol, double alpha_min, int warm_start, int compute_mult, int *kk, int *ret,
                           double *stat, double *pass_ms, int *n_ticks, void *stream);

int hpmpc_mi355x_ric_sv_batch(const hpmpc_mi355x_plan *plan, const hpmpc_mi355x_layout *lay, int nprob, int p0,
                              int count, const double *BAbt, const double *RSQrq, double *ux, double *pi, double *ws,
                              int compute_pi, int compute_Pb, double *Pb, void *stream);

int hpmpc_mi355x_ric_trf_batch(const hpmpc_mi355x_plan *plan, const hpmpc_mi355x_layout *lay, int nprob, int p0,
                               int count, const double *BAbt, const double *RSQrq, double *ws, void *stream);

int hpmpc_mi355x_ric_trs_batch(const hpmpc_mi355x_plan *plan, const hpmpc_mi355x_layout *lay, int nprob, int p0,
                               int count, const double *BAbt, const double *RSQrq, const double *b, const double *q,
                               double *ux, double *pi, double *ws, int compute_pi, int compute_Pb, double *Pb,
                               void *stream);

int hpmpc_mi355x_last_error(void);
const char *hpmpc_mi355x_version(void);


typedef struct hpmpc_mi355x_pcond_plan hpmpc_mi355x_pcond_plan;
hpmpc_mi355x_pcond_plan *hpmpc_mi355x_pcond_plan_create(int N, const int *nx, const int *nu, const int *nb,
                                                        const int *const *idxb, const int *ng, int N2);
void hpmpc_mi355x_pcond_plan_destroy(hpmpc_mi355x_pcond_plan *plan);
int hpmpc_mi355x_pcond_sizes(const hpmpc_mi355x_pcond_plan *plan, long long *out);
int hpmpc_mi355x_pcond_offsets(const hpmpc_mi355x_pcond_plan *plan, int which, long long *out);
int hpmpc_mi355x_pcond_batch(const hpmpc_mi355x_pcond_plan *plan, int nprob, int p0, int count, const double *BAbt,
                             const double *RSQrq, const double *d, double *G, double *BAbt2, double *RSQrq2,
                             double *DCt2, double *d2, void *stream);
int hpmpc_mi355x_pcond_ric_sv_batch(const hpmpc_mi355x_pcond_plan *plan, int nprob, int p0, int count,
                                    const double *BAbt2, const double *RSQrq2, double *ws, double *ux2, double *pi2,
                                    int compute_pi, void *stream);
int hpmpc_mi355x_pexpand_batch(const hpmpc_mi355x_pcond_plan *plan, int nprob, int p0, int count, const double *BAbt,
                               const double *RSQrq, const double *ux2, const double *pi2, const double *lam2,
                               const double *t2, double *ux, double *pi, double *lam, double *t, void *stream);

typedef struct hpmpc_mi355x_wide_plan hpmpc_mi355x_wide_plan;
hpmpc_mi355x_wide_plan *hpmpc_mi355x_wide_plan_create(int N, const int *nx, const int *nu, const int *nb,
                                                      const int *const *idxb, const int *ng);
void hpmpc_mi355x_wide_plan_destroy(hpmpc_mi355x_wide_plan *plan);
int hpmpc_mi355x_wide_sizes(const hpmpc_mi355x_wide_plan *plan, long long *out);
int hpmpc_mi355x_wide_offsets(const hpmpc_mi355x_wide_plan *plan, long long *out);
int hpmpc_mi355x_wide_ipm_batch(const hpmpc_mi355x_wide_plan *plan, int nprob, int p0, int count, const double *BAbt,
                                const double *RSQrq, const double *DCt, const double *d, double *ux, double *pi,
                                double *lam, double *t, double *work, int k_max, double mu0, double mu_tol,
                                double alpha_min, int warm_start, int compute_mult, int *kk, int *ret, double *stat,
                                void *stream);
const hpmpc_mi355x_wide_plan *hpmpc_mi355x_pcond_wide_plan(const hpmpc_mi355x_pcond_plan *plan);

typedef struct hpmpc_mi355x_soft_plan hpmpc_mi355x_soft_plan;
hpmpc_mi355x_soft_plan *hpmpc_mi355x_soft_plan_create(int N, const int *nx, const int *nu, const int *nb,
                                                      const int *const *idxb, const int *ng, const int *ns);
void hpmpc_mi355x_soft_plan_destroy(hpmpc_mi355x_soft_plan *plan);
int hpmpc_mi355x_soft_sizes(const hpmpc_mi355x_soft_plan *plan, long long *out);
int hpmpc_mi355x_soft_offsets(const hpmpc_mi355x_soft_plan *plan, long long *out);
int hpmpc_mi355x_ipm_soft_batch(const hpmpc_mi355x_soft_plan *plan, const hpmpc_mi355x_layout *lay, int nprob,
                                int p0, int count, const double *BAbt, const double *RSQrq, const double *Z,
                                const double *z, const double *d, double *ux, double *pi, double *lam, double *t,
                                double *ws, int k_max, double mu0, double mu_tol, double alpha_min, int warm_start,
                                int compute_mult, int *kk, int *ret, double *stat, void *stream);

typedef struct hpmpc_mi355x_ocp_plan hpmpc_mi355x_ocp_plan;
enum {
    HPMPC_MI355X_OCP_A, HPMPC_MI355X_OCP_B, HPMPC_MI355X_OCP_b, HPMPC_MI355X_OCP_Q, HPMPC_MI355X_OCP_S,
    HPMPC_MI355X_OCP_R, HPMPC_MI355X_OCP_q, HPMPC_MI355X_OCP_r, HPMPC_MI355X_OCP_lb, HPMPC_MI355X_OCP_ub,
    HPMPC_MI355X_OCP_C, HPMPC_MI355X_OCP_D, HPMPC_MI355X_OCP_lg, HPMPC_MI355X_OCP_ug, HPMPC_MI355X_OCP_NARRAYS
};
typedef struct {
    const double *ptr[HPMPC_MI355X_OCP_NARRAYS];
    long long stride[HPMPC_MI355X_OCP_NARRAYS];
} hpmpc_mi355x_ocp_data;
hpmpc_mi355x_ocp_plan *hpmpc_mi355x_ocp_plan_create(int N, const int *nx, const int *nu, const int *nb,
                                                    const int *const *idxb, const int *ng, int row_major);
void hpmpc_mi355x_ocp_plan_destroy(hpmpc_mi355x_ocp_plan *plan);
const hpmpc_mi355x_plan *hpmpc_mi355x_ocp_tile_plan(const hpmpc_mi355x_ocp_plan *plan);
#define HPMPC_MI355X_OCP_NSIZES 29
int hpmpc_mi355x_ocp_sizes(const hpmpc_mi355x_ocp_plan *plan, long long *out);
#define HPMPC_MI355X_OCP_NOFFSETS 18
int hpmpc_mi355x_ocp_offsets(const hpmpc_mi355x_ocp_plan *plan, long long *out);
int hpmpc_mi355x_ocp_pack_batch(const hpmpc_mi355x_ocp_plan *plan, const hpmpc_mi355x_ocp_data *data, int matrices,
                                int nprob, int p0, int count, double *BAbt, double *RSQrq, double *DCt, double *d,
                                const double *u0, const double *x0, double *ux, void *stream);
int hpmpc_mi355x_ocp_ipm_batch(const hpmpc_mi355x_ocp_plan *plan, int nprob, int p0, int count, const double *BAbt,
                               const double *RSQrq, const double *DCt, const double *d, double *ux, double *pi,
                               double *lam, double *t, double *ws, int k_max, double mu0, double mu_tol,
                               double alpha_min, int warm_start, int compute_mult, int *kk, int *ret, double *stat,
                               void *stream);
int hpmpc_mi355x_ocp_finish_batch(const hpmpc_mi355x_ocp_plan *plan, int nprob, int p0, int count, const double *BAbt,
                                  const double *RSQrq, const double *DCt, const double *d, const double *ux,
                                  const double *pi, const double *lam, const double *t, double *res, double *u,
                                  double *x, double *pi_out, double *lam_out, double *t_out, double *inf_norm_res,
                                  void *stream);

long long hpmpc_mi355x_kkt_scratch_doubles(const hpmpc_mi355x_plan *plan);
int hpmpc_mi355x_kkt_new_rhs_batch(const hpmpc_mi355x_plan *plan, const hpmpc_mi355x_layout *lay, int nprob, int p0,
                                   int count, int nrhs, const double *BAbt, const double *RSQrq, const double *DCt,
                                   const double *b, const double *q, const double *d, double *ux, double *pi,
                                   double *lam, double *t, const double *ws, double *scratch, int compute_mult,
                                   void *stream);
int hpmpc_mi355x_ocp_kkt_batch(const hpmpc_mi355x_ocp_plan *plan, int nprob, int p0, int count, const double *BAbt,
                               const double *RSQrq, const double *DCt, const double *d, double *ux, double *pi,
                               double *lam, double *t, const double *ws, double *scratch, void *stream);
int hpmpc_mi355x_ocp_unpack_sets(const hpmpc_mi355x_ocp_plan *plan, int nprob, int p0, int count, int nrhs,
                                 const double *d, const double *ux, const double *pi, const double *lam,
                                 const double *t, double *u, double *x, double *pi_out, double *lam_out,
                                 double *t_out, void *stream);

int hpmpc_mi355x_kkt_tangent_batch(const hpmpc_mi355x_plan *plan, const hpmpc_mi355x_layout *lay, int nprob, int p0,
                                   int count, int ndir, const double *BAbt, const double *RSQrq, const double *DCt,
                                   const double *db, const double *dq, const double *dd, double *dux, double *dpi,
                                   double *dlam, double *dt, const double *ws, double *scratch, int compute_mult,
                                   void *stream);
int hpmpc_mi355x_ocp_tangent_batch(const hpmpc_mi355x_ocp_plan *plan, const hpmpc_mi355x_ocp_data *dirs, int nprob,
                                   int p0, int count, int ndir, const double *BAbt, const double *RSQrq,
                                   const double *DCt, double *du, double *dx, double *dpi, double *dlam, double *dt,
                                   const double *ws, double *scratch, int compute_mult, void *stream);

int hpmpc_mi355x_kkt_adjoint_batch(const hpmpc_mi355x_plan *plan, const hpmpc_mi355x_layout *lay, int nprob, int p0,
                                   int count, int nadj, const double *BAbt, const double *RSQrq, const double *DCt,
                                   const double *gux, const double *gpi, const double *glam, const double *gt,
                                   double *bbar, double *qbar, double *dbar, const double *ws, double *scratch,
                                   void *stream);
int hpmpc_mi355x_ocp_adjoint_batch(const hpmpc_mi355x_ocp_plan *plan, int nprob, int p0, int count, int nadj,
                                   const double *BAbt, const double *RSQrq, const double *DCt, const double *gu,
                                   const double *gx, const double *gpi, const double *glam, const double *gt,
                                   double *gb, double *gq, double *gr, double *glb, double *gub, double *glg,
                                   double *gug, const double *ws, double *scratch, void *stream);

typedef struct {
    double *ptr[HPMPC_MI355X_OCP_NARRAYS];
    long long stride[HPMPC_MI355X_OCP_NARRAYS];
} hpmpc_mi355x_ocp_grads;
int hpmpc_mi355x_ocp_matrix_grads_batch(const hpmpc_mi355x_ocp_plan *plan, int nprob, int p0, int count, int nadj,
                                        const double *ux, const double *pi, const double *lam, const double *bbar,
                                        const double *qbar, const double *dbar, const hpmpc_mi355x_ocp_grads *grads,
                                        void *stream);
int hpmpc_mi355x_ocp_adjoint_data_batch(const hpmpc_mi355x_ocp_plan *plan, int nprob, int p0, int count, int nadj,
                                        const double *BAbt, const double *RSQrq, const double *DCt, const double *ux,
                                        const double *pi, const double *lam, const double *gu, const double *gx,
                                        const double *gpi, const double *glam, const double *gt,
                                        const hpmpc_mi355x_ocp_grads *grads, const double *ws, double *scratch,
                                        void *stream);

int hpmpc_mi355x_ocp_matrix_dirs_batch(const hpmpc_mi355x_ocp_plan *plan, const hpmpc_mi355x_ocp_data *dirs, int nprob,
                                       int p0, int count, int ndir, const double *ux, const double *pi,
                                       const double *lam, double *db, double *dq, double *dd, void *stream);
int hpmpc_mi355x_ocp_tangent_data_batch(const hpmpc_mi355x_ocp_plan *plan, const hpmpc_mi355x_ocp_data *dirs, int nprob,
                                        int p0, int count, int ndir, const double *BAbt, const double *RSQrq,
                                        const double *DCt, const double *ux, const double *pi, const double *lam,
                                        double *du, double *dx, double *dpi, double *dlam, double *dt, const double *ws,
                                        double *scratch, int compute_mult, void *stream);

#ifdef __cplusplus
}
#endif
#endif
```

Before: 2.149 million.

## Add uniform stage-run fast path to Riccati backward recursion

On the host, finds the longest run of consecutive stages that share the same shape, box count and tile slots and have constant offset strides. The run is passed to the kernels in KArgs. Inside that run, the backward factorisation steps pointers by a fixed delta instead of reading per-stage table entries, which removes table loads and address computation from the recursion's critical path. By default this path is on only in the fact kernel; the predictor and corrector solves keep it behind a compile flag. It adds extra code paths and template instantiations, which may raise register pressure.

```diff
diff --git a/hpmpc_amd/bindings.py b/hpmpc_amd/bindings.py
--- a/hpmpc_amd/bindings.py
+++ b/hpmpc_amd/bindings.py
@@ -12,6 +12,7 @@
 _SIG = dict(
     plan_create="p:ippppp",
     plan_destroy="v:p",
+    stage_run="i:ippppppp",
     ws_doubles="l:p",
     ipm_batch="i:ppiiippppppppidddiipppp",
     ipm_solo="i:ppiiippppppppidddiipppp",
diff --git a/hpmpc_amd/build.py b/hpmpc_amd/build.py
--- a/hpmpc_amd/build.py
+++ b/hpmpc_amd/build.py
@@ -95,6 +95,31 @@
     return build_hip(force=force, verbose=verbose, variant="ric2", extra=["-DHK_RIC2"], sources=["hk_ric2.hip"])
 
 
+def build_norun(verbose: bool = False, force: bool = False) -> str:
+    build_hip(verbose=verbose)
+    objdir = os.path.join(ROOT, "build", "obj_norun")
+    os.makedirs(objdir, exist_ok=True)
+    os.makedirs(os.path.join(LIBDIR, "ab"), exist_ok=True)
+    out = os.path.join(LIBDIR, "ab", "libnorun.so")
+    src = "hpmpc_capi.cpp"
+    hdrs_all = [os.path.join(CSRC, h) for h in HEADERS] + [os.path.join(ROOT, "include", "hpmpc_mi355x.h")]
+    obj = os.path.join(objdir, src + ".o")
+    if force or not _newer(obj, [os.path.join(CSRC, src)] + _deps(src, hdrs_all)):
+        cmd = [HIPCC, f"--offload-arch={ARCH}", "-O3", "-std=c++17", "-fPIC", "-fvisibility=hidden", "-Wall",
+               "-Wno-unused-function", "-DHK_NO_RUN"] + KFLAGS + ["-c", os.path.join(CSRC, src), "-o", obj]
+        if verbose:
+            print(" ".join(cmd), flush=True)
+        subprocess.run(cmd, check=True)
+    objs = [obj if s == src else os.path.join(ROOT, "build", "obj", s + ".o") for s in SOURCES]
+    if force or not _newer(out, objs + [EXPORTS]):
+        cmd = [HIPCC, f"--offload-arch={ARCH}", "-shared", "-fPIC", f"-Wl,--version-script={EXPORTS}"] + objs + \
+              ["-o", out]
+        if verbose:
+            print(" ".join(cmd), flush=True)
+        subprocess.run(cmd, check=True)
+    return out
+
+
 def build_calib(verbose: bool = False) -> str:
     os.makedirs(LIBDIR, exist_ok=True)
     out = os.path.join(LIBDIR, "libhbm_calib.so")
@@ -122,6 +147,7 @@
     build_hip(force=force, verbose=verbose)
     build_stamps(verbose=verbose, force=force)
     build_ric2(verbose=verbose, force=force)
+    build_norun(verbose=verbose, force=force)
     build_calib(verbose=verbose)
     build_oracle(force=force)
 
diff --git a/hpmpc_amd/csrc/hk_ipm_body.h b/hpmpc_amd/csrc/hk_ipm_body.h
--- a/hpmpc_amd/csrc/hk_ipm_body.h
+++ b/hpmpc_amd/csrc/hk_ipm_body.h
@@ -99,6 +99,7 @@
     io.RSQS = a.RSQ;
     io.F = F;
     io.DCt = a.DCt ? a.DCt + (long)p * a.sG : a.RSQ;
+    io.run = a.run;
     return io;
 }
 
@@ -422,7 +423,7 @@
 
 namespace {
 
-template <class FX>
+template <class FX, bool RUN = false>
 __device__ __forceinline__ void fact_body(const KArgs& a, const LdsTabs& T, IpmView& v) {
     Scratch& sm = *T.sm;
     const double* st = v.w.state;
@@ -438,17 +439,17 @@
     v.bc.cert = T.gc;
     if (st[S_PHASE] == 1.0) {
         if (first)
-            ric_backward<true, BX_P1, FX, CERT_FORM>(v.io, &sm, 0, nullptr, 0, nullptr, v.bc, 1, v.w.Pb);
+            ric_backward<true, BX_P1, FX, CERT_FORM, RUN>(v.io, &sm, 0, nullptr, 0, nullptr, v.bc, 1, v.w.Pb);
         else
-            ric_backward<true, BX_P1, FX, CERT_LOAD>(v.io, &sm, 0, nullptr, 0, nullptr, v.bc, 1, v.w.Pb);
+            ric_backward<true, BX_P1, FX, CERT_LOAD, RUN>(v.io, &sm, 0, nullptr, 0, nullptr, v.bc, 1, v.w.Pb);
     } else {
         v.bc.res_rhs = !sn;
         v.bc.no_tinv = a.no_bkp;
-        ric_backward<true, BX_P2R, FX, CERT_LOAD>(v.io, &sm, 0, nullptr, 0, nullptr, v.bc, 1, v.w.Pb);
-    }
-}
-
-template <class FX>
+        ric_backward<true, BX_P2R, FX, CERT_LOAD, RUN>(v.io, &sm, 0, nullptr, 0, nullptr, v.bc, 1, v.w.Pb);
+    }
+}
+
+template <class FX, bool RUN = false>
 __device__ __forceinline__ void pred_body(const KArgs& a, const LdsTabs& T, IpmView& v) {
     Scratch& sm = *T.sm;
     double* st = v.w.state;
@@ -459,9 +460,9 @@
     double al = 1.0;
     if (phase == 1) {
         v.bc.pred = 1;
-        ric_forward<0, BX_P1, FX, true>(v.io, &sm, nullptr, 0, v.w.dux, 0, v.w.dpi, v.bc, al);
+        ric_forward<0, BX_P1, FX, true, RUN>(v.io, &sm, nullptr, 0, v.w.dux, 0, v.w.dpi, v.bc, al);
     } else {
-        ric_forward<0, BX_P2, FX, true>(v.io, &sm, v.w.res_b, !sn, v.w.dux, 0, v.w.dpi, v.bc, al);
+        ric_forward<0, BX_P2, FX, true, RUN>(v.io, &sm, v.w.res_b, !sn, v.w.dux, 0, v.w.dpi, v.bc, al);
     }
     al = wave_min(al);
     wsync();
@@ -482,7 +483,7 @@
     }
 }
 
-template <class FX>
+template <class FX, bool RUN = false>
 __device__ __forceinline__ void corr_body(const KArgs& a, const LdsTabs& T, IpmView& v) {
     Scratch& sm = *T.sm;
     double* st = v.w.state;
@@ -490,10 +491,10 @@
     v.bc.smu = st[S_SMU];
     double al = 1.0;
     if (phase == 1)
-        ric_trs<BX_P1, BX_P1, FX, false>(v.io, &sm, nullptr, nullptr, v.bc, v.w.dux, a.compute_mult, v.w.dpi, 0, v.w.Pb,
+        ric_trs<BX_P1, BX_P1, FX, false, RUN>(v.io, &sm, nullptr, nullptr, v.bc, v.w.dux, a.compute_mult, v.w.dpi, 0, v.w.Pb,
                                          al);
     else
-        ric_trs<BX_P2, BX_P2, FX, false>(v.io, &sm, v.w.res_b, v.w.res_q, v.bc, v.w.dux, a.compute_mult, v.w.dpi, 0,
+        ric_trs<BX_P2, BX_P2, FX, false, RUN>(v.io, &sm, v.w.res_b, v.w.res_q, v.bc, v.w.dux, a.compute_mult, v.w.dpi, 0,
                                          v.w.Pb, al);
     al = wave_min(al);
     if (v.l == 0) {
diff --git a/hpmpc_amd/csrc/hk_plan.h b/hpmpc_amd/csrc/hk_plan.h
--- a/hpmpc_amd/csrc/hk_plan.h
+++ b/hpmpc_amd/csrc/hk_plan.h
@@ -1,5 +1,6 @@
 #pragma once
 #include <climits>
+#include <cstring>
 #include <mutex>
 #include <vector>
 
@@ -10,6 +11,48 @@
 struct StageInfoH {
     int nu, nx, nb, ng, xo, nx1, nu1, xo1, sdB, sdR, oB, oR, oD, pnb, r0, oG;
 };
+
+inline StageRun stage_run(int N, const StageInfoH* st, const signed char* tileslot) {
+    StageRun best{};
+#ifndef HK_NO_RUN
+    auto same = [&](int a, int b) {
+        return st[b].r0 == st[a].r0 && st[b].nb == st[a].nb && st[b].pnb == st[a].pnb && st[b].ng == 0 &&
+               !memcmp(tileslot + 16 * a, tileslot + 16 * b, 16);
+    };
+    int lo = 1;
+    while (lo < N) {
+        if (!(st[lo].r0 & 1) || st[lo].ng != 0) {
+            lo++;
+            continue;
+        }
+        int hi = lo, next = lo + 1;
+        while (hi + 1 < N && same(lo, hi + 1) && st[hi + 1].oD - st[hi].oD == V32) {
+            if (hi > lo && (st[hi + 1].oB - st[hi].oB != st[lo + 1].oB - st[lo].oB ||
+                            st[hi + 1].oR - st[hi].oR != st[lo + 1].oR - st[lo].oR)) {
+                next = hi;
+                break;
+            }
+            hi++;
+            next = hi + 1;
+        }
+        const int n = hi - lo + 1;
+        if (n > best.n) {
+            best.lo = lo;
+            best.n = n;
+            best.nb = st[lo].nb;
+            best.pnb = st[lo].pnb;
+            best.fl = st[lo].r0;
+            best.oB = st[lo].oB;
+            best.oR = st[lo].oR;
+            best.dB = n > 1 ? st[lo + 1].oB - st[lo].oB : 0;
+            best.dR = n > 1 ? st[lo + 1].oR - st[lo].oR : 0;
+        }
+        lo = next;
+    }
+    if (best.n < STAGE_RUN_MIN) best = StageRun{};
+#endif
+    return best;
+}
 
 struct hpmpc_mi355x_plan {
     int N = 0;
@@ -24,7 +67,9 @@
     struct LayoutTable {
         std::vector<StageInfoH> st;
         DevTable<StageInfoH> d;
+        StageRun run;
     };
+    StageRun run{};
     mutable std::vector<LayoutTable> ltabs;
     mutable std::mutex ltabs_mu;
     int fixcls = 0;
diff --git a/hpmpc_amd/csrc/hk_riccati.h b/hpmpc_amd/csrc/hk_riccati.h
--- a/hpmpc_amd/csrc/hk_riccati.h
+++ b/hpmpc_amd/csrc/hk_riccati.h
@@ -407,6 +407,7 @@
     const double* RSQS;
     double* F;
     const double* DCt;
+    StageRun run{};
 };
 
 __device__ __forceinline__ StageInfo load_stage(const StageInfo* st, int k) {
@@ -466,6 +467,41 @@
           oR(srd(s, &StageInfo::oR)), fl(srd(s, &StageInfo::r0)) {}
 };
 
+#ifdef HK_NO_RUN_BWD
+constexpr bool RUN_BWD = false;
+#else
+constexpr bool RUN_BWD = true;
+#endif
+#ifdef HK_NO_RUN_FWD
+constexpr bool RUN_FWD = false;
+#else
+constexpr bool RUN_FWD = true;
+#endif
+#ifdef HK_NO_RUN_TRS
+constexpr bool RUN_TRS = false;
+#else
+constexpr bool RUN_TRS = true;
+#endif
+
+template <class FX>
+struct RunSh;
+template <int NU, int NX>
+struct RunSh<FixSh<NU, NX>> {
+    using F = FixSh<NU, NX>;
+    static constexpr bool fixed = true, enabled = true;
+    static constexpr int nu = F::nu, nx = F::nx, xo = F::xo, nx1 = F::nx1, nu1 = F::nu1, xo1 = F::xo1, sdB = F::sdB,
+                         sdR = F::sdR;
+    int nb, pnb;
+    const double *B, *R;
+    __device__ __forceinline__ RunSh(const RicIO& io, int k)
+        : nb(io.run.nb), pnb(io.run.pnb),
+          B(((io.run.fl & 2) ? io.BAbtS : io.BAbt) + (io.run.oB + (long)(k - io.run.lo) * io.run.dB)),
+          R(((io.run.fl & 4) ? io.RSQS : io.RSQ) + (io.run.oR + (long)(k - io.run.lo) * io.run.dR)) {}
+    __device__ __forceinline__ void step(const StageRun& r, int d) {
+        B += d * r.dB;
+        R += d * r.dR;
+    }
+};
 
 __device__ __forceinline__ int stage_flags(const StageInfo& s) { return s.r0; }
 template <class SH>
@@ -478,6 +514,11 @@
 __device__ __forceinline__ const double* stage_R(const RicIO& io, const SH& sh) {
     return ((stage_flags(sh) & 4) ? io.RSQS : io.RSQ) + sh.oR;
 }
+
+template <int NU, int NX>
+__device__ __forceinline__ const double* stage_B(const RicIO&, const RunSh<FixSh<NU, NX>>& sh) { return sh.B; }
+template <int NU, int NX>
+__device__ __forceinline__ const double* stage_R(const RicIO&, const RunSh<FixSh<NU, NX>>& sh) { return sh.R; }
 
 struct NoFix {
     static constexpr bool enabled = false;
@@ -613,6 +654,11 @@
     b.up = b.lo + pnb;
     b.s16 = k * V16 + slot;
     return b;
+}
+__device__ __forceinline__ void box_lane_step(BoxLane& b, int d) {
+    b.lo += d * V32;
+    b.up += d * V32;
+    b.s16 += d * V16;
 }
 
 __device__ __forceinline__ void ld_lu(const double* p, const BoxLane& b, double& vlo, double& vup) {
@@ -873,8 +919,9 @@
 }
 
 template <bool AUG, int BM, class SH>
-__device__ __forceinline__ void bwd_fetch(const RicIO& io, const SH& sh, int k, int update_b, const double* bsrc,
-                                          int update_q, const double* qsrc, const BoxCtx& bc, BwdFrag& f) {
+__device__ __forceinline__ void bwd_fetch(const RicIO& io, const SH& sh, const BoxLane& b, int k, int update_b,
+                                          const double* bsrc, int update_q, const double* qsrc, const BoxCtx& bc,
+                                          BwdFrag& f) {
     const int l = lane_id(), g = l >> 4, c = l & 15;
     const int nux = sh.nu + sh.nx;
     const double* R = stage_R(io, sh);
@@ -886,7 +933,6 @@
         const int qi = update_q ? vc : lib4_idx(sh.sdR, nux, vc);
         f.mlq = ldsel(qp, qi, vc >= 0);
     }
-    const BoxLane b = box_lane(io.tileslot, sh.pnb, k);
     f.bl = b;
     f.gc = cert_loaded(BM) ? bc.cert[k] : 0.0;
 #pragma unroll
@@ -926,6 +972,11 @@
         f.pim1 = ldsel(bc.pi, (k - 1) * V16 + (vc - sh.nu), k > 0 && vc >= sh.nu);
         f.brow[0] = ldsel(Bk, lib4_idx(sh.sdB, nux, sc), oks);
     }
+}
+template <bool AUG, int BM, class SH>
+__device__ __forceinline__ void bwd_fetch(const RicIO& io, const SH& sh, int k, int update_b, const double* bsrc,
+                                          int update_q, const double* qsrc, const BoxCtx& bc, BwdFrag& f) {
+    bwd_fetch<AUG, BM>(io, sh, box_lane(io.tileslot, sh.pnb, k), k, update_b, bsrc, update_q, qsrc, bc, f);
 }
 
 template <bool AUG, int BM>
@@ -1138,7 +1189,7 @@
     bwd_core<AUG, cert_loaded(BM)>(io, sm, sh, k, cur.bop, cur.brow, M, ml, dq, gc, compute_Pb, Pb, S, ml_prev, invd_prev, kg_prev);
 }
 
-template <bool AUG, int BM, class FX, int CN = CERT_LOAD>
+template <bool AUG, int BM, class FX, int CN = CERT_LOAD, bool RUN = false>
 __device__ void ric_backward(const RicIO& io, Scratch* sm, int update_b, const double* bsrc, int update_q,
                              const double* qsrc, const BoxCtx& bc, int compute_Pb, double* Pb) {
     d4 S = {0.0, 0.0, 0.0, 0.0};
@@ -1182,6 +1233,35 @@
     };
     BwdFrag alt;
     for (int k = io.N;;) {
+        if constexpr (FX::enabled && RUN_BWD && RUN) {
+            const int klast = io.run.lo + 1;
+            if (io.run.n && k < io.run.lo + io.run.n - 1 && k - 1 >= klast) {
+                RunSh<FX> sh(io, k);
+                BoxLane bl = box_lane(io.tileslot, sh.pnb, k);
+                auto rstage = [&](int k, const BwdFrag& cur, BwdFrag& nxt) __attribute__((always_inline)) {
+                    HK_STAMP(0, k);
+                    sh.step(io.run, -1);
+                    box_lane_step(bl, -1);
+                    HK_STAMP(5, k);
+                    bwd_fetch<AUG, BM>(io, sh, bl, k - 1, update_b, bsrc, update_q, qsrc, bc, nxt);
+                    HK_STAMP(6, k);
+                    store_factor_fixed<FX::nx>(io.F + (long)(k + 1) * FSTRIDE, S, AUG ? ml_prev : 0.0, invd_prev,
+                                               kg_prev, true);
+                    asm volatile("" ::: "memory");
+                    HK_STAMP(1, k);
+                    bwd_step<AUG, BM, CN>(io, sm, sh, k, cur, bc, compute_Pb, Pb, S, ml_prev, invd_prev, kg_prev);
+                    if constexpr (BM == BX_P2R) bwd_residual(io, sm, sh, k - 1, bc, nxt, cur.uc, true);
+                    HK_STAMP(4, k);
+                };
+                do {
+                    rstage(k, cur, alt);
+                    rstage(k - 1, alt, cur);
+                    k -= 2;
+                } while (k - 1 >= klast);
+                si = StageRef{io.st, k};
+                rec_fixed = true;
+            }
+        }
         stage(k, cur, alt);
         if (--k < 0) break;
         stage(k, alt, cur);
@@ -1280,7 +1360,7 @@
 };
 
 template <int MODE, int FM, bool PRED, class SH>
-__device__ __forceinline__ void fwd_fetch(const RicIO& io, const SH& sh, int k, int pnbk, const double* bsrc,
+__device__ __forceinline__ void fwd_fetch(const RicIO& io, const SH& sh, int k, const BoxLane& b, const double* bsrc,
                                           int use_bsrc, const double* ux, int compute_pi_, const BoxCtx& bc,
                                           FwdFrag& f) {
     const int compute_pi = PRED ? 0 : compute_pi_;
@@ -1324,7 +1404,6 @@
 #pragma unroll
     for (int i = 0; i < 10; i++) f.bx[i] = 0.0;
     if (FM != BX_NONE) {
-        const BoxLane b = box_lane(io.tileslot, pnbk, k);
         f.bl = b;
         if (FM == BX_P1) {
             f.bx[0] = ldsel(bc.d, b.lo, b.ok);
@@ -1351,9 +1430,10 @@
                                             const double* ux, int compute_pi, const BoxCtx& bc, FwdFrag& f) {
     const int kk = k < io.N ? k : io.N - 1;
     const StageRef sk{io.st, kk};
-    const int pnbk = srd(StageRef{io.st, k}, &StageInfo::pnb);
+    BoxLane b{};
+    if (FM != BX_NONE) b = box_lane(io.tileslot, srd(StageRef{io.st, k}, &StageInfo::pnb), k);
     with_shape<FX>(sk, [&](const auto& sh) {
-        fwd_fetch<MODE, FM, PRED>(io, sh, k, pnbk, bsrc, use_bsrc, ux, compute_pi, bc, f);
+        fwd_fetch<MODE, FM, PRED>(io, sh, k, b, bsrc, use_bsrc, ux, compute_pi, bc, f);
     });
 }
 
@@ -1459,7 +1539,7 @@
     HK_STAMP(11, k);
 }
 
-template <int MODE, int FM, class FX, bool PRED = false>
+template <int MODE, int FM, class FX, bool PRED = false, bool RUN = false>
 __device__ void ric_forward(const RicIO& io, Scratch* sm, const double* bsrc, int use_bsrc, double* ux,
                             int compute_pi, double* pi, const BoxCtx& bc, double& al) {
     const int l = lane_id(), g = l >> 4, c = l & 15;
@@ -1490,6 +1570,28 @@
         box_alpha<FM, PRED>(bc, fN, xcol, al);
     };
     for (int k = 0;;) {
+        if constexpr (FX::enabled && RUN_FWD && RUN) {
+            const int klast = io.run.lo + io.run.n - 3;
+            if (io.run.n && k >= io.run.lo && k + 2 <= klast) {
+                RunSh<FX> sh(io, k + 1);
+                BoxLane bl{};
+                if (FM != BX_NONE) bl = box_lane(io.tileslot, sh.pnb, k + 1);
+                auto rstage = [&](int k, const FwdFrag& fa, FwdFrag& fc) __attribute__((always_inline)) {
+                    HK_STAMP(8, k);
+                    sh.step(io.run, 1);
+                    box_lane_step(bl, 1);
+                    fwd_fetch<MODE, FM, PRED>(io, sh, k + 2, bl, bsrc, use_bsrc, ux, compute_pi, bc, fc);
+                    fwd_step<MODE, FM, PRED>(io, sm, sh, k, fa, xcol, ux, compute_pi, pi, bc, al);
+                    HK_STAMP(12, k);
+                };
+                do {
+                    rstage(k, f0, f2);
+                    rstage(k + 1, f1, f0);
+                    rstage(k + 2, f2, f1);
+                    k += 3;
+                } while (k + 2 <= klast);
+            }
+        }
         if (k >= io.N) { finish(f0); break; }
         stage(k, f0, f1, f2);
         if (++k >= io.N) { finish(f1); break; }
@@ -1524,8 +1626,9 @@
 };
 
 template <int TM, bool RPB, class SH>
-__device__ __forceinline__ void trs_fetch(const RicIO& io, const SH& sh, int k, const double* hb, const double* hq,
-                                          const BoxCtx& bc, int compute_Pb_, const double* Pb, TrsFrag& f) {
+__device__ __forceinline__ void trs_fetch(const RicIO& io, const SH& sh, const BoxLane& b, int k, const double* hb,
+                                          const double* hq, const BoxCtx& bc, int compute_Pb_, const double* Pb,
+                                          TrsFrag& f) {
     const int compute_Pb = RPB ? compute_Pb_ : 0;
     const int l = lane_id(), g = l >> 4, c = l & 15;
     const double* Fk = io.F + (long)k * FSTRIDE;
@@ -1546,7 +1649,6 @@
     const int vc = tile_var(c, sh.nu, sh.nx, sh.xo);
     const double* R = stage_R(io, sh);
     f.h0 = hq ? ldsel(hq + k * V16, vc, vc >= 0) : ldsel(R, lib4_idx(sh.sdR, nux, vc), vc >= 0);
-    const BoxLane b = box_lane(io.tileslot, sh.pnb, k);
     f.bl = b;
 #pragma unroll
     for (int i = 0; i < 12; i++) f.bx[i] = 0.0;
@@ -1580,6 +1682,11 @@
     const int s = c - sh.xo1;
     f.pbc = ldsel(Pb + k * V16, s, !compute_Pb && live && s >= 0 && s < sh.nx1);
 }
+template <int TM, bool RPB, class SH>
+__device__ __forceinline__ void trs_fetch(const RicIO& io, const SH& sh, int k, const double* hb, const double* hq,
+                                          const BoxCtx& bc, int compute_Pb, const double* Pb, TrsFrag& f) {
+    trs_fetch<TM, RPB>(io, sh, box_lane(io.tileslot, sh.pnb, k), k, hb, hq, bc, compute_Pb, Pb, f);
+}
 
 template <int TM>
 __device__ __forceinline__ double box_gradient(const BoxCtx& bc, const TrsFrag& f) {
@@ -1644,7 +1751,7 @@
     S1 = cur.S;
 }
 
-template <int TM, int FM, class FX, bool RPB = true>
+template <int TM, int FM, class FX, bool RPB = true, bool RUN = false>
 __device__ void ric_trs(const RicIO& io, Scratch* sm, const double* hb, const double* hq, const BoxCtx& bc,
                         double* ux, int compute_pi, double* pi, int compute_Pb, double* Pb, double& al) {
     const int l = lane_id(), g = l >> 4, c = l & 15;
@@ -1671,6 +1778,25 @@
         with_shape<FX>(si, [&](const auto& sh) { trs_step<TM, RPB>(io, sm, sh, k, fa, bc, ux, compute_Pb, Pb, S1, pcol); });
     };
     for (int k = io.N - 1;;) {
+        if constexpr (FX::enabled && RUN_TRS && RUN) {
+            const int klast = io.run.lo + 1;
+            if (io.run.n && k < io.run.lo + io.run.n && k - 1 >= klast) {
+                RunSh<FX> sh(io, k);
+                BoxLane bl = box_lane(io.tileslot, sh.pnb, k);
+                auto rstage = [&](int k, const TrsFrag& fa, TrsFrag& fb) __attribute__((always_inline)) {
+                    sh.step(io.run, -1);
+                    box_lane_step(bl, -1);
+                    trs_fetch<TM, RPB>(io, sh, bl, k - 1, hb, hq, bc, compute_Pb, Pb, fb);
+                    asm volatile("" ::: "memory");
+                    trs_step<TM, RPB>(io, sm, sh, k, fa, bc, ux, compute_Pb, Pb, S1, pcol);
+                };
+                do {
+                    rstage(k, nxt, cur);
+                    rstage(k - 1, cur, nxt);
+                    k -= 2;
+                } while (k - 1 >= klast);
+            }
+        }
         if (k < 0) break;
         stage(k, nxt, cur);
         if (--k < 0) break;
@@ -1678,7 +1804,7 @@
         --k;
     }
     __syncthreads();
-    ric_forward<1, FM, FX>(io, sm, hb, hb != nullptr, ux, compute_pi, pi, bc, al);
-}
-
-}
+    ric_forward<1, FM, FX, false, RUN>(io, sm, hb, hb != nullptr, ux, compute_pi, pi, bc, al);
+}
+
+}
diff --git a/hpmpc_amd/csrc/hpmpc_capi.cpp b/hpmpc_amd/csrc/hpmpc_capi.cpp
--- a/hpmpc_amd/csrc/hpmpc_capi.cpp
+++ b/hpmpc_amd/csrc/hpmpc_capi.cpp
@@ -63,8 +63,8 @@
     return true;
 }
 
-static const void* plan_stage_table(const hpmpc_mi355x_plan* P, const long long* offB, const long long* offR,
-                                    const unsigned char* shB = nullptr, const unsigned char* shR = nullptr) {
+static std::vector<StageInfoH> layout_table(const hpmpc_mi355x_plan* P, const long long* offB, const long long* offR,
+                                            const unsigned char* shB, const unsigned char* shR) {
     const int N = P->N;
     std::vector<StageInfoH> st = P->st;
     for (int k = 0; k <= N; k++) {
@@ -72,11 +72,24 @@
         st[k].oR = (int)offR[k];
         st[k].r0 = (P->st[k].r0 & 1) | ((shB && k < N && shB[k]) ? 2 : 0) | ((shR && shR[k]) ? 4 : 0);
     }
+    return st;
+}
+
+static const void* plan_stage_table(const hpmpc_mi355x_plan* P, const long long* offB, const long long* offR,
+                                    const unsigned char* shB, const unsigned char* shR, StageRun* run) {
+    const int N = P->N;
+    std::vector<StageInfoH> st = layout_table(P, offB, offR, shB, shR);
     const size_t bytes = sizeof(StageInfoH) * (N + 1);
-    if (!memcmp(st.data(), P->st.data(), bytes)) return P->d_st.get();
+    if (!memcmp(st.data(), P->st.data(), bytes)) {
+        *run = P->run;
+        return P->d_st.get();
+    }
     std::lock_guard<std::mutex> lock(P->ltabs_mu);
     for (const auto& t : P->ltabs)
-        if (!memcmp(st.data(), t.st.data(), bytes)) return t.d.get();
+        if (!memcmp(st.data(), t.st.data(), bytes)) {
+            *run = t.run;
+            return t.d.get();
+        }
     constexpr size_t kMaxLayouts = 64;
     if (P->ltabs.size() >= kMaxLayouts) {
         hk_set_error(HPMPC_MI355X_EUNSUPPORTED, "more than 64 distinct stage layouts on one plan (create a plan per layout "
@@ -85,12 +98,13 @@
     }
     DevTable<StageInfoH> d;
     if (!d.upload(st, "layout stage table")) return nullptr;
-    P->ltabs.push_back({std::move(st), std::move(d)});
+    *run = stage_run(N, st.data(), P->tileslot.data());
+    P->ltabs.push_back({std::move(st), std::move(d), *run});
     return P->ltabs.back().d.get();
 }
 
-extern "C" hpmpc_mi355x_plan* hpmpc_mi355x_plan_create(int N, const int* nx, const int* nu, const int* nb,
-                                                       const int* const* idxb, const int* ng) {
+static hpmpc_mi355x_plan* plan_host(int N, const int* nx, const int* nu, const int* nb, const int* const* idxb,
+                                    const int* ng) {
     const char* why = nullptr;
     if (!plan_supported(N, nx, nu, nb, idxb, ng, &why)) {
         hk_set_error(HPMPC_MI355X_EUNSUPPORTED, why);
@@ -160,6 +174,14 @@
         P->st[k].oB = k < N ? (int)P->offB[k] : 0;
         P->st[k].oR = (int)P->offR[k];
     }
+    P->run = stage_run(N, P->st.data(), P->tileslot.data());
+    return P;
+}
+
+extern "C" hpmpc_mi355x_plan* hpmpc_mi355x_plan_create(int N, const int* nx, const int* nu, const int* nb,
+                                                       const int* const* idxb, const int* ng) {
+    hpmpc_mi355x_plan* P = plan_host(N, nx, nu, nb, idxb, ng);
+    if (!P) return nullptr;
     if (!P->d_st.upload(P->st, "plan tables") || !P->d_tileslot.upload(P->tileslot, "plan tables") ||
         !P->d_slotvar.upload(P->slotvar, "plan tables")) {
         delete P;
@@ -170,6 +192,23 @@
 }
 
 extern "C" void hpmpc_mi355x_plan_destroy(hpmpc_mi355x_plan* P) { delete P; }
+
+extern "C" int hpmpc_mi355x_stage_run(int N, const int* nx, const int* nu, const int* nb, const int* const* idxb,
+                                      const int* ng, const hpmpc_mi355x_layout* lay, int* out) {
+    hpmpc_mi355x_plan* P = plan_host(N, nx, nu, nb, idxb, ng);
+    if (!P) return g_err;
+    StageRun r = P->run;
+    if (lay && lay->BAbt_off && lay->RSQrq_off) {
+        const std::vector<StageInfoH> st =
+            layout_table(P, lay->BAbt_off, lay->RSQrq_off, lay->BAbt_shared, lay->RSQrq_shared);
+        r = stage_run(N, st.data(), P->tileslot.data());
+    }
+    const int v[9] = {r.lo, r.lo + r.n - 1, r.nb, r.pnb, r.fl, r.oB, r.dB, r.oR, r.dR};
+    memcpy(out, v, sizeof v);
+    delete P;
+    g_err = 0;
+    return 0;
+}
 
 void idxb_table(int N, const int* nb, const int* const* idxb, int* out) {
     for (int k = 0; k <= N; k++)
@@ -229,8 +268,9 @@
     a.st = P->d_st.get();
     a.tileslot = P->d_tileslot.get();
     a.slotvar = P->d_slotvar.get();
+    a.run = P->run;
     if (lay && lay->BAbt_off && lay->RSQrq_off) {
-        a.st = plan_stage_table(P, lay->BAbt_off, lay->RSQrq_off, lay->BAbt_shared, lay->RSQrq_shared);
+        a.st = plan_stage_table(P, lay->BAbt_off, lay->RSQrq_off, lay->BAbt_shared, lay->RSQrq_shared, &a.run);
         if (!a.st) return false;
     }
     a.sB = lay ? lay->BAbt_stride : P->packB;
diff --git a/hpmpc_amd/csrc/hpmpc_kargs.h b/hpmpc_amd/csrc/hpmpc_kargs.h
--- a/hpmpc_amd/csrc/hpmpc_kargs.h
+++ b/hpmpc_amd/csrc/hpmpc_kargs.h
@@ -27,6 +27,15 @@
 static_assert(K_PASS_FACT == K_PASS_INIT + 1 && K_PASS_PRED == K_PASS_INIT + 2 && K_PASS_CORR == K_PASS_INIT + 3 &&
                   K_PASS_UPDATE == K_PASS_INIT + 4,
               "the pass ids are consecutive: the host computes them as K_PASS_INIT + pass and K_PASS_FACT + i % 4");
+
+struct StageRun {
+    int lo, n;
+    int nb, pnb;
+    int fl;
+    int oB, oR;
+    int dB, dR;
+};
+constexpr int STAGE_RUN_MIN = 3;
 
 struct KArgs {
     int N, nprob, p0;
@@ -66,4 +75,5 @@
     int qpar;
     int* dctr;
     int* qnext;
+    StageRun run;
 };
diff --git a/hpmpc_amd/csrc/hpmpc_kernels.hip b/hpmpc_amd/csrc/hpmpc_kernels.hip
--- a/hpmpc_amd/csrc/hpmpc_kernels.hip
+++ b/hpmpc_amd/csrc/hpmpc_kernels.hip
@@ -125,6 +125,12 @@
 }
 
 
+#ifdef HK_RUN_SOLVES
+constexpr bool RUN_SOLVES = true;
+#else
+constexpr bool RUN_SOLVES = false;
+#endif
+
 template <class FX>
 __global__ __launch_bounds__(64) HK_TWO_WAVES void hk_ipm_fact(KArgs a) {
     if (a.nq && blockIdx.x == 0 && lane_id() == 0) *qcount(a, a.qpar ^ 1) = 0;
@@ -133,7 +139,7 @@
     const LdsTabs T = lds_tables(a);
     IpmView v = ipm_view(a, T, who);
     if (v.w.state[S_ACTIVE] == 0.0) return;
-    fact_body<FX>(a, T, v);
+    fact_body<FX, true>(a, T, v);
 }
 
 template <class FX>
@@ -143,7 +149,7 @@
     const LdsTabs T = lds_tables(a);
     IpmView v = ipm_view(a, T, who);
     if (v.w.state[S_ACTIVE] == 0.0) return;
-    pred_body<FX>(a, T, v);
+    pred_body<FX, RUN_SOLVES>(a, T, v);
 }
 
 template <class FX>
@@ -153,7 +159,7 @@
     const LdsTabs T = lds_tables(a);
     IpmView v = ipm_view(a, T, who);
     if (v.w.state[S_ACTIVE] == 0.0) return;
-    corr_body<FX>(a, T, v);
+    corr_body<FX, RUN_SOLVES>(a, T, v);
 }
 
 template <class FX>
@@ -164,14 +170,14 @@
     {
         IpmView v = ipm_view(a, T, who);
         if (v.w.state[S_ACTIVE] == 0.0) return;
-        pred_body<FX>(a, T, v);
+        pred_body<FX, RUN_SOLVES>(a, T, v);
     }
     wsync();
     int s = who.s, q = who.q, d = who.d;
     asm volatile("" : "+v"(s), "+v"(q), "+v"(d));
     const Who w2{__builtin_amdgcn_readfirstlane(s), __builtin_amdgcn_readfirstlane(q), __builtin_amdgcn_readfirstlane(d)};
     IpmView v = ipm_view(a, T, w2);
-    corr_body<FX>(a, T, v);
+    corr_body<FX, RUN_SOLVES>(a, T, v);
 }
 
 template <class FX>
diff --git a/include/hpmpc_mi355x.h b/include/hpmpc_mi355x.h
--- a/include/hpmpc_mi355x.h
+++ b/include/hpmpc_mi355x.h
@@ -161,6 +161,9 @@
     const unsigned char *RSQrq_shared;
 } hpmpc_mi355x_layout;
 
+int hpmpc_mi355x_stage_run(int N, const int *nx, const int *nu, const int *nb, const int *const *idxb,
+                           const int *ng, const hpmpc_mi355x_layout *lay, int *out);
+
 long long hpmpc_mi355x_ws_doubles(const hpmpc_mi355x_plan *plan);
 
 int hpmpc_mi355x_ipm_batch(const hpmpc_mi355x_plan *plan, const hpmpc_mi355x_layout *lay, int nprob, int p0,
```

After: 2.146 million. About the same (-0.1%).
